# emmyoh/zebra

Measured on AMD Instinct MI355X. Metric: queries/sec, higher is better.
Workload: dtype f32

## Files before the change

### zebra_amd/csrc/zh_api.hip

```cpp
#include <algorithm>
#include <atomic>
#include <chrono>
#include <condition_variable>
#include <cmath>
#include <deque>
#include <cstdarg>
#include <cstdio>
#include <cstring>
#include <mutex>
#include <shared_mutex>
#include <new>
#include <string>
#include <thread>
#include <vector>

#include "zh_internal.h"
#include "zh_snapfile.h"

static thread_local std::string g_err;

static int fail(int code, const char *fmt, ...) {
    char buf[512];
    va_list ap;
    va_start(ap, fmt);
    vsnprintf(buf, sizeof buf, fmt, ap);
    va_end(ap);
    g_err = buf;
    return code;
}
#define HIPCHK(expr)                                                                                       \
    do {                                                                                                   \
        hipError_t e_ = (expr);                                                                            \
        if (e_ != hipSuccess)                                                                              \
            return fail(e_ == hipErrorOutOfMemory ? ZH_ENOMEM : ZH_EHIP, "%s: %s (%s:%d)", #expr,          \
                        hipGetErrorString(e_), __FILE__, __LINE__);                                        \
    } while (0)

int zh_set_error(int code, const char *fmt, ...) {
    char buf[512];
    va_list ap;
    va_start(ap, fmt);
    vsnprintf(buf, sizeof buf, fmt, ap);
    va_end(ap);
    g_err = buf;
    return code;
}

extern "C" const char *zh_last_error(void) { return g_err.c_str(); }
extern "C" const char *zh_version(void) { return "zebra-hip 0.1 (gfx950)"; }

struct DevBuf {
    void *p = nullptr;
    size_t cap = 0;
    bool defer = false;
    std::vector<void *> old;
    size_t old_bytes = 0;
    int ensure(size_t bytes, bool keep = false, hipStream_t s = nullptr) {
        if (bytes <= cap) return ZH_OK;
        if (defer) bytes += bytes / 8;
        if (defer && old_bytes + cap > (size_t(2) << 30)) {
            for (void *o : old) hipFree(o);
            old.clear();
            old_bytes = 0;
        }
        size_t ncap = std::max(bytes, cap + cap / 2);
        ncap = (ncap + 255) & ~size_t(255);
        void *np = nullptr;
        hipError_t e = hipMalloc(&np, ncap);
        if (e != hipSuccess) {
            ncap = (bytes + 255) & ~size_t(255);
            e = hipMalloc(&np, ncap);
        }
        if (e != hipSuccess) return fail(ZH_ENOMEM, "hipMalloc(%zu bytes): %s", ncap, hipGetErrorString(e));
        if (keep && p && cap) {
            e = hipMemcpyAsync(np, p, cap, hipMemcpyDeviceToDevice, s);
            if (e == hipSuccess) e = hipStreamSynchronize(s);
            if (e != hipSuccess) { hipFree(np); return fail(ZH_EHIP, "grow copy: %s", hipGetErrorString(e)); }
        }
        if (p) { if (defer) { old.push_back(p); old_bytes += cap; } else hipFree(p); }
        p = np;
        cap = ncap;
        return ZH_OK;
    }
    void release() {
        if (p) hipFree(p);
        for (void *o : old) hipFree(o);
        old.clear();
        old_bytes = 0;
        p = nullptr;
        cap = 0;
    }
    template <typename T>
    T *as() const { return reinterpret_cast<T *>(p); }
};

struct zh_search_ctx {
    zh_index *ix = nullptr;
    DevBuf wQQ, wBits, wCounts, wInline, wRowBase, wCandBase, wVisitBase, wTotals, wVisits, wKeys, wCandKeys, wCandIds,
        wLeafCount, wLeafFill, wGroupBase, wGroupRowBase, wGroups, wGroupRowOff, wWaveGroup, wVisitBits, wNodeVisit, wScore, wJunkBits, wZeros, wQnorm, wQpad, wFixList, wLogPool, wLogHead, wLogCtl,
        wPfRows, wPfCounts, wPfKeys, wPfIds, wPfAmb, wPfCtl, wUnc, wQh, wQmeta, wApList, wApCount, wApEx, wApExKeys, wApCtl, wRaw;
    ZhApprox dbg_ap{};
    bool dbg_valid = false, dbg_raw = false;
    size_t log_chunks = 0;
    ZhTotals *h_totals = nullptr;
    hipEvent_t ev[6] = {};
    hipEvent_t ev_totals = nullptr, ev_emit = nullptr, ev_sw0 = nullptr, ev_sw1 = nullptr;
    bool ev_ok = false;
    int state = 0;
    bool trivial = false;
    const float *dQ = nullptr;
    size_t B = 0, k = 0;
    size_t nwin = 1, bwin = 0;
    DevBuf wQwin, wOutWin;
    int metric = 0, mode = 0;
    uint32_t P_dense = 0, wpq = 0;
    hipStream_t s = nullptr;
    ZhTotals tot{};
    bool scan = false;
    bool approx_f32rows = false;
    bool approx_fused = false;
    bool approx_bytes = false;
    bool approx = false, approx_mfma = false, approx_leaf = false;
    uint32_t *h_ap = nullptr;
    bool score_hash = false;
    uint32_t score_Bp = 0;
    bool lazy_fix = false;
    bool prefilter = false, prefilter_off_once = false, stream_ordered = false;
    uint32_t pf_cap = 0;
    uint32_t *h_pf = nullptr;
    std::vector<const float *> sv_q;
    std::vector<uint64_t *> sv_ids, sv_keys;
    std::vector<uint32_t *> sv_counts;
    hipStream_t sv_heavy = nullptr;
    std::vector<DevBuf *> all_bufs() {
        return {&wQQ, &wBits, &wCounts, &wInline, &wRowBase, &wCandBase, &wVisitBase, &wTotals, &wVisits, &wKeys,
                &wCandKeys, &wCandIds, &wLeafCount, &wLeafFill, &wGroupBase, &wGroupRowBase, &wGroups, &wGroupRowOff, &wWaveGroup, &wVisitBits, &wNodeVisit, &wScore, &wJunkBits, &wZeros, &wQnorm, &wQpad, &wFixList,
                &wLogPool, &wLogHead, &wLogCtl, &wQwin, &wOutWin, &wPfRows, &wPfCounts, &wPfKeys, &wPfIds, &wPfAmb, &wPfCtl, &wUnc,
                &wQh, &wQmeta, &wApList, &wApCount, &wApEx, &wApExKeys, &wApCtl, &wRaw};
    }
    void release_all() {
        for (DevBuf *b : all_bufs()) b->release();
        if (ev_ok) { for (auto &e : ev) hipEventDestroy(e); hipEventDestroy(ev_totals); hipEventDestroy(ev_emit); hipEventDestroy(ev_sw0); hipEventDestroy(ev_sw1); ev_ok = false; }
        if (h_totals) { hipHostFree(h_totals); h_totals = nullptr; }
        if (h_pf) { hipHostFree(h_pf); h_pf = nullptr; }
        if (h_ap) { hipHostFree(h_ap); h_ap = nullptr; }
    }
};

struct zh_index {
    zh_options opt{};
    int device = 0;
    hipStream_t stream = nullptr;
    hipStream_t sweep_stream = nullptr;
    std::shared_mutex mu;

    DevBuf X;
    uint64_t n_rows = 0;

    DevBuf node_plane, node_left, node_right, node_pack, roots, planes, consts, leaf_ids;
    uint32_t n_nodes = 0, n_planes = 0, n_trees = 0;
    uint64_t n_leaf_ids = 0;
    std::vector<int32_t> h_plane, h_left, h_right;
    std::vector<uint32_t> h_roots;
    std::vector<uint32_t> planes_below_level;
    std::vector<uint32_t> h_leaf_ids;
    std::vector<uint8_t> h_dead;
    uint64_t n_dead = 0;
    uint64_t rows_gen = 1, dead_gen = 1;
    uint32_t max_leaf_len = 0;
    std::mutex blk_mu;

    struct Stamp {
        std::atomic<uint64_t> rows{0}, gen{0};
        bool is(uint64_t r, uint64_t g) const { return rows == r && gen == g; }
        void set(uint64_t r, uint64_t g) { rows = r; gen = g; }
    };
    struct BlocksView {
        DevBuf recs, upper, roots;
        std::atomic<uint32_t> n_blocks{0}, n_upper{0};
        std::atomic<bool> valid{false};
        std::atomic<bool> inner{false};
        std::atomic<size_t> recs_b{0};
        void mark_built(uint32_t blocks, uint32_t uppers, bool inner_only, size_t second_halves) {
            n_blocks = blocks; n_upper = uppers; inner = inner_only; recs_b = second_halves; valid = true;
        }
        void invalidate() { valid = false; }
        void drop() { recs.release(); upper.release(); roots.release(); n_blocks = 0; n_upper = 0; inner = false; recs_b = 0; valid = false; }
    } blocks;
    struct RowLeafView {
        DevBuf table;
        std::atomic<bool> valid{false}, failed{false};
        std::atomic<uint64_t> rows{0};
        uint64_t version = 0;
        bool current(const zh_index *ix) const { return valid && rows == ix->n_rows; }
        void mark_built(uint64_t n) { valid = true; rows = n; version++; }
        void mark_failed() { failed = true; }
        void invalidate() { valid = false; failed = false; }
        void drop() { table.release(); invalidate(); }
    } row_leaf;
    struct RowHalfView {
        DevBuf tiles, meta, rho_dev;
        Stamp at;
        std::atomic<bool> failed{false};
        std::atomic<float> rho{0.f};
        bool current(const zh_index *ix) const { return at.is(ix->n_rows, ix->rows_gen); }
        bool known_failed(const zh_index *ix) const { return failed && current(ix); }
        void mark_built(const zh_index *ix, float r) { rho = r; at.set(ix->n_rows, ix->rows_gen); }
        void mark_failed(const zh_index *ix) { failed = true; at.set(ix->n_rows, ix->rows_gen); }
        void retry() { failed = false; }
        void remake() { at.gen = 0; }
        void drop() { at.set(0, 0); rho = 0.f; tiles.release(); meta.release(); failed = false; }
    } half;
    struct ScanOrder {
        DevBuf perm, row_leaf_p;
        bool off = false;
        uint32_t keys = 0;
        double worth = 0;
        uint64_t rows = 0;
        uint64_t version = 0;
// ... 2164 lines not shown
    zh_index *ix = c->ix;
    if (c->state != 1) return fail(ZH_ESTATE, "zh_search_finish without zh_search_begin");
    const uint32_t d = ix->opt.dim, T = ix->n_trees;
    const size_t B = c->B, k = c->k, nwin = c->nwin, bwin = c->bwin;
    hipStream_t s = c->s;
    int rc;
    c->state = 0;
    if (c->trivial) {
        for (size_t j = 0; j < nwin && bwin; j++) {
            HIPCHK(hipMemsetAsync(outCounts[j], 0, bwin * 4, s));
            if (k) {
                HIPCHK(hipMemsetAsync(outIds[j], 0xFF, bwin * k * 8, s));
                HIPCHK(hipMemsetAsync(outKeys[j], 0xFF, bwin * k * 8, s));
            }
        }
        HIPCHK(hipEventRecord(c->ev[5], s));
        c->state = 2;
        return ZH_OK;
    }
    uint64_t *dOutIds = outIds[0], *dOutKeys = outKeys[0];
    uint32_t *dOutCounts = outCounts[0];
    if (nwin > 1) {
        if ((rc = c->wOutWin.ensure(B * k * 16 + B * 4))) { return rc; }
        dOutIds = c->wOutWin.as<uint64_t>();
        dOutKeys = dOutIds + B * k;
        dOutCounts = reinterpret_cast<uint32_t *>(dOutKeys + B * k);
    }
    HIPCHK(hipEventSynchronize(c->ev_totals));
    const ZhTotals tot = c->tot = *c->h_totals;
    {
        std::lock_guard<std::mutex> lk(ix->stats_mu);
        const double v = (double)tot.visits / (double)((uint64_t)B * T);
        ix->visits_per_pair = ix->visits_per_pair > 0 ? 0.5 * (ix->visits_per_pair + v) : v;
    }
    if (tot.visits > 0xFFFFFFFull || tot.rows >= (1ull << 36))
        return fail(ZH_ELIMIT, "more than 2^28 leaf visits or 2^36 scored rows in one batch; use a smaller batch");
    c->sv_ids.assign(outIds, outIds + nwin); c->sv_keys.assign(outKeys, outKeys + nwin); c->sv_counts.assign(outCounts, outCounts + nwin);
    c->sv_heavy = heavy;
    if (c->prefilter && (tot.flags & 1u)) {
        const std::vector<const float *> q = c->sv_q;
        c->prefilter_off_once = true;
        rc = ctx_begin(c, q.data(), nwin, bwin, k, c->metric, c->mode, s);
        c->prefilter_off_once = false;
        if (rc) return rc;
        return ctx_finish(c, outIds, outKeys, outCounts, heavy);
    }
    if (c->prefilter) return finish_prefilter(c, dOutIds, dOutKeys, dOutCounts, outIds, outKeys, outCounts);
    if ((rc = c->wVisits.ensure(std::max<uint64_t>(tot.visits, 1) * sizeof(ZhVisit)))) return rc;
    if ((rc = c->wGroups.ensure(std::max<uint64_t>(tot.groups, 1) * sizeof(ZhGroup)))) return rc;
    if ((rc = c->wGroupRowOff.ensure(std::max<uint64_t>(tot.groups, 1) * 8))) return rc;
    if ((rc = c->wWaveGroup.ensure((tot.group_rows / 64 + 2) * 4))) return rc;
    if ((rc = c->wKeys.ensure(std::max<uint64_t>(tot.rows, 1) * 8))) return rc;
    if ((rc = c->wCandKeys.ensure(std::max<uint64_t>(tot.takes, 1) * 8))) return rc;
    if ((rc = c->wCandIds.ensure(std::max<uint64_t>(tot.takes, 1) * 4))) return rc;
    ZhForestDev f = forest_dev(ix);
    if (!(tot.flags & 1u)) {
        HIPCHK(zh_launch_expand(f, (uint32_t)B, c->wCounts.as<ZhPairCounts>(), c->wInline.as<ZhVisit>(),
                                c->wRowBase.as<uint64_t>(), c->wCandBase.as<uint64_t>(), c->wVisitBase.as<uint64_t>(),
                                c->wVisits.as<ZhVisit>(), c->wLeafCount.as<uint32_t>(), c->wLeafFill.as<uint32_t>(),
                                c->wGroupBase.as<uint32_t>(), c->wGroupRowBase.as<uint64_t>(), c->wGroups.as<ZhGroup>(),
                                c->wGroupRowOff.as<uint64_t>(), walk_log(c), s));
    } else {
        if (c->lazy_fix)
            HIPCHK(zh_launch_score_unc_fix(c->dQ, (uint32_t)B, d, f.planes, f.consts, ix->n_planes, c->wBits.as<uint32_t>(), c->wUnc.as<uint32_t>(), c->wpq, s));
        HIPCHK(zh_launch_walk_emit(f, c->dQ, (uint32_t)B, d, (int32_t)k, c->wBits.as<uint32_t>(), c->wpq, c->P_dense,
                                   c->wCounts.as<ZhPairCounts>(), c->wInline.as<ZhVisit>(), c->wRowBase.as<uint64_t>(),
                                   c->wCandBase.as<uint64_t>(), c->wVisitBase.as<uint64_t>(), c->wVisits.as<ZhVisit>(),
                                   c->wLeafCount.as<uint32_t>(), c->wLeafFill.as<uint32_t>(), c->wGroupBase.as<uint32_t>(),
                                   c->wGroupRowBase.as<uint64_t>(), c->wGroups.as<ZhGroup>(), c->wGroupRowOff.as<uint64_t>(), s));
        const uint64_t pairs = (uint64_t)B * T;
        const uint64_t want = tot.visits / (ZH_LOG_CHUNK - 1) + std::min<uint64_t>(pairs, tot.visits / (ZH_INLINE_VISITS + 1)) + 16;
        static const bool fixed = getenv("ZH_WALK_LOG_FIXED") != nullptr;
        if (!fixed && want > c->log_chunks) {
            const size_t chunks = (size_t)(want + want / 2);
            if (c->wLogPool.ensure(chunks * ZH_LOG_CHUNK * sizeof(uint2)) == ZH_OK) c->log_chunks = chunks;
        }
    }
    c->scan = choose_scan(ix, tot, c->metric, B, k);
    if (c->scan && !ix->row_leaf.current(ix)) {
        std::lock_guard<std::mutex> lk(ix->blk_mu);
        if (!ix->row_leaf.current(ix) && !ix->row_leaf.failed && (rc = build_row_leaf(ix))) return rc;
        if (!ix->row_leaf.current(ix)) c->scan = false;
    }
    if (c->scan) {
        const size_t nn = std::max<uint32_t>(ix->n_nodes, 1);
        if ((rc = c->wVisitBits.ensure((nn + 31) / 32 * 4))) return rc;
        if ((rc = c->wNodeVisit.ensure(nn * sizeof(uint4)))) return rc;
        HIPCHK(zh_launch_node_visits(c->wLeafCount.as<uint32_t>(), c->wGroupBase.as<uint32_t>(), c->wGroups.as<ZhGroup>(), ix->n_nodes,
                                     c->wVisitBits.as<uint32_t>(), c->wNodeVisit.as<uint4>(), s));
    }
    if (!c->scan)
        HIPCHK(zh_launch_wave_groups(c->wGroups.as<ZhGroup>(), c->wGroupRowOff.as<uint64_t>(), tot.groups, c->wWaveGroup.as<uint32_t>(), s));
    c->approx = c->scan && use_approx(ix, tot, B, k, c->metric);
    c->approx_leaf = false; c->approx_bytes = false;
    if (!c->scan && use_approx_leaf(ix, tot, B, k, c->metric)) {
        bool ok = false;
        const char *be = getenv("ZH_S128H_BYTES"), *ke = getenv("ZH_S128H_KERNEL"), *de = getenv("ZH_S128H_DMA");
        const bool want_bytes = !(be && be[0] == '0') && !(ke && ke[0] == 'r') && !(de && de[0] == '1');
        std::lock_guard<std::mutex> lk(ix->blk_mu);
        if ((rc = ensure_row_half128(ix, &ok, want_bytes))) return rc;
        c->approx = c->approx_leaf = ok;
        c->approx_bytes = ok && ix->half128.bytes;
    }
    ZhApprox ap{};
    bool mfma = c->approx && !c->approx_leaf && mfma_wanted(ix) && B < (1u << 23) - 1;
    const uint2 *scan_row_leaf = ix->row_leaf.table.as<uint2>();
    if (mfma) {
        std::lock_guard<std::mutex> lk(ix->blk_mu);
        if ((rc = ensure_row_half(ix, &mfma))) return rc;
        if (mfma && ix->order.rows) {
            if ((rc = ensure_row_leaf_p(ix))) return rc;
            if (!ix->order.rows) {
                ix->order.switch_off();
                ix->half.remake();
                if ((rc = ensure_row_half(ix, &mfma))) return rc;
            } else
                scan_row_leaf = ix->order.row_leaf_p.as<uint2>();
        }
    }
    c->approx_mfma = mfma;
    c->approx_f32rows = mfma && ix->half.tiles.p == nullptr;
    if (c->approx) {
        const char *cap_e = getenv("ZH_APX_CAPS");
        unsigned e_capq = 0, e_excap = 0, e_exrows = 0;
        if (cap_e) sscanf(cap_e, "%u,%u,%u", &e_capq, &e_excap, &e_exrows);
        const uint32_t capq = e_capq ? std::min(e_capq, 8192u) : (ix->fb.approx_strikes.load() ? 8192u : 4096u);
        const uint32_t ex_cap = e_excap ? e_excap : (uint32_t)std::min<uint64_t>(std::max<uint64_t>(4096, tot.visits / 4 + 1024), 1u << 24);
        const uint32_t ex_rows = e_exrows ? e_exrows : (uint32_t)std::min<uint64_t>(std::max<uint64_t>(1u << 20, tot.rows / 16), 1u << 26);
        if ((rc = c->wQh.ensure(B * d * 2)) || (rc = c->wQmeta.ensure(B * sizeof(float4))) || (rc = c->wApList.ensure((size_t)B * capq * 12)) ||
            (rc = c->wApCount.ensure(B * 8 + std::max<uint64_t>(tot.visits, 1) * 4)) || (rc = c->wApEx.ensure((size_t)ex_cap * 8)) || (rc = c->wApExKeys.ensure((size_t)ex_rows * 20)) ||
            (rc = c->wApCtl.ensure(ZH_APX_CTL_WORDS * 4)))
            return rc;
        ap.Qh = c->wQh.p; ap.qmeta = c->wQmeta.as<float4>(); ap.iv = c->wKeys.as<uint64_t>();
        ap.list_lo = c->wApList.as<uint32_t>(); ap.list_hi = ap.list_lo + (size_t)B * capq; ap.list_id = ap.list_hi + (size_t)B * capq;
        ap.qcount = c->wApCount.as<uint32_t>(); ap.capq = capq; ap.qtau = ap.qcount + B; ap.tauv = ap.qtau + B;
        ap.ex_visits = c->wApEx.as<uint2>(); ap.ex_cap = ex_cap;
        ap.ex_keys = c->wApExKeys.as<uint64_t>(); ap.ex_ckeys = ap.ex_keys + ex_rows; ap.ex_cids = reinterpret_cast<uint32_t *>(ap.ex_ckeys + ex_rows);
        ap.ex_rows_cap = ex_rows; ap.ctl = c->wApCtl.as<uint32_t>();
        ap.n_queries = (uint32_t)B; ap.iv_cap = tot.rows;
        ap.mfma = mfma ? 1u : 0u; ap.row_half = mfma ? ix->half.tiles.p : nullptr; ap.row_meta = mfma ? ix->half.meta.as<float2>() : nullptr;
        ap.row_rho = mfma ? ix->half.rho.load() : 0.f;
        if (c->approx_leaf) { ap.mfma = 2u; ap.row_rho = ap.rho_norm = c->approx_bytes ? 0.f : ix->half128.rho.load(); }
        const char *pte = getenv("ZH_S128H_PRETEST");
        ap.nx_max = c->approx_leaf && c->approx_bytes && !(pte && pte[0] == '0') ? 2885.1f : 0.f;
        HIPCHK(hipMemsetAsync(c->wApCount.p, 0, B * 4, s));
        HIPCHK(hipMemsetAsync(ap.qtau, 0xFF, B * 4, s));
        HIPCHK(hipMemsetAsync(c->wApCtl.p, 0, ZH_APX_CTL_WORDS * 4, s));
        HIPCHK(zh_launch_qhalf(c->dQ, (uint32_t)B, d, c->wQh.p, c->wQmeta.as<float4>(), c->approx_leaf ? 2 : (mfma ? 1 : 0), s));
    }
    HIPCHK(hipEventRecord(c->ev[2], s));
    hipStream_t hs = heavy ? heavy : s;
    if (hs != s) { HIPCHK(hipEventRecord(c->ev_emit, s)); HIPCHK(hipStreamWaitEvent(hs, c->ev_emit, 0)); }
    HIPCHK(hipEventRecord(c->ev_sw0, hs));
    c->approx_fused = false;
    if (c->approx_leaf && k <= 64 && !ix->debug_keep_raw) {
        const char *fe = getenv("ZH_S128H_FUSED"), *ke = getenv("ZH_S128H_KERNEL"), *de = getenv("ZH_S128H_DMA");
        const bool lean = !(ke && ke[0] == 'r') && !(de && de[0] == '1');
        c->approx_fused = lean && (fe ? fe[0] == '1' : (!ix->fb.fused_off && tot.rows >= 1024 * std::max<uint64_t>(tot.visits, 1)));
    }
    const int kinda = c->metric != ZH_COSINE ? 0 : (c->mode == ZH_COSINE_PARITY ? 2 : 1);
    if (c->approx_leaf)
        HIPCHK(zh_launch_sweep128h(ix->half128.copy.p, c->wQh.p, ldexpf(1.f, ix->half128.ex - 14), c->wGroups.as<ZhGroup>(), c->wGroupRowOff.as<uint64_t>(),
                                   tot.groups, c->wWaveGroup.as<uint32_t>(), f.leaf_ids, tot.group_rows, c->wKeys.as<uint64_t>(), hs,
                                   c->approx_fused ? &ap : nullptr, kinda, (uint32_t)k, zh_approx_bound(c->metric, d, 2), c->approx_bytes));
    else if (c->approx)
        HIPCHK(zh_launch_scan_approx(ix->X.as<float>(), d, ix->n_rows, ap, mfma ? scan_row_leaf : ix->row_leaf.table.as<uint2>(), T, c->wVisitBits.as<uint32_t>(),
                                     c->wNodeVisit.as<uint4>(), c->wGroups.as<ZhGroup>(), f.group, c->metric, c->mode, hs));
    else if (c->scan)
        HIPCHK(zh_launch_scan_sweep(ix->X.as<float>(), d, ix->n_rows, c->dQ, c->wQQ.as<float>(), ix->row_leaf.table.as<uint2>(), T,
                                    c->wVisitBits.as<uint32_t>(), c->wNodeVisit.as<uint4>(), c->wGroups.as<ZhGroup>(), f.group,
                                    c->metric, c->mode, c->wKeys.as<uint64_t>(), nullptr, hs));
    else
        HIPCHK(zh_launch_sweep(ix->X.as<float>(), d, c->dQ, c->wQQ.as<float>(), c->wGroups.as<ZhGroup>(),
                               c->wGroupRowOff.as<uint64_t>(), tot.groups, c->wWaveGroup.as<uint32_t>(), f.leaf_ids,
                               tot.group_rows, c->metric, c->mode, c->wKeys.as<uint64_t>(), hs));
    HIPCHK(hipEventRecord(c->ev_sw1, hs));
    if (hs != s) HIPCHK(hipStreamWaitEvent(s, c->ev_sw1, 0));
    HIPCHK(hipEventRecord(c->ev[3], s));
    const uint32_t *run_if = nullptr;
    c->dbg_valid = c->approx;
    c->dbg_raw = false;
    if (c->approx) {
        c->dbg_ap = ap;
        if (ix->debug_keep_raw && tot.rows) {
            if ((rc = c->wRaw.ensure(tot.rows * 8))) return rc;
            HIPCHK(hipMemcpyAsync(c->wRaw.p, c->wKeys.p, tot.rows * 8, hipMemcpyDeviceToDevice, s));
            c->dbg_raw = true;
        }
        if (c->approx_fused) HIPCHK(zh_launch_exact_register(c->wVisits.as<ZhVisit>(), tot.visits, (uint32_t)k, ap, s));
        else HIPCHK(zh_launch_select_interval(c->wVisits.as<ZhVisit>(), tot.visits, (uint32_t)k, f.leaf_ids, ap, c->metric, c->mode, d, s));
        HIPCHK(hipEventRecord(c->ev[4], s));
        HIPCHK(zh_launch_final_interval(c->wVisits.as<ZhVisit>(), ix->X.as<float>(), d, c->dQ, c->wQQ.as<float>(), (uint32_t)B, (uint32_t)k,
                                        f.leaf_ids, c->metric, c->mode, ix->opt.id_base, ap, dOutIds, dOutKeys, dOutCounts, ix->max_leaf_len, s));
        HIPCHK(hipMemcpyAsync(c->h_ap, c->wApCtl.p, ZH_APX_CTL_WORDS * 4, hipMemcpyDeviceToHost, s));
        run_if = ap.ctl + 1;
        if (c->approx_leaf)
            HIPCHK(zh_launch_sweep(ix->X.as<float>(), d, c->dQ, c->wQQ.as<float>(), c->wGroups.as<ZhGroup>(), c->wGroupRowOff.as<uint64_t>(), tot.groups,
                                   c->wWaveGroup.as<uint32_t>(), f.leaf_ids, tot.group_rows, c->metric, c->mode, c->wKeys.as<uint64_t>(), s, run_if));
        else
            HIPCHK(zh_launch_scan_sweep(ix->X.as<float>(), d, ix->n_rows, c->dQ, c->wQQ.as<float>(), ix->row_leaf.table.as<uint2>(), T,
                                        c->wVisitBits.as<uint32_t>(), c->wNodeVisit.as<uint4>(), c->wGroups.as<ZhGroup>(), f.group,
                                        c->metric, c->mode, c->wKeys.as<uint64_t>(), run_if, s));
    }
    HIPCHK(zh_launch_select(c->wVisits.as<ZhVisit>(), tot.visits, f.leaf_ids, c->wKeys.as<uint64_t>(),
                            c->wCandKeys.as<uint64_t>(), c->wCandIds.as<uint32_t>(), ix->max_leaf_len, run_if, s));
    if (!c->approx) HIPCHK(hipEventRecord(c->ev[4], s));
    HIPCHK(zh_launch_final(c->wCandBase.as<uint64_t>(), (uint32_t)B, T, (uint32_t)k, c->wCandKeys.as<uint64_t>(),
                           c->wCandIds.as<uint32_t>(), ix->opt.id_base, dOutIds, dOutKeys, dOutCounts, run_if, s));
    for (size_t j = 0; j < nwin && nwin > 1; j++) {
        HIPCHK(hipMemcpyAsync(outIds[j], dOutIds + j * bwin * k, bwin * k * 8, hipMemcpyDeviceToDevice, s));
        HIPCHK(hipMemcpyAsync(outKeys[j], dOutKeys + j * bwin * k, bwin * k * 8, hipMemcpyDeviceToDevice, s));
        HIPCHK(hipMemcpyAsync(outCounts[j], dOutCounts + j * bwin, bwin * 4, hipMemcpyDeviceToDevice, s));
    }
    HIPCHK(hipEventRecord(c->ev[5], s));
    c->state = 2;
    return ZH_OK;
}

int ctx_wait(zh_search_ctx *c) {
    zh_index *ix = c->ix;
    if (c->state == 1) return fail(ZH_ESTATE, "zh_search_wait: the batch was begun but not finished");
    if (c->state != 2) return ZH_OK;
    c->state = 0;
    HIPCHK(hipEventSynchronize(c->ev[5]));
    if (c->trivial) return ZH_OK;
    const bool pf = c->prefilter;
    const uint32_t pf_amb = pf ? c->h_pf[0] : 0, pf_flags = pf ? c->h_pf[1] : 0, pf_exact = pf ? c->h_pf[2] : 0;
    if (pf_flags) {
        {
            std::lock_guard<std::mutex> lk(ix->stats_mu);
            ix->stats.prefilter_fallbacks_accum++;
            ix->stats.prefilter_last_overflow = pf_flags;
        }
        ix->fb.prefilter_ran_over();
        const std::vector<const float *> q = c->sv_q;
        const std::vector<uint64_t *> ids = c->sv_ids, keys = c->sv_keys;
        const std::vector<uint32_t *> counts = c->sv_counts;
        c->prefilter_off_once = true;
        int rc = ctx_begin(c, q.data(), c->nwin, c->bwin, c->k, c->metric, c->mode, c->s);
        if (!rc) rc = ctx_finish(c, ids.data(), keys.data(), counts.data(), c->sv_heavy);
        c->prefilter_off_once = false;
        if (rc) return rc;
        return ctx_wait(c);
    }
    if (pf) ix->fb.prefilter_held();
    const ZhTotals tot = c->tot;
    uint64_t uniq = 0;
    if (ix->profiling >= 2 && tot.visits && !pf) {
        std::vector<ZhVisit> hv(tot.visits);
        HIPCHK(hipMemcpy(hv.data(), c->wVisits.p, tot.visits * sizeof(ZhVisit), hipMemcpyDeviceToHost));
        std::vector<std::pair<uint32_t, uint32_t>> leaves(hv.size());
        for (size_t i = 0; i < hv.size(); i++) leaves[i] = {hv[i].leaf_off, hv[i].len};
        std::sort(leaves.begin(), leaves.end());
        leaves.erase(std::unique(leaves.begin(), leaves.end()), leaves.end());
        for (auto &l : leaves) uniq += l.second;
    }
    float ms[5] = {0, 0, 0, 0, 0};
    if (ix->profiling > 0) {
        for (int i = 0; i < 5; i++) HIPCHK(hipEventElapsedTime(&ms[i], c->ev[i], c->ev[i + 1]));
        HIPCHK(hipEventElapsedTime(&ms[2], c->ev_sw0, c->ev_sw1));
    }
    std::lock_guard<std::mutex> lk(ix->stats_mu);
    zh_stats_t &st = ix->stats;
    st.batch = c->B; st.window_batches = c->nwin; st.visits = tot.visits; st.rows_scored = tot.rows; st.candidates = tot.takes;
    st.planes_dense = c->P_dense; st.planes_total = ix->n_planes;
    const uint64_t swept = pf ? pf_exact : (c->scan ? ix->n_rows : tot.group_rows);
    st.rows_swept = swept;
    st.sweep_bytes = pf ? tot.rows * 64 + (uint64_t)pf_exact * 4 * ix->opt.dim
                        : (c->scan ? ix->n_rows * ((uint64_t)4 * ix->opt.dim + 8 * ix->n_trees) + tot.rows * 8
                                   : tot.group_rows * ((uint64_t)4 * ix->opt.dim + 4) + tot.rows * 8);
    st.table_scan = c->scan && !pf ? 1 : 0;
    const bool apx = c->approx && !pf;
    st.approx_scan = apx ? (c->approx_leaf ? 3 : (c->approx_mfma ? 2 : 1)) : 0;
    st.approx_fused = apx && c->approx_leaf && c->approx_fused ? 1 : 0;
    st.approx_byte_rows = apx && c->approx_leaf && c->approx_bytes ? 1 : 0;
    st.approx_exact_visits = apx ? c->h_ap[0] : 0;
    st.approx_survivors = apx ? c->h_ap[3] : 0;
    st.approx_list_entries = apx ? c->h_ap[4] : 0;
    if (apx && c->h_ap[7]) fprintf(stderr, "zebra_hip: scan guard tripped, bits %u (diagnostic build)\n", c->h_ap[7]);
    st.approx_columns = apx && c->approx_mfma ? c->h_ap[5] : 0;
    st.approx_column_pairs = apx && c->approx_mfma ? c->h_ap[6] : 0;
    if (apx && c->h_ap[1]) {
        st.approx_fallbacks_accum++;
        st.approx_last_overflow = c->h_ap[1];
// ... 3683 lines not shown
```

### zebra_amd/csrc/zh_approx.hip

```cpp

#include <cstdlib>

#include "zh_internal.h"
#include "zh_device.h"

#ifndef ZH_APX_G768
#define ZH_APX_G768 2
#endif
#ifndef ZH_APX_G128
#define ZH_APX_G128 8
#endif
uint32_t zh_approx_groups(uint32_t d) {
    switch (d) {
    case 128: return ZH_APX_G128;
    case 256: case 384: return 4;
    case 768: return ZH_APX_G768;
    case 512: case 1024: return 2;
    default: return 0;
    }
}
bool zh_approx_pays(uint32_t d) { return d >= 384; }

float zh_approx_bound(int metric, uint32_t d, int mfma) {
    const double u = 5.9604644775390625e-8, c0 = (d + 255) / 256 + 8.0, ops = mfma ? 33.0 * (d / 128) + 2.0 + (mfma == 2 ? 40.0 : 0.0) : 0.0;
    if (metric == ZH_COSINE) return (float)(1.01 * (2.0 * c0 + 80.0 + 2.0 * ops) * u);
    return (float)(1.01 * (c0 + 100.0 + ops) * u);
}

__device__ __forceinline__ _Float16 f16_no_subnormal(float v) {
    const _Float16 h = (_Float16)v;
    return fabsf((float)h) < 6.103515625e-05f ? (_Float16)0.f : h;
}

template <int G>
__global__ __launch_bounds__(64) void qhalf_kernel(const float *__restrict__ Q, uint32_t B, uint32_t d, _Float16 *__restrict__ Qh,
                                                    float4 *__restrict__ qmeta) {
    constexpr uint32_t LG = 64 / G;
    const uint32_t b = blockIdx.x, lane = threadIdx.x;
    const float *q = Q + (size_t)b * d;
    float m = 0.f, s2 = 0.f;
    bool bad = false;
    for (uint32_t e = lane; e < d; e += 64) {
        const float v = q[e];
        bad |= !(v - v == 0.f);
        m = fmaxf(m, fabsf(v));
        s2 = __builtin_fmaf(v, v, s2);
    }
    m = wave_butterfly<OpMax>(m);
    s2 = wave_sum_canonical(s2);
    bad = __ballot(bad) != 0;
    float sigma = 1.f, inv = 1.f;
    if (!bad && m > 0.f) {
        int ex = 0;
        (void)frexpf(m, &ex);
        if (ex < -90 || ex > 90) bad = true;
        else { sigma = ldexpf(1.f, 14 - ex); inv = ldexpf(1.f, ex - 14); }
    }
    float d2 = 0.f;
    for (uint32_t e = lane; e < d; e += 64) {
        const float v = bad ? 0.f : q[e];
        const _Float16 h = f16_no_subnormal(v * sigma);
        const float df = v - (float)h * inv;
        d2 = __builtin_fmaf(df, df, d2);
        const uint32_t j = e / (4 * LG), rem = e % (4 * LG), l = rem / 4, t = rem % 4, i = j / 2, wh = j % 2;
        Qh[(size_t)b * d + ((size_t)(i * LG + l)) * 8 + wh * 4 + t] = h;
    }
    d2 = wave_sum_canonical(d2);
    if (lane == 0) {
        float4 o;
        if (bad || !(s2 - s2 == 0.f)) o = make_float4(NAN, NAN, NAN, NAN);
        else o = make_float4(inv, s2, sqrtf(s2) * (1.0f + 1e-5f), sqrtf(d2) * 1.001f);
        qmeta[b] = o;
    }
}

hipError_t zh_launch_qhalf(const float *dQ, uint32_t B, uint32_t d, void *dQh, float4 *dQmeta, int layout, hipStream_t s) {
    if (!B) return hipSuccess;
    const uint32_t G = layout == 2 ? 64 : (layout == 1 ? 16 : zh_approx_groups(d));
    if (G == 64) hipLaunchKernelGGL(qhalf_kernel<64>, dim3(B), dim3(64), 0, s, dQ, B, d, (_Float16 *)dQh, dQmeta);
    else if (G == 16) hipLaunchKernelGGL(qhalf_kernel<16>, dim3(B), dim3(64), 0, s, dQ, B, d, (_Float16 *)dQh, dQmeta);
    else if (G == 8) hipLaunchKernelGGL(qhalf_kernel<8>, dim3(B), dim3(64), 0, s, dQ, B, d, (_Float16 *)dQh, dQmeta);
    else if (G == 4) hipLaunchKernelGGL(qhalf_kernel<4>, dim3(B), dim3(64), 0, s, dQ, B, d, (_Float16 *)dQh, dQmeta);
    else if (G == 2) hipLaunchKernelGGL(qhalf_kernel<2>, dim3(B), dim3(64), 0, s, dQ, B, d, (_Float16 *)dQh, dQmeta);
    else return hipErrorInvalidValue;
    return hipGetLastError();
}

template <int LG>
__device__ __forceinline__ float group_sum(float s) {
    s = s + dpp_mov<0xB1>(s);
    s = s + dpp_mov<0x4E>(s);
    s = s + dpp_mov<0x141>(s);
    if (LG >= 16) s = s + dpp_mov<0x140>(s);
    if (LG >= 32) s = xor16<OpAdd>(s);
    if (LG >= 64) {
        const auto r = __builtin_amdgcn_permlane32_swap(__float_as_uint(s), __float_as_uint(s), false, false);
        s = __uint_as_float(r[0]) + __uint_as_float(r[1]);
    }
    return s;
}


__device__ __forceinline__ uint32_t scan_phase1(uint32_t lane, uint32_t n_ent, const uint2 *__restrict__ ent,
                                                const uint32_t *__restrict__ visitBits, const uint4 *__restrict__ nodeVisit,
                                                uint32_t *eGb, uint32_t *eWithin, uint32_t *eC, uint32_t *off, uint32_t *eB0, uint64_t *eK0) {
    unsigned long long rlw[ZH_SCAN_NE];
#pragma unroll
    for (int j = 0; j < ZH_SCAN_NE; j++) {
        const uint32_t e = lane + 64u * j;
        rlw[j] = __builtin_nontemporal_load(reinterpret_cast<const unsigned long long *>(ent + (e < n_ent ? e : 0)));
    }
    uint32_t word[ZH_SCAN_NE];
    bool in[ZH_SCAN_NE];
#pragma unroll
    for (int j = 0; j < ZH_SCAN_NE; j++) {
        const uint32_t node = (uint32_t)rlw[j];
        in[j] = lane + 64u * j < n_ent && node != 0xFFFFFFFFu;
        word[j] = visitBits[in[j] ? node >> 5 : 0];
    }
    uint4 nv[ZH_SCAN_NE];
#pragma unroll
    for (int j = 0; j < ZH_SCAN_NE; j++) {
        const uint32_t node = (uint32_t)rlw[j];
        in[j] = in[j] && ((word[j] >> (node & 31)) & 1u);
        nv[j] = nodeVisit[in[j] ? node : 0];
    }
    uint32_t P = 0;
#pragma unroll
    for (int j = 0; j < ZH_SCAN_NE; j++) {
        eWithin[j] = (uint32_t)(rlw[j] >> 32);
        eC[j] = in[j] ? nv[j].x & 0x0FFFFFFFu : 0u;
        eGb[j] = nv[j].y; eB0[j] = nv[j].z;
        eK0[j] = ((uint64_t)(nv[j].x >> 28) << 32) | nv[j].w;
        uint32_t incl = eC[j];
#pragma unroll
        for (int o = 1; o < 64; o <<= 1) {
            const uint32_t t = __shfl_up(incl, o);
            if (lane >= (uint32_t)o) incl += t;
        }
        off[j] = P + incl - eC[j];
        P += (uint32_t)__builtin_amdgcn_readlane((int)incl, 63);
    }
    return P;
}

#define ZH_APX_CAP 512
#ifndef ZH_APX_WAVES
#define ZH_APX_WAVES 0
#endif
#ifndef ZH_APX_REPL_ROWS
#define ZH_APX_REPL_ROWS 0
#endif
template <int D, int G, int KINDA>
__global__ __launch_bounds__(256)
#if ZH_APX_WAVES
__attribute__((amdgpu_waves_per_eu(ZH_APX_WAVES, 8)))
#endif
void scan_approx_kernel(const float *__restrict__ X, const uint4 *__restrict__ Qh,
                                                           const float4 *__restrict__ qmeta, const uint2 *__restrict__ rowLeaf,
                                                           uint32_t T, uint32_t RW, const uint32_t *__restrict__ visitBits,
                                                           const uint4 *__restrict__ nodeVisit, const ZhGroup *__restrict__ groups,
                                                           uint32_t GRP, uint64_t row_begin, uint64_t row_end, float Kc,
                                                           uint64_t *__restrict__ iv) {
    constexpr int LG = 64 / G, NH = D * G / 512, NR = 2 * NH;
    constexpr int RB = NR <= 6 ? 4 : 2;
    static_assert(D * G % 512 == 0 && NH >= 1, "a lane's share of a query is whole 16-byte loads");
    __shared__ uint4 pair_list[4][ZH_APX_CAP];
    __shared__ uint32_t row_start[4][20];
    const uint32_t lane = threadIdx.x & 63, l = lane & (LG - 1), g = lane / LG;
    const uint32_t wid = (uint32_t)__builtin_amdgcn_readfirstlane((int)(threadIdx.x >> 6));
    const uint64_t wave = (uint64_t)blockIdx.x * (blockDim.x >> 6) + wid;
    const uint64_t r0 = row_begin + wave * RW;
    if (r0 >= row_end) return;
    const uint32_t nr = (uint32_t)(row_end - r0 < RW ? row_end - r0 : RW);
    const uint32_t n_ent = nr * T;
    const uint2 *__restrict__ ent = rowLeaf + (size_t)r0 * T;
    uint32_t eGb[ZH_SCAN_NE], eWithin[ZH_SCAN_NE], eC[ZH_SCAN_NE], off[ZH_SCAN_NE], eB0[ZH_SCAN_NE];
    uint64_t eK0[ZH_SCAN_NE];
    const uint32_t P = scan_phase1(lane, n_ent, ent, visitBits, nodeVisit, eGb, eWithin, eC, off, eB0, eK0);
    if (P == 0) return;
    const float4 *__restrict__ X4 = reinterpret_cast<const float4 *>(X);
    float my_s = 0.f, my_a2 = 0.f;
    uint64_t my_slot = 0;
    uint32_t nst = 0;
    bool my_on = false;
    auto flush = [&]() {
        if (my_on) __builtin_nontemporal_store(((uint64_t)__float_as_uint(my_a2) << 32) | __float_as_uint(my_s), iv + my_slot);
        my_on = false;
        nst = 0;
    };
    auto load_q = [&](uint32_t b, uint4 *hq) {
        const uint4 *qp = Qh + (size_t)b * (D / 8) + l;
#pragma unroll
        for (int i = 0; i < NH; i++) hq[i] = qp[i * LG];
    };
    auto load_x = [&](uint64_t row, float4 *v) {
        if constexpr (G == 2 && !ZH_APX_REPL_ROWS) {
            const float4 *r4 = X4 + (size_t)row * (D / 4) + lane;
#pragma unroll
            for (int j = 0; j < NR / 2; j++) {
                const float4 t = ld16<true>(r4 + 64 * j);
                const auto sx = __builtin_amdgcn_permlane32_swap(__float_as_uint(t.x), __float_as_uint(t.x), false, false);
                const auto sy = __builtin_amdgcn_permlane32_swap(__float_as_uint(t.y), __float_as_uint(t.y), false, false);
                const auto sz = __builtin_amdgcn_permlane32_swap(__float_as_uint(t.z), __float_as_uint(t.z), false, false);
                const auto sw = __builtin_amdgcn_permlane32_swap(__float_as_uint(t.w), __float_as_uint(t.w), false, false);
                v[2 * j] = make_float4(__uint_as_float(sx[0]), __uint_as_float(sy[0]), __uint_as_float(sz[0]), __uint_as_float(sw[0]));
                v[2 * j + 1] = make_float4(__uint_as_float(sx[1]), __uint_as_float(sy[1]), __uint_as_float(sz[1]), __uint_as_float(sw[1]));
            }
        } else {
            const float4 *r4 = X4 + (size_t)row * (D / 4) + l;
#pragma unroll
            for (int j = 0; j < NR; j++) v[j] = ld16<true>(r4 + LG * j);
        }
    };
    auto row_sumsq = [&](const float4 *v) {
        float4 c = make_float4(0.f, 0.f, 0.f, 0.f);
#pragma unroll
        for (int j = 0; j < NR; j++) sq4(v[j], c);
        return group_sum<LG>((c.x + c.y) + (c.z + c.w));
    };
    auto dot_h = [&](const float4 *v, const uint4 *hq) {
        float ax = 0.f, ay = 0.f, az = 0.f, aw = 0.f;
#pragma unroll
        for (int i = 0; i < NH; i++) {
            f16x8 h;
            __builtin_memcpy(&h, &hq[i], 16);
            ax = __builtin_fmaf(v[2 * i].x, (float)h[0], ax);
            ay = __builtin_fmaf(v[2 * i].y, (float)h[1], ay);
            az = __builtin_fmaf(v[2 * i].z, (float)h[2], az);
            aw = __builtin_fmaf(v[2 * i].w, (float)h[3], aw);
            ax = __builtin_fmaf(v[2 * i + 1].x, (float)h[4], ax);
            ay = __builtin_fmaf(v[2 * i + 1].y, (float)h[5], ay);
            az = __builtin_fmaf(v[2 * i + 1].z, (float)h[6], az);
            aw = __builtin_fmaf(v[2 * i + 1].w, (float)h[7], aw);
        }
        return group_sum<LG>((ax + ay) + (az + aw));
    };
    auto stash = [&](float s, float a2, uint32_t, uint64_t slot, bool valid) {
        if (l == nst) { my_s = s; my_a2 = a2; my_slot = slot; my_on = valid; }
        if (++nst == (uint32_t)LG) flush();
    };
    if (P <= ZH_APX_CAP) {
        uint4 *list = pair_list[wid];
        uint32_t *rstart = row_start[wid];
        uint32_t mrows = 0;
#pragma unroll
        for (int j = 0; j < ZH_SCAN_NE; j++) {
            const uint32_t e = lane + 64u * j, c = eC[j];
            if (e < n_ent && e % T == 0) rstart[e / T] = off[j];
            if (c) {
                const uint32_t rl = e / T, gb = eGb[j];
                mrows |= 1u << rl;
                {
                    const uint64_t slot = eK0[j] + eWithin[j];
                    list[off[j]] = make_uint4(rl, eB0[j], (uint32_t)slot, (uint32_t)(slot >> 32));
                }
                for (uint32_t sidx = 1; sidx < c; sidx++) {
                    const ZhGroup *gp = groups + gb + sidx / GRP;
                    const uint64_t slot = gp->key_off[sidx % GRP] + eWithin[j];
                    list[off[j] + sidx] = make_uint4(rl, gp->b[sidx % GRP], (uint32_t)slot, (uint32_t)(slot >> 32));
                }
            }
// ... 70 lines not shown
                    uint4 hq[NH];
                    load_q(b, hq);
                    const float s = dot_h(v, hq);
                    stash(s, a2, b, gp->key_off[sidx % GRP] + w, s0 + g < c);
                }
            }
        }
    }
    flush();
}


__global__ __launch_bounds__(256) void row_half_kernel(const float *__restrict__ X, uint64_t row0, uint64_t n_rows, uint32_t d,
                                                       _Float16 *__restrict__ Xh, float2 *__restrict__ rowMeta, uint32_t *__restrict__ rhoMax,
                                                       const uint32_t *__restrict__ perm, uint64_t perm_rows) {
    const uint32_t lane = threadIdx.x & 63, NS = d / 32;
    const uint64_t nw = (uint64_t)gridDim.x * 4;
    float rho_w = 0.f;
    for (uint64_t i = (uint64_t)blockIdx.x * 4 + (threadIdx.x >> 6); i < n_rows; i += nw) {
        const uint64_t row = row0 + i;
        const float *x = X + (size_t)(perm && row < perm_rows ? perm[row] : row) * d;
        float m = 0.f, a2 = 0.f;
        bool bad = false;
        for (uint32_t e = lane; e < d; e += 64) {
            const float v = x[e];
            bad |= !(v - v == 0.f);
            m = fmaxf(m, fabsf(v));
            a2 = __builtin_fmaf(v, v, a2);
        }
        m = wave_butterfly<OpMax>(m);
        a2 = wave_sum_canonical(a2);
        bad = __ballot(bad) != 0;
        bool usable = false;
        float sigma = 1.f, inv = __uint_as_float(0x7FC00000u);
        if (!bad) {
            int ex = 14;
            if (m > 0.f) (void)frexpf(m, &ex);
            if (ex >= -100 && ex <= 100) { usable = true; sigma = ldexpf(1.f, 14 - ex); inv = ldexpf(1.f, ex - 14); }
        }
        float s2 = 0.f, d2 = 0.f;
        _Float16 *tile = Xh + ((size_t)(row >> 4) * NS * 64 + (row & 15)) * 8;
        for (uint32_t e = lane; e < d; e += 64) {
            const float v = x[e] * sigma;
            const _Float16 hv = usable ? f16_no_subnormal(v) : (_Float16)0.f;
            const float df = v - (float)hv;
            s2 = __builtin_fmaf(v, v, s2);
            d2 = __builtin_fmaf(df, df, d2);
            const uint32_t st = e >> 5, w = e & 31, hh = (w & 15) >> 2, j = (w & 3) + ((w >> 4) << 2);
            if (Xh) tile[((size_t)st * 64 + hh * 16) * 8 + j] = hv;
        }
        s2 = wave_sum_canonical(s2);
        d2 = wave_sum_canonical(d2);
        if (usable && s2 > 0.f) rho_w = fmaxf(rho_w, sqrtf(d2) * 1.001f / (sqrtf(s2) * 0.9999f));
        if (lane == 0) rowMeta[row] = make_float2(a2, inv);
    }
    if (lane == 0 && rho_w > 0.f) atomicMax(rhoMax, __float_as_uint(rho_w));
}

hipError_t zh_launch_row_half(const float *dX, uint64_t row0, uint64_t n_rows, uint32_t d, void *dXh, float2 *dRowMeta, uint32_t *dRhoMax,
                              const uint32_t *dPerm, uint64_t perm_rows, hipStream_t s) {
    if (!n_rows) return hipSuccess;
    const uint64_t blocks = std::min<uint64_t>((n_rows + 3) / 4, 256 * 32);
    hipLaunchKernelGGL(row_half_kernel, dim3((uint32_t)blocks), dim3(256), 0, s, dX, row0, n_rows, d, (_Float16 *)dXh, dRowMeta, dRhoMax, dPerm, perm_rows);
    return hipGetLastError();
}

__global__ __launch_bounds__(256) void permute_row_leaf_kernel(const uint2 *__restrict__ rowLeaf, const uint32_t *__restrict__ perm, uint64_t perm_rows,
                                                               uint64_t n_entries, uint32_t T, uint2 *__restrict__ out) {
    for (uint64_t e = (uint64_t)blockIdx.x * blockDim.x + threadIdx.x; e < n_entries; e += (uint64_t)gridDim.x * blockDim.x) {
        const uint64_t p = e / T, t = e % T;
        out[e] = rowLeaf[(size_t)(p < perm_rows ? perm[p] : p) * T + t];
    }
}
hipError_t zh_launch_permute_row_leaf(const uint2 *dRowLeaf, const uint32_t *dPerm, uint64_t perm_rows, uint64_t n_rows, uint32_t T, uint2 *dOut, hipStream_t s) {
    const uint64_t n = n_rows * T;
    if (!n) return hipSuccess;
    hipLaunchKernelGGL(permute_row_leaf_kernel, dim3((uint32_t)std::min<uint64_t>((n + 255) / 256, 256 * 64)), dim3(256), 0, s, dRowLeaf, dPerm, perm_rows, n, T, dOut);
    return hipGetLastError();
}

#ifndef ZH_MFMA_CL
#define ZH_MFMA_CL 0
#endif
#ifdef ZH_SCAN_GUARD
#define ZH_GUARD(cond, bit) ((cond) ? true : (atomicOr(guard, (bit)), false))
#else
#define ZH_GUARD(cond, bit) true
#endif
#ifdef ZH_SCAN_PROF
__device__ unsigned long long zh_scan_prof_buf[16];
extern "C" __attribute__((visibility("default"))) int zh_debug_scan_prof(uint64_t *out, uint32_t words, int reset) {
    static const unsigned long long zero[16] = {};
    if (reset) return (int)hipMemcpyToSymbol(HIP_SYMBOL(zh_scan_prof_buf), zero, sizeof(zero));
    return (int)hipMemcpyFromSymbol(out, HIP_SYMBOL(zh_scan_prof_buf), (size_t)words * 8);
}
#define SP(...) __VA_ARGS__
#else
#define SP(...)
#endif
#ifndef ZH_MFMA_WAVES
#define ZH_MFMA_WAVES 3
#endif
template <int D, bool F32ROWS>
__global__ __launch_bounds__(256) __attribute__((amdgpu_waves_per_eu(D > 768 ? 2 : ZH_MFMA_WAVES, D > 768 ? 2 : ZH_MFMA_WAVES)))
void scan_mfma_kernel(const u32x4 *__restrict__ Xh, const float *__restrict__ Xf, const float2 *__restrict__ rowMeta,
                                                         const uint4 *__restrict__ Qh, const uint2 *__restrict__ rowLeaf, uint32_t T,
                                                         uint32_t RW, const uint32_t *__restrict__ visitBits,
                                                         const uint4 *__restrict__ nodeVisit, const ZhGroup *__restrict__ groups,
                                                         uint32_t GRP, uint64_t row_begin, uint64_t row_end, uint64_t *__restrict__ iv,
                                                         uint32_t *__restrict__ colStats ,
                                                         uint32_t nq, uint64_t iv_cap, uint32_t *__restrict__ guard) {
    constexpr int NS = D / 32;
    constexpr int NL = D / 64;
    constexpr int CL = ZH_MFMA_CL ? ZH_MFMA_CL : (NL % 4 == 0 ? 2 : 3);
    constexpr int NCH = NL / CL;
    static_assert(D % 128 == 0 && NL % CL == 0 && NCH % 2 == 0, "four accumulators; the chunk registers alternate with a static parity");
    __shared__ uint64_t pair_list[4][ZH_APX_CAP > CL * 256 ? ZH_APX_CAP : CL * 256];
    __shared__ uint64_t tile_list[4][ZH_APX_CAP];
    __shared__ uint32_t col_query[4][ZH_APX_CAP];
    __shared__ uint32_t tile_start[4][36];
    __shared__ f32x4 acc_lds[4][64];
    __shared__ float2 row_meta[4][16];
    const uint32_t lane = threadIdx.x & 63, c16 = lane & 15, h = lane >> 4;
    const uint32_t wid = (uint32_t)__builtin_amdgcn_readfirstlane((int)(threadIdx.x >> 6));
    const uint64_t wave = (uint64_t)blockIdx.x * (blockDim.x >> 6) + wid;
    const uint64_t r0 = row_begin + wave * RW;
    if (r0 >= row_end) return;
    SP(const uint64_t sp0 = clock64();)
    const uint32_t nr = (uint32_t)(row_end - r0 < RW ? row_end - r0 : RW);
    const uint32_t n_ent = nr * T;
    const uint2 *__restrict__ ent = rowLeaf + (size_t)r0 * T;
    uint32_t eGb[ZH_SCAN_NE], eWithin[ZH_SCAN_NE], eC[ZH_SCAN_NE], off[ZH_SCAN_NE], eB0[ZH_SCAN_NE];
    uint64_t eK0[ZH_SCAN_NE];
    const uint32_t P = scan_phase1(lane, n_ent, ent, visitBits, nodeVisit, eGb, eWithin, eC, off, eB0, eK0);
    if (P == 0) return;
    SP(const uint64_t sp1 = clock64();)
    uint64_t *list = pair_list[wid];
    const bool listed = P <= ZH_APX_CAP;
    auto pack = [](uint32_t rl, uint32_t b, uint64_t slot) { return slot | ((uint64_t)b << 36) | ((uint64_t)rl << 60); };
#pragma unroll
    for (int j = 0; j < ZH_SCAN_NE; j++) {
        const uint32_t e = lane + 64u * j, c = eC[j];
        if (c && listed && ZH_GUARD(off[j] + c <= (uint32_t)ZH_APX_CAP && e / T < 16u, 32u)) {
            const uint32_t rl = e / T, gb = eGb[j];
            list[off[j]] = pack(rl, eB0[j], eK0[j] + eWithin[j]);
            for (uint32_t sidx = 1; sidx < c; sidx++) {
                const ZhGroup *gp = groups + gb + sidx / GRP;
                list[off[j] + sidx] = pack(rl, gp->b[sidx % GRP], gp->key_off[sidx % GRP] + eWithin[j]);
            }
        }
    }
    SP(__builtin_amdgcn_s_waitcnt(0); const uint64_t sp2 = clock64();)
    f16x8 A[NS];
    if constexpr (!F32ROWS) {
        const u32x4 *tp = Xh + (size_t)(r0 >> 4) * (NS * 64) + lane;
#pragma unroll
        for (int st = 0; st < NS; st++) A[st] = __builtin_bit_cast(f16x8, __builtin_nontemporal_load(tp + 64 * st));
        if (lane < 16) row_meta[wid][lane] = rowMeta[r0 + (lane < nr ? lane : 0u)];
        __builtin_amdgcn_fence(__ATOMIC_RELEASE, "wavefront");
        __builtin_amdgcn_wave_barrier();
    } else {
        if (lane < 16) row_meta[wid][lane] = rowMeta[r0 + (lane < nr ? lane : 0u)];
        __builtin_amdgcn_fence(__ATOMIC_RELEASE, "wavefront");
        __builtin_amdgcn_wave_barrier();
        const float inv_c = row_meta[wid][c16].y;
        const bool usable_c = inv_c - inv_c == 0.f;
        const float sigma_c = usable_c ? 1.0f / inv_c : 0.f;
        f32x4 *xt = reinterpret_cast<f32x4 *>(tile_list[wid]);
        const f32x4 *X4 = reinterpret_cast<const f32x4 *>(Xf);
        const uint32_t g4 = lane >> 4, p16 = lane & 15;
        auto cvt8 = [&](const f32x4 lo, const f32x4 hi) {
            f16x8 o;
#pragma unroll
            for (int t = 0; t < 4; t++) {
                o[t] = usable_c ? f16_no_subnormal(lo[t] * sigma_c) : (_Float16)0.f;
                o[4 + t] = usable_c ? f16_no_subnormal(hi[t] * sigma_c) : (_Float16)0.f;
            }
            return o;
        };
        f32x4 Rr[4];
        auto issue_rows = [&](int kb) {
#pragma unroll
            for (int i = 0; i < 4; i++) {
                const uint32_t rr = 4u * i + g4;
                Rr[i] = __builtin_nontemporal_load(X4 + (size_t)(r0 + (rr < nr ? rr : nr - 1)) * (D / 4) + kb * 16 + p16);
            }
        };
        issue_rows(0);
#pragma unroll
        for (int kb = 0; kb < D / 64; kb++) {
#pragma unroll
            for (int i = 0; i < 4; i++) {
                const uint32_t rr = 4u * i + g4;
                xt[rr * 16 + (p16 ^ rr)] = Rr[i];
            }
            __builtin_amdgcn_fence(__ATOMIC_RELEASE, "wavefront");
            __builtin_amdgcn_wave_barrier();
            if (kb + 1 < D / 64) issue_rows(kb + 1);
#pragma unroll
            for (int s2 = 0; s2 < 2; s2++) {
                const f32x4 lo = xt[c16 * 16 + ((8u * s2 + h) ^ c16)], hi = xt[c16 * 16 + ((8u * s2 + 4u + h) ^ c16)];
                A[2 * kb + s2] = cvt8(lo, hi);
            }
            __builtin_amdgcn_fence(__ATOMIC_RELEASE, "wavefront");
            __builtin_amdgcn_wave_barrier();
        }
    }
    const float2 *rmeta = row_meta[wid];
    u32x4 *stg = reinterpret_cast<u32x4 *>(pair_list[wid]);
    const u32x4 *__restrict__ Qv = reinterpret_cast<const u32x4 *>(Qh);
    const uint32_t g8 = lane >> 3, pc = lane & 7;
    const uint32_t swA = (g8 >> 1) & 7u, swB = (4u + (g8 >> 1)) & 7u;
    const uint32_t rd0 = (c16 >> 3) * 64u + (c16 & 7u) * 8u + ((h ^ (c16 >> 1)) & 7u);
    const uint32_t rd1 = (c16 >> 3) * 64u + (c16 & 7u) * 8u + (((4u + h) ^ (c16 >> 1)) & 7u);
    auto issue = [&](uint32_t bA, uint32_t bB, int chunk, u32x4 *dst) {
        if (!ZH_GUARD(bA < nq && bB < nq, 1u)) { bA = 0; bB = 0; }
        const u32x4 *qa = Qv + (size_t)bA * (D / 8) + (size_t)(chunk * CL * 8) + (pc ^ swA);
// ... 101 lines not shown
        }
        __builtin_amdgcn_fence(__ATOMIC_RELEASE, "wavefront");
        __builtin_amdgcn_wave_barrier();
        const uint32_t nt = (nd + 15) / 16;
        SP(const uint64_t sp3 = clock64();)
        if (colStats && lane == 0 && (wave & 63u) == 0u) { atomicAdd(&colStats[0], nd); atomicAdd(&colStats[1], P); }
        auto col_b = [&](uint32_t t, uint32_t col) { const uint32_t ci = 16 * t + col; return colq[ci < nd ? ci : nd - 1]; };
        uint32_t bA = col_b(0, g8), bB = col_b(0, 8 + g8);
        u32x4 ra[2 * CL], rb[2 * CL];
        issue(bA, bB, 0, ra);
        SP(__builtin_amdgcn_s_waitcnt(0); const uint64_t sp4 = clock64();)
        f32x4 *al = acc_lds[wid];
        for (uint32_t t = 0; t < nt; t++) {
            f32x4 acc[4] = {{0.f, 0.f, 0.f, 0.f}, {0.f, 0.f, 0.f, 0.f}, {0.f, 0.f, 0.f, 0.f}, {0.f, 0.f, 0.f, 0.f}};
#pragma unroll
            for (int c = 0; c < NCH; c += 2) {
                issue(bA, bB, c + 1, rb);
                to_lds(ra);
                mfma_chunk(c, acc);
                if (c + 2 < NCH) issue(bA, bB, c + 2, ra);
                else {
                    bA = col_b(t + 1, g8); bB = col_b(t + 1, 8 + g8);
                    issue(bA, bB, 0, ra);
                }
                to_lds(rb);
                mfma_chunk(c + 1, acc);
            }
            al[c16 * 4 + h] = (acc[0] + acc[1]) + (acc[2] + acc[3]);
            __builtin_amdgcn_fence(__ATOMIC_RELEASE, "wavefront");
            __builtin_amdgcn_wave_barrier();
            const uint32_t pe = tstart[t + 1];
            for (uint32_t pi = tstart[t] + lane; pi < pe; pi += 64) {
                const uint64_t rec = tl[pi];
                const uint32_t rl = (uint32_t)(rec >> 60), col = (uint32_t)(rec >> 36) & 15u;
                const float sv = reinterpret_cast<const float *>(al)[col * 16 + rl];
                const float2 rm = rmeta[rl];
                if (ZH_GUARD((rec & 0xFFFFFFFFFull) < iv_cap, 2u))
                    __builtin_nontemporal_store(((uint64_t)__float_as_uint(rm.x) << 32) | __float_as_uint(sv * rm.y), iv + (rec & 0xFFFFFFFFFull));
            }
            __builtin_amdgcn_wave_barrier();
        }
        SP(if ((wave & 15u) == 0u && lane == 0) {
            __builtin_amdgcn_s_waitcnt(0);
            const uint64_t sp5 = clock64();
            atomicAdd(&zh_scan_prof_buf[0], 1ull); atomicAdd(&zh_scan_prof_buf[1], sp1 - sp0); atomicAdd(&zh_scan_prof_buf[2], sp2 - sp1);
            atomicAdd(&zh_scan_prof_buf[3], sp3 - sp2); atomicAdd(&zh_scan_prof_buf[4], sp4 - sp3); atomicAdd(&zh_scan_prof_buf[5], sp5 - sp4);
            atomicAdd(&zh_scan_prof_buf[6], (unsigned long long)nt); atomicAdd(&zh_scan_prof_buf[7], (unsigned long long)P);
            atomicAdd(&zh_scan_prof_buf[8], (unsigned long long)nd); atomicAdd(&zh_scan_prof_buf[9], sp5 - sp0);
        })
    } else {
#pragma unroll
        for (int j = 0; j < ZH_SCAN_NE; j++) {
            unsigned long long m = __ballot(eC[j] != 0);
            while (m) {
                const int ll = __builtin_ctzll(m);
                m &= m - 1;
                const uint32_t c = (uint32_t)__builtin_amdgcn_readlane((int)eC[j], ll);
                const uint32_t gb = (uint32_t)__builtin_amdgcn_readlane((int)eGb[j], ll);
                const uint32_t w = (uint32_t)__builtin_amdgcn_readlane((int)eWithin[j], ll);
                const uint32_t rl = ((uint32_t)ll + 64u * j) / T;
                for (uint32_t s0 = 0; s0 < c; s0 += 16) {
                    auto visit_b = [&](uint32_t col) { const uint32_t si = s0 + col < c ? s0 + col : c - 1; return groups[gb + si / GRP].b[si % GRP]; };
                    const uint32_t bA = visit_b(g8), bB = visit_b(8 + g8);
                    const uint32_t sidx = s0 + c16 < c ? s0 + c16 : c - 1;
                    const ZhGroup *gp = groups + gb + sidx / GRP;
                    f32x4 acc[4] = {{0.f, 0.f, 0.f, 0.f}, {0.f, 0.f, 0.f, 0.f}, {0.f, 0.f, 0.f, 0.f}, {0.f, 0.f, 0.f, 0.f}};
                    u32x4 rq[2 * CL];
#pragma unroll
                    for (int cc = 0; cc < NCH; cc++) {
                        issue(bA, bB, cc, rq);
                        to_lds(rq);
                        mfma_chunk(cc, acc);
                        __builtin_amdgcn_sched_barrier(0);
                    }
                    emit(acc, rl, gp->key_off[sidx % GRP] + w, s0 + c16 < c);
                }
            }
        }
    }
}

template <int D>
static hipError_t launch_scan_mfma_d(const float *dX, uint64_t n_rows, const ZhApprox &ap, const uint2 *dRowLeaf, uint32_t T,
                                     const uint32_t *dVisitBits, const uint4 *dNodeVisit, const ZhGroup *dGroups, uint32_t group, hipStream_t s) {
    const uint32_t RW = zh_scan_rows_per_wave(T);
    uint64_t rows_per_launch = zh_sweep_rows_per_launch(D);
    rows_per_launch = rows_per_launch / (4 * RW) * (4 * RW);
    for (uint64_t r = 0; r < n_rows; r += rows_per_launch) {
        const uint64_t r_end = r + rows_per_launch < n_rows ? r + rows_per_launch : n_rows;
        const uint64_t waves = (r_end - r + RW - 1) / RW, blocks = (waves + 3) / 4;
        if (blocks > 0x7FFFFFFFull) return hipErrorInvalidValue;
        if (ap.row_half)
            hipLaunchKernelGGL((scan_mfma_kernel<D, false>), dim3((uint32_t)blocks), dim3(256), 0, s, (const u32x4 *)ap.row_half, dX, ap.row_meta, (const uint4 *)ap.Qh, dRowLeaf, T, RW,
                               dVisitBits, dNodeVisit, dGroups, group, r, r_end, ap.iv, ap.ctl + 5, ap.n_queries, ap.iv_cap, ap.ctl + 7);
        else
            hipLaunchKernelGGL((scan_mfma_kernel<D, true>), dim3((uint32_t)blocks), dim3(256), 0, s, (const u32x4 *)nullptr, dX, ap.row_meta, (const uint4 *)ap.Qh, dRowLeaf, T, RW,
                               dVisitBits, dNodeVisit, dGroups, group, r, r_end, ap.iv, ap.ctl + 5, ap.n_queries, ap.iv_cap, ap.ctl + 7);
    }
    return hipGetLastError();
}

__global__ __launch_bounds__(256) void absmax_kernel(const float *__restrict__ X, uint64_t n, uint32_t *__restrict__ out) {
    float m = 0.f;
    for (uint64_t i = (uint64_t)blockIdx.x * blockDim.x + threadIdx.x; i < n; i += (uint64_t)gridDim.x * blockDim.x) {
        const float v = fabsf(X[i]);
        if (v - v == 0.f) m = fmaxf(m, v);
    }
    m = wave_butterfly<OpMax>(m);
    if ((threadIdx.x & 63) == 0 && m > 0.f) atomicMax(out, __float_as_uint(m));
}

__global__ __launch_bounds__(256) void row_half128_kernel(const float *__restrict__ X, uint64_t row0, uint64_t n_rows, float sigma,
                                                          _Float16 *__restrict__ Xh, uint32_t *__restrict__ rhoMax) {
    const uint32_t lane = threadIdx.x & 63;
    const uint64_t nw = (uint64_t)gridDim.x * 4;
    float rho_w = 0.f;
    for (uint64_t i = (uint64_t)blockIdx.x * 4 + (threadIdx.x >> 6); i < n_rows; i += nw) {
        const uint64_t row = row0 + i;
        const float2 x = reinterpret_cast<const float2 *>(X + (size_t)row * 128)[lane];
        const float v0 = x.x * sigma, v1 = x.y * sigma;
        bool bad = !(v0 - v0 == 0.f) || !(v1 - v1 == 0.f) || fabsf(v0) > 60000.f || fabsf(v1) > 60000.f;
        const _Float16 h0 = f16_no_subnormal(v0), h1 = f16_no_subnormal(v1);
        const float d0 = v0 - (float)h0, d1 = v1 - (float)h1;
        const float s2 = wave_sum_canonical(__builtin_fmaf(v0, v0, v1 * v1));
        const float d2 = wave_sum_canonical(__builtin_fmaf(d0, d0, d1 * d1));
        const float m = wave_butterfly<OpMax>(fmaxf(fabsf(x.x), fabsf(x.y)));
        bad = __ballot(bad) != 0 || !(s2 - s2 == 0.f) || (s2 == 0.f && m > 0.f);
        const float rho = s2 > 0.f ? sqrtf(d2) * 1.001f / (sqrtf(s2) * 0.9999f) : 0.f;
        bad = bad || !(rho <= 9.765625e-4f);
        if (!bad) rho_w = fmaxf(rho_w, rho);
        const _Float16 nanh = (_Float16)__uint_as_float(0x7FC00000u);
        typedef _Float16 f16x2v __attribute__((ext_vector_type(2)));
        reinterpret_cast<f16x2v *>(Xh + (size_t)row * 128)[lane] = bad ? f16x2v{nanh, nanh} : f16x2v{h0, h1};
    }
    if (lane == 0 && rho_w > 0.f) atomicMax(rhoMax, __float_as_uint(rho_w));
}

hipError_t zh_launch_absmax(const float *dX, uint64_t n, uint32_t *dOut, hipStream_t s) {
    if (!n) return hipSuccess;
    hipLaunchKernelGGL(absmax_kernel, dim3((uint32_t)std::min<uint64_t>((n + 255) / 256, 256 * 16)), dim3(256), 0, s, dX, n, dOut);
    return hipGetLastError();
}
hipError_t zh_launch_row_half128(const float *dX, uint64_t row0, uint64_t n_rows, float sigma, void *dXh, uint32_t *dRhoMax, hipStream_t s) {
    if (!n_rows) return hipSuccess;
    hipLaunchKernelGGL(row_half128_kernel, dim3((uint32_t)std::min<uint64_t>((n_rows + 3) / 4, 256 * 32)), dim3(256), 0, s, dX, row0, n_rows, sigma,
                       (_Float16 *)dXh, dRhoMax);
    return hipGetLastError();
}

__global__ __launch_bounds__(256) void row_byte128_kernel(const float4 *__restrict__ X4, uint64_t n4, uint32_t *__restrict__ Xb,
                                                          uint32_t *__restrict__ notBytes) {
    bool bad = false;
    for (uint64_t i = (uint64_t)blockIdx.x * 256 + threadIdx.x; i < n4; i += (uint64_t)gridDim.x * 256) {
        const float4 v = X4[i];
        const float e[4] = {v.x, v.y, v.z, v.w};
        uint32_t w = 0;
#pragma unroll
        for (int j = 0; j < 4; j++) {
            const uint32_t b = (uint32_t)fminf(fmaxf(e[j], 0.f), 255.f);
            bad |= !((float)b == e[j]);
            w |= b << (8 * j);
        }
        Xb[i] = w;
    }
    if (__ballot(bad) != 0 && (threadIdx.x & 63) == 0) atomicOr(notBytes, 1u);
}
hipError_t zh_launch_row_byte128(const float *dX, uint64_t row0, uint64_t n_rows, void *dXb, uint32_t *dNotBytes, hipStream_t s) {
    if (!n_rows) return hipSuccess;
    const uint64_t n4 = n_rows * 32;
    hipLaunchKernelGGL(row_byte128_kernel, dim3((uint32_t)std::min<uint64_t>((n4 + 255) / 256, 256 * 32)), dim3(256), 0, s,
                       reinterpret_cast<const float4 *>(dX + (size_t)row0 * 128), n4, reinterpret_cast<uint32_t *>(dXb) + (size_t)row0 * 32, dNotBytes);
    return hipGetLastError();
}
__device__ __forceinline__ f16x8 bytes8_to_f16(uint32_t w0, uint32_t w1) {
    typedef _Float16 h2 __attribute__((ext_vector_type(2)));
    const h2 off = {(_Float16)-1024.f, (_Float16)-1024.f};
    const h2 a = __builtin_bit_cast(h2, __builtin_amdgcn_perm(0x64646464u, w0, 0x04010400u)) + off;
    const h2 b = __builtin_bit_cast(h2, __builtin_amdgcn_perm(0x64646464u, w0, 0x04030402u)) + off;
    const h2 c = __builtin_bit_cast(h2, __builtin_amdgcn_perm(0x64646464u, w1, 0x04010400u)) + off;
    const h2 d = __builtin_bit_cast(h2, __builtin_amdgcn_perm(0x64646464u, w1, 0x04030402u)) + off;
// ... 880 lines not shown
#define ZH_S128L_CH 4
#endif
#ifndef ZH_S128F_CH
#define ZH_S128F_CH 16
#endif
#ifndef ZH_S128H_LAUNCH_X
#define ZH_S128H_LAUNCH_X 4
#endif
#ifndef ZH_S128B_LAUNCH_X
#define ZH_S128B_LAUNCH_X 8
#endif
#ifndef ZH_S128B_CH
#define ZH_S128B_CH 64
#endif
uint64_t zh_sweep128h_rows_per_launch(bool lean, bool byte_rows) {
    return (lean ? (byte_rows ? ZH_S128B_LAUNCH_X : ZH_S128H_LAUNCH_X) : 1) * zh_sweep_rows_per_launch(128);
}
template <int FUSE, bool BYTES>
static void launch_sweep128h_lean(const void *dXh, const void *dQh, float inv, const ZhGroup *dGroups, const uint64_t *dGroupRowOff, uint64_t n_groups,
                                  const uint32_t *dWaveGroup, const uint32_t *dLeafIds, uint64_t R_grouped, uint64_t *dIv, const ZhApprox &ap,
                                  uint32_t k_top, float Kc, hipStream_t s) {
    const uint64_t rows_per_launch = zh_sweep128h_rows_per_launch(true, BYTES);
    for (uint64_t r = 0; r < R_grouped; r += rows_per_launch) {
        const uint64_t r_end = r + rows_per_launch < R_grouped ? r + rows_per_launch : R_grouped;
        constexpr int CHL = FUSE >= 0 ? (BYTES ? ZH_S128B_CH : ZH_S128F_CH) : ZH_S128L_CH;
        const uint64_t wl = (r_end - r + 64 * CHL - 1) / (64 * CHL);
        if constexpr (BYTES)
            hipLaunchKernelGGL((sweep128b_lean_kernel<CHL, FUSE>), dim3((uint32_t)((wl + 3) / 4)), dim3(256), 0, s, (const u32x4 *)dXh,
                               (const u32x4 *)dQh, dGroups, dGroupRowOff, n_groups, dWaveGroup, dLeafIds, r, r_end, dIv, ap, k_top, Kc);
        else
            hipLaunchKernelGGL((sweep128h_lean_kernel<CHL, FUSE>), dim3((uint32_t)((wl + 3) / 4)), dim3(256), 0, s, (const u32x4 *)dXh,
                               (const u32x4 *)dQh, inv, dGroups, dGroupRowOff, n_groups, dWaveGroup, dLeafIds, r, r_end, dIv, ap, k_top, Kc);
    }
    const uint64_t bw = ((R_grouped + 63) / 64 + 63) / 64, bb = (bw + 3) / 4;
    hipLaunchKernelGGL((sweep128h_boundary_kernel<FUSE, BYTES>), dim3((uint32_t)bb), dim3(256), 0, s, (const u32x4 *)dXh, (const u32x4 *)dQh, inv, dGroups,
                       dGroupRowOff, n_groups, dWaveGroup, dLeafIds, (uint64_t)0, R_grouped, dIv, ap, k_top, Kc);
}
hipError_t zh_launch_sweep128h(const void *dXh, const void *dQh, float inv, const ZhGroup *dGroups, const uint64_t *dGroupRowOff, uint64_t n_groups,
                               const uint32_t *dWaveGroup, const uint32_t *dLeafIds, uint64_t R_grouped, uint64_t *dIv, hipStream_t s,
                               const ZhApprox *fuse, int fuse_kinda, uint32_t k_top, float Kc, bool byte_rows) {
    if (R_grouped == 0 || n_groups == 0) return hipSuccess;
    constexpr int CH = 4;
    const uint64_t rows_per_launch = zh_sweep_rows_per_launch(128);
    if ((R_grouped + 16383) / 16384 > 0x7FFFFFFFull) return hipErrorInvalidValue;
    const char *dma_e = getenv("ZH_S128H_DMA"), *kern_e = getenv("ZH_S128H_KERNEL");
    const bool dma = dma_e && dma_e[0] == '1', r5 = kern_e && kern_e[0] == 'r';
    if (fuse) {
        if (!dWaveGroup || k_top == 0 || k_top > 64) return hipErrorInvalidValue;
#define ZH_LEAN(F)                                                                                                                                  \
    do {                                                                                                                                            \
        if (byte_rows) launch_sweep128h_lean<F, true>(dXh, dQh, 1.f, dGroups, dGroupRowOff, n_groups, dWaveGroup, dLeafIds, R_grouped, dIv, *fuse, k_top, Kc, s); \
        else launch_sweep128h_lean<F, false>(dXh, dQh, inv, dGroups, dGroupRowOff, n_groups, dWaveGroup, dLeafIds, R_grouped, dIv, *fuse, k_top, Kc, s);           \
    } while (0)
        if (fuse_kinda == 0) ZH_LEAN(0);
        else if (fuse_kinda == 1) ZH_LEAN(1);
        else ZH_LEAN(2);
#undef ZH_LEAN
        return hipGetLastError();
    }
    if (!dma && !r5) {
        const ZhApprox none{};
        if (byte_rows) launch_sweep128h_lean<-1, true>(dXh, dQh, 1.f, dGroups, dGroupRowOff, n_groups, dWaveGroup, dLeafIds, R_grouped, dIv, none, 0u, 0.f, s);
        else launch_sweep128h_lean<-1, false>(dXh, dQh, inv, dGroups, dGroupRowOff, n_groups, dWaveGroup, dLeafIds, R_grouped, dIv, none, 0u, 0.f, s);
        return hipGetLastError();
    }
    if (byte_rows) return hipErrorInvalidValue;
    for (uint64_t r = 0; r < R_grouped; r += rows_per_launch) {
        const uint64_t r_end = r + rows_per_launch < R_grouped ? r + rows_per_launch : R_grouped;
        const uint64_t w = (r_end - r + 64 * CH - 1) / (64 * CH), blocks = (w + 3) / 4;
        if (!dma)
            hipLaunchKernelGGL((sweep128h_kernel<CH>), dim3((uint32_t)blocks), dim3(256), 0, s, (const u32x4 *)dXh, (const u32x4 *)dQh, inv, dGroups,
                               dGroupRowOff, n_groups, dWaveGroup, dLeafIds, r, r_end, dIv);
        else
            hipLaunchKernelGGL((sweep128h_dma_kernel<CH>), dim3((uint32_t)blocks), dim3(256), 0, s, (const u32x4 *)dXh, (const u32x4 *)dQh, inv, dGroups,
                               dGroupRowOff, n_groups, dWaveGroup, dLeafIds, r, r_end, dIv);
    }
    return hipGetLastError();
}


template <int G, int KINDA>
__global__ __launch_bounds__(256) void scan_approx128_kernel(const float *__restrict__ X, const uint4 *__restrict__ Qh,
                                                              const float4 *__restrict__ qmeta, const uint2 *__restrict__ rowLeaf,
                                                              uint32_t T, uint32_t RW, const uint32_t *__restrict__ visitBits,
                                                              const uint4 *__restrict__ nodeVisit, const ZhGroup *__restrict__ groups,
                                                              uint32_t GRP, uint64_t row_begin, uint64_t row_end, float Kc,
                                                              uint64_t *__restrict__ iv) {
    constexpr int LG = 64 / G, NH = G / 4, NR = 2 * NH;
    constexpr uint32_t CAP = 240;
    __shared__ uint64_t pair_list[4][CAP];
    __shared__ float4 row_lds[4][16 * 32];
    __shared__ float a2_lds[4][16];
    const uint32_t lane = threadIdx.x & 63, l = lane & (LG - 1), g = lane / LG;
    const uint32_t wid = (uint32_t)__builtin_amdgcn_readfirstlane((int)(threadIdx.x >> 6));
    const uint64_t wave = (uint64_t)blockIdx.x * (blockDim.x >> 6) + wid;
    const uint64_t r0 = row_begin + wave * RW;
    if (r0 >= row_end) return;
    const uint32_t nr = (uint32_t)(row_end - r0 < RW ? row_end - r0 : RW);
    const uint32_t n_ent = nr * T;
    const uint2 *__restrict__ ent = rowLeaf + (size_t)r0 * T;
    uint32_t eGb[ZH_SCAN_NE], eWithin[ZH_SCAN_NE], eC[ZH_SCAN_NE], off[ZH_SCAN_NE], eB0[ZH_SCAN_NE];
    uint64_t eK0[ZH_SCAN_NE];
    const uint32_t P = scan_phase1(lane, n_ent, ent, visitBits, nodeVisit, eGb, eWithin, eC, off, eB0, eK0);
    if (P == 0) return;
    {
        const float4 *src = reinterpret_cast<const float4 *>(X) + (size_t)r0 * 32;
        float4 t[8];
#pragma unroll
        for (int i = 0; i < 8; i++) t[i] = (lane + 64u * i < nr * 32u) ? ld16<true>(src + lane + 64 * i) : make_float4(0.f, 0.f, 0.f, 0.f);
#pragma unroll
        for (int i = 0; i < 8; i++) row_lds[wid][lane + 64 * i] = t[i];
    }
    __builtin_amdgcn_fence(__ATOMIC_RELEASE, "wavefront");
    __builtin_amdgcn_wave_barrier();
#pragma unroll
    for (int rr = 0; rr < 16 / G; rr++) {
        const uint32_t row = g + (uint32_t)G * rr;
        float4 c = make_float4(0.f, 0.f, 0.f, 0.f);
#pragma unroll
        for (int j = 0; j < NR; j++) sq4(row_lds[wid][row * 32 + LG * j + l], c);
        const float a2 = group_sum<LG>((c.x + c.y) + (c.z + c.w));
        if (l == 0) a2_lds[wid][row] = a2;
    }
    float my_s = 0.f;
    uint64_t my_slot = 0;
    uint32_t my_row = 0, nst = 0;
    bool my_on = false;
    auto flush = [&]() {
        if (my_on) __builtin_nontemporal_store(((uint64_t)__float_as_uint(a2_lds[wid][my_row]) << 32) | __float_as_uint(my_s), iv + my_slot);
        my_on = false;
        nst = 0;
    };
    struct Ops { float4 v[NR]; uint4 hq[NH]; };
    auto fetch = [&](uint32_t row, uint32_t b, Ops &o) {
#pragma unroll
        for (int i = 0; i < NH; i++) o.hq[i] = Qh[(size_t)b * 16 + i * LG + l];
#pragma unroll
        for (int j = 0; j < NR; j++) o.v[j] = row_lds[wid][row * 32 + LG * j + l];
    };
    auto dot8 = [&](const Ops &o) {
        float ax = 0.f, ay = 0.f, az = 0.f, aw = 0.f;
#pragma unroll
        for (int i = 0; i < NH; i++) {
            f16x8 h;
            __builtin_memcpy(&h, &o.hq[i], 16);
            ax = __builtin_fmaf(o.v[2 * i].x, (float)h[0], ax); ay = __builtin_fmaf(o.v[2 * i].y, (float)h[1], ay);
            az = __builtin_fmaf(o.v[2 * i].z, (float)h[2], az); aw = __builtin_fmaf(o.v[2 * i].w, (float)h[3], aw);
            ax = __builtin_fmaf(o.v[2 * i + 1].x, (float)h[4], ax); ay = __builtin_fmaf(o.v[2 * i + 1].y, (float)h[5], ay);
            az = __builtin_fmaf(o.v[2 * i + 1].z, (float)h[6], az); aw = __builtin_fmaf(o.v[2 * i + 1].w, (float)h[7], aw);
        }
        return group_sum<LG>((ax + ay) + (az + aw));
    };
    auto stash = [&](float s, uint32_t row, uint32_t, uint64_t slot, bool valid) {
        if (l == nst) { my_s = s; my_row = row; my_slot = slot; my_on = valid; }
        if (++nst == (uint32_t)LG) flush();
    };
    auto pack = [](uint32_t rl, uint32_t b, uint64_t slot) { return slot | ((uint64_t)b << 36) | ((uint64_t)rl << 60); };
    if (P <= CAP) {
        uint64_t *list = pair_list[wid];
#pragma unroll
        for (int j = 0; j < ZH_SCAN_NE; j++) {
            const uint32_t e = lane + 64u * j, c = eC[j];
            if (c) {
                const uint32_t rl = e / T, gb = eGb[j];
                {
                    const uint64_t slot = eK0[j] + eWithin[j];
                    list[off[j]] = pack(rl, eB0[j], slot);
                }
                for (uint32_t sidx = 1; sidx < c; sidx++) {
                    const ZhGroup *gp = groups + gb + sidx / GRP;
                    const uint64_t slot = gp->key_off[sidx % GRP] + eWithin[j];
                    list[off[j] + sidx] = pack(rl, gp->b[sidx % GRP], slot);
                }
            }
        }
        __builtin_amdgcn_fence(__ATOMIC_RELEASE, "wavefront");
        __builtin_amdgcn_wave_barrier();
        auto r_row = [](uint64_t r) { return (uint32_t)(r >> 60); };
        auto r_b = [](uint64_t r) { return (uint32_t)(r >> 36) & 0xFFFFFFu; };
        uint64_t rec = list[g < P ? g : P - 1];
        Ops cur;
        fetch(r_row(rec), r_b(rec), cur);
        for (uint32_t p = 0; p < P; p += G) {
            const uint32_t pn = p + G + g;
            const uint64_t recn = list[pn < P ? pn : P - 1];
            Ops nxt;
            fetch(r_row(recn), r_b(recn), nxt);
            const float s = dot8(cur);
            stash(s, r_row(rec), r_b(rec), rec & 0xFFFFFFFFFull, p + g < P);
            rec = recn; cur = nxt;
        }
    } else {
#pragma unroll
        for (int j = 0; j < ZH_SCAN_NE; j++) {
            unsigned long long m = __ballot(eC[j] != 0);
            while (m) {
                const int ll = __builtin_ctzll(m);
                m &= m - 1;
                const uint32_t c = (uint32_t)__builtin_amdgcn_readlane((int)eC[j], ll);
                const uint32_t gb = (uint32_t)__builtin_amdgcn_readlane((int)eGb[j], ll);
                const uint32_t w = (uint32_t)__builtin_amdgcn_readlane((int)eWithin[j], ll);
                const uint32_t rl = ((uint32_t)ll + 64u * j) / T;
                for (uint32_t s0 = 0; s0 < c; s0 += G) {
                    const uint32_t sidx = s0 + g < c ? s0 + g : c - 1;
                    const ZhGroup *gp = groups + gb + sidx / GRP;
                    const uint32_t b = gp->b[sidx % GRP];
                    Ops o;
                    fetch(rl, b, o);
                    const float s = dot8(o);
                    stash(s, rl, b, gp->key_off[sidx % GRP] + w, s0 + g < c);
                }
            }
        }
    }
    flush();
}

template <int D, int G>
static hipError_t launch_scan_approx_d(const float *dX, uint64_t n_rows, const ZhApprox &ap, const uint2 *dRowLeaf, uint32_t T,
                                       const uint32_t *dVisitBits, const uint4 *dNodeVisit, const ZhGroup *dGroups, uint32_t group,
                                       int metric, int mode, hipStream_t s) {
    const uint32_t RW = zh_scan_rows_per_wave(T);
    uint64_t rows_per_launch = zh_sweep_rows_per_launch(D);
    rows_per_launch = rows_per_launch / (4 * RW) * (4 * RW);
    const float Kc = zh_approx_bound(metric, D, 0);
    const int kinda = metric == ZH_COSINE ? (mode == ZH_COSINE_PARITY ? 2 : 1) : 0;
    for (uint64_t r = 0; r < n_rows; r += rows_per_launch) {
        const uint64_t r_end = r + rows_per_launch < n_rows ? r + rows_per_launch : n_rows;
        const uint64_t waves = (r_end - r + RW - 1) / RW, blocks = (waves + 3) / 4;
        if (blocks > 0x7FFFFFFFull) return hipErrorInvalidValue;
#define ZH_APX_LAUNCH(KA) \
        hipLaunchKernelGGL((scan_approx_kernel<D, G, KA>), dim3((uint32_t)blocks), dim3(256), 0, s, dX, (const uint4 *)ap.Qh, ap.qmeta, dRowLeaf, T, \
                           RW, dVisitBits, dNodeVisit, dGroups, group, r, r_end, Kc, ap.iv)
        if (kinda == 0) ZH_APX_LAUNCH(0);
        else if (kinda == 1) ZH_APX_LAUNCH(1);
        else ZH_APX_LAUNCH(2);
#undef ZH_APX_LAUNCH
    }
    return hipGetLastError();
}

bool zh_scan_mfma_supported(uint32_t d, uint32_t T) { return (d == 256 || d == 384 || d == 512 || d == 768 || d == 1024) && zh_scan_rows_per_wave(T) == 16; }
bool zh_scan_approx_supported(uint32_t d, uint32_t T, int metric) {
    if (metric != ZH_L2 && metric != ZH_L2SQ && metric != ZH_COSINE) return false;
    return zh_approx_groups(d) != 0 && zh_scan_rows_per_wave(T) != 0;
}

hipError_t zh_launch_scan_approx(const float *dX, uint32_t d, uint64_t n_rows, ZhApprox ap, const uint2 *dRowLeaf, uint32_t T,
                                 const uint32_t *dVisitBits, const uint4 *dNodeVisit, const ZhGroup *dGroups, uint32_t group, int metric,
                                 int mode, hipStream_t s) {
    if (!n_rows) return hipSuccess;
    if (ap.mfma) switch (d) {
    case 256: return launch_scan_mfma_d<256>(dX, n_rows, ap, dRowLeaf, T, dVisitBits, dNodeVisit, dGroups, group, s);
    case 384: return launch_scan_mfma_d<384>(dX, n_rows, ap, dRowLeaf, T, dVisitBits, dNodeVisit, dGroups, group, s);
    case 512: return launch_scan_mfma_d<512>(dX, n_rows, ap, dRowLeaf, T, dVisitBits, dNodeVisit, dGroups, group, s);
    case 768: return launch_scan_mfma_d<768>(dX, n_rows, ap, dRowLeaf, T, dVisitBits, dNodeVisit, dGroups, group, s);
    case 1024: return launch_scan_mfma_d<1024>(dX, n_rows, ap, dRowLeaf, T, dVisitBits, dNodeVisit, dGroups, group, s);
    default: return hipErrorInvalidValue;
    }
    switch (d) {
    case 128: {
        const uint32_t RW = zh_scan_rows_per_wave(T);
        uint64_t rows_per_launch = zh_sweep_rows_per_launch(128);
        rows_per_launch = rows_per_launch / (4 * RW) * (4 * RW);
        const float Kc = zh_approx_bound(metric, 128, 0);
        const int kinda = metric == ZH_COSINE ? (mode == ZH_COSINE_PARITY ? 2 : 1) : 0;
        for (uint64_t r = 0; r < n_rows; r += rows_per_launch) {
            const uint64_t r_end = r + rows_per_launch < n_rows ? r + rows_per_launch : n_rows;
            const uint64_t waves = (r_end - r + RW - 1) / RW, blocks = (waves + 3) / 4;
            if (blocks > 0x7FFFFFFFull) return hipErrorInvalidValue;
#define ZH_APX_LAUNCH(KA) \
            hipLaunchKernelGGL((scan_approx128_kernel<ZH_APX_G128, KA>), dim3((uint32_t)blocks), dim3(256), 0, s, dX, (const uint4 *)ap.Qh, ap.qmeta, dRowLeaf, T, RW, \
                               dVisitBits, dNodeVisit, dGroups, group, r, r_end, Kc, ap.iv)
            if (kinda == 0) ZH_APX_LAUNCH(0);
            else if (kinda == 1) ZH_APX_LAUNCH(1);
            else ZH_APX_LAUNCH(2);
#undef ZH_APX_LAUNCH
        }
        return hipGetLastError();
    }
    case 256: return launch_scan_approx_d<256, 4>(dX, n_rows, ap, dRowLeaf, T, dVisitBits, dNodeVisit, dGroups, group, metric, mode, s);
    case 384: return launch_scan_approx_d<384, 4>(dX, n_rows, ap, dRowLeaf, T, dVisitBits, dNodeVisit, dGroups, group, metric, mode, s);
    case 512: return launch_scan_approx_d<512, 2>(dX, n_rows, ap, dRowLeaf, T, dVisitBits, dNodeVisit, dGroups, group, metric, mode, s);
    case 768: return launch_scan_approx_d<768, ZH_APX_G768>(dX, n_rows, ap, dRowLeaf, T, dVisitBits, dNodeVisit, dGroups, group, metric, mode, s);
    case 1024: return launch_scan_approx_d<1024, 2>(dX, n_rows, ap, dRowLeaf, T, dVisitBits, dNodeVisit, dGroups, group, metric, mode, s);
    default: return hipErrorInvalidValue;
    }
}

#define ZH_APX_RADIX_SELECT(n, need_in, VAL, result)                                                        \
    {                                                                                                       \
        uint32_t prefix_ = 0, need_ = (need_in);                                                            \
        for (int sh_ = 24; sh_ >= 0; sh_ -= 8) {                                                            \
            __syncthreads();                                                                                \
            hist[tid] = 0;                                                                                  \
            __syncthreads();                                                                                \
            const uint32_t himask_ = sh_ == 24 ? 0u : (0xFFFFFFFFu << (sh_ + 8));                           \
            for (uint32_t i_ = tid; i_ < (n); i_ += 256) {                                                  \
                const uint32_t x_ = (VAL(i_));                                                              \
                if ((x_ & himask_) == prefix_) atomicAdd(&hist[(x_ >> sh_) & 255u], 1u);                    \
            }                                                                                               \
            __syncthreads();                                                                                \
            if (tid < 64) {                            \
                const uint32_t h0_ = hist[4 * tid], h1_ = hist[4 * tid + 1], h2_ = hist[4 * tid + 2], h3_ = hist[4 * tid + 3]; \
                const uint32_t ss_ = h0_ + h1_ + h2_ + h3_;                                                 \
                uint32_t inc_ = ss_;                                                                        \
                for (int m_ = 1; m_ < 64; m_ <<= 1) {                                                       \
                    const uint32_t t_ = __shfl_up(inc_, m_);                                                \
                    if ((int)tid >= m_) inc_ += t_;                                                         \
                }                                                                                           \
                const uint32_t exc_ = inc_ - ss_;                                                           \
                if (exc_ < need_ && need_ <= inc_) {                                                        \
                    uint32_t c_ = exc_, j_ = 4 * tid;                                                       \
                    if (need_ > c_ + h0_) { c_ += h0_; j_++;                                                \
                        if (need_ > c_ + h1_) { c_ += h1_; j_++;                                            \
                            if (need_ > c_ + h2_) { c_ += h2_; j_++; } } }                                  \
                    s_u[6] = j_; s_u[7] = c_;                                                               \
                }                                                                                           \
            }                                                                                               \
            __syncthreads();                                                                                \
            prefix_ |= s_u[6] << sh_;                                                                       \
            need_ -= s_u[7];                                                                                \
        }                                                                                                   \
        (result) = prefix_;                                                                                 \
    }

template <int KINDA>
__global__ __launch_bounds__(256) void select_tau_kernel(const ZhVisit *__restrict__ visits, uint64_t n_visits, uint32_t chunk,
                                                          uint32_t k_top, float Kc, ZhApprox ap) {
    __shared__ uint32_t hist[256];
    __shared__ uint32_t s_u[8];
    const uint32_t tid = threadIdx.x;
    const uint64_t base = (uint64_t)blockIdx.x * chunk;
    const uint32_t cnt = (uint32_t)(n_visits - base < chunk ? n_visits - base : chunk);
    for (uint32_t c = 0; c < cnt; c++) {
        const ZhVisit v = visits[base + c];
        if (v.take) {
            const float4 qm = ap.qmeta[v.b];
            uint64_t *__restrict__ raw = ap.iv + v.row_off;
            for (uint32_t i = tid; i < v.len; i += 256) {
                const uint64_t w = raw[i];
                raw[i] = approx_interval<KINDA>(__uint_as_float((uint32_t)w), __uint_as_float((uint32_t)(w >> 32)), qm, Kc, ap.row_rho, ap.rho_norm);
            }
            __syncthreads();
        }
        uint32_t tau = 0xFFFFFFFFu;
        if (v.take && v.take < v.len) {
            if (v.take < k_top) {
                if (tid == 0) {
                    const uint32_t slot = atomicAdd(&ap.ctl[0], 1u);
                    const uint32_t eb = atomicAdd(&ap.ctl[2], v.len);
                    if (slot >= ap.ex_cap) atomicOr(&ap.ctl[1], 4u);
                    else if ((uint64_t)eb + v.len > ap.ex_rows_cap) { atomicOr(&ap.ctl[1], 8u); ap.ex_visits[slot] = make_uint2(0xFFFFFFFFu, 0u); }
                    else ap.ex_visits[slot] = make_uint2((uint32_t)(base + c), eb);
                    ap.tauv[base + c] = 0u;
                }
                continue;
            }
            const uint64_t *__restrict__ kp = ap.iv + v.row_off;
#define ZH_APX_HI(i) ((uint32_t)(kp[i] >> 32))
            ZH_APX_RADIX_SELECT(v.len, v.take, ZH_APX_HI, tau);
#undef ZH_APX_HI
            if (tid == 0) atomicMin(&ap.qtau[v.b], tau);
        }
        if (tid == 0) ap.tauv[base + c] = tau;
    }
}

// ... 346 lines not shown
```

### zebra_amd/csrc/zh_device.h

```cpp
#pragma once
#include <type_traits>

#include "zh_internal.h"

#define WAVE 64

typedef float f32x16 __attribute__((ext_vector_type(16)));
typedef _Float16 f16x8 __attribute__((ext_vector_type(8)));
typedef float f32x4 __attribute__((ext_vector_type(4)));
typedef uint32_t u32x4 __attribute__((ext_vector_type(4)));

template <int CTRL>
__device__ __forceinline__ float dpp_mov(float x) {
    return __int_as_float(__builtin_amdgcn_update_dpp(0, __float_as_int(x), CTRL, 0xF, 0xF, false));
}
struct OpAdd { __device__ __forceinline__ static float f(float a, float b) { return a + b; } };
struct OpMax { __device__ __forceinline__ static float f(float a, float b) { return fmaxf(a, b); } };
template <class OP>
__device__ __forceinline__ float xor16(float s) {
    const auto r = __builtin_amdgcn_permlane16_swap(__float_as_uint(s), __float_as_uint(s), false, false);
    return OP::f(__uint_as_float(r[0]), __uint_as_float(r[1]));
}
template <class OP>
__device__ __forceinline__ float wave_butterfly(float s) {
    s = OP::f(s, dpp_mov<0xB1>(s));
    s = OP::f(s, dpp_mov<0x4E>(s));
    s = OP::f(s, dpp_mov<0x141>(s));
    s = OP::f(s, dpp_mov<0x140>(s));
    s = xor16<OP>(s);
    const auto r = __builtin_amdgcn_permlane32_swap(__float_as_uint(s), __float_as_uint(s), false, false);
    return OP::f(__uint_as_float(r[0]), __uint_as_float(r[1]));
}
__device__ __forceinline__ float wave_sum_canonical(float s) { return wave_butterfly<OpAdd>(s); }
__device__ __forceinline__ uint64_t f64_bits(double x) { return (uint64_t)__double_as_longlong(x); }

__device__ __forceinline__ uint64_t key_cosine(float ab, float a2, float b2, int mode) {
    double c;
    if (a2 == 0.0f && b2 == 0.0f) c = 0.0;
    else if (ab == 0.0f) c = 1.0;
    else {
        double r = 1.0 - (double)ab / sqrt((double)a2 * (double)b2);
        c = r > 0.0 ? r : 0.0;
    }
    return f64_bits(mode == ZH_COSINE_PARITY ? 1.0 - c : c);
}
__device__ __forceinline__ uint64_t key_l2(float l2sq, int metric) {
    return f64_bits(metric == ZH_L2SQ ? (double)l2sq : sqrt((double)l2sq));
}

enum { K_L2 = 0, K_COS = 1, K_MAX = 2, K_CANB = 3, K_BRAY = 4, K_ABS = 5, K_P3 = 6, K_P4 = 7, K_HAMM = 8, K_PP = 9 };

__host__ __device__ inline int zh_kind_of(int metric) {
    switch (metric) {
    case ZH_COSINE: return K_COS;
    case ZH_CHEBYSHEV: return K_MAX;
    case ZH_CANBERRA: return K_CANB;
    case ZH_BRAY_CURTIS: return K_BRAY;
    case ZH_MANHATTAN: return K_ABS;
    case ZH_L3: return K_P3;
    case ZH_L4: return K_P4;
    case ZH_HAMMING: return K_HAMM;
    case ZH_MINKOWSKI: case ZH_PNORM: return K_PP;
    default: return K_L2;
    }
}

template <int KIND, class F>
inline hipError_t zh_dispatch_dim(uint32_t d, F &f) {
    using K = std::integral_constant<int, KIND>;
    if constexpr (KIND == K_L2 || KIND == K_COS) {
        switch (d) {
        case 256: return f(K{}, std::integral_constant<int, 256>{});
        case 512: return f(K{}, std::integral_constant<int, 512>{});
        case 1024: return f(K{}, std::integral_constant<int, 1024>{});
        default: break;
        }
    }
    switch (d) {
    case 128: return f(K{}, std::integral_constant<int, 128>{});
    case 384: return f(K{}, std::integral_constant<int, 384>{});
    case 768: return f(K{}, std::integral_constant<int, 768>{});
    default: return f(K{}, std::integral_constant<int, 0>{});
    }
}
template <class F>
inline hipError_t zh_dispatch_kind_dim(int metric, uint32_t d, F f) {
    switch (zh_kind_of(metric)) {
    case K_COS: return zh_dispatch_dim<K_COS>(d, f);
    case K_MAX: return zh_dispatch_dim<K_MAX>(d, f);
    case K_CANB: return zh_dispatch_dim<K_CANB>(d, f);
    case K_BRAY: return zh_dispatch_dim<K_BRAY>(d, f);
    case K_ABS: return zh_dispatch_dim<K_ABS>(d, f);
    case K_P3: return zh_dispatch_dim<K_P3>(d, f);
    case K_P4: return zh_dispatch_dim<K_P4>(d, f);
    case K_HAMM: return zh_dispatch_dim<K_HAMM>(d, f);
    case K_PP: return zh_dispatch_dim<K_PP>(d, f);
    default: return zh_dispatch_dim<K_L2>(d, f);
    }
}

__device__ __forceinline__ float powi_f32(float a, int b) {
    const bool recip = b < 0;
    float r = 1.0f;
    for (;;) {
        if (b & 1) r *= a;
        b /= 2;
        if (b == 0) break;
        a *= a;
    }
    return recip ? 1.0f / r : r;
}

__device__ __forceinline__ double root_p(double s, int p) {
    if (!(s > 0.0) || s == (double)INFINITY || p == 1) return s;
    if (p == 2) return sqrt(s);
    uint64_t u = (uint64_t)__double_as_longlong(s);
    int e = (int)((u >> 52) & 0x7FF) - 1023;
// ... 679 lines not shown
```

### zebra_amd/csrc/zh_internal.h

```cpp
#pragma once
#include <hip/hip_runtime.h>
#include <stddef.h>
#include <stdint.h>

#include "../../include/zebra_hip.h"

int zh_set_error(int code, const char *fmt, ...) __attribute__((format(printf, 2, 3)));
double zh_index_visits_per_pair(zh_index *ix);
void zh_search_ctx_abandon(zh_search_ctx *c);
void zh_search_ctx_stream_ordered(zh_search_ctx *c);

struct ZhVisit {
    uint32_t b;
    uint32_t leaf_off;
    uint32_t len;
    uint32_t take;
    uint64_t row_off;
    uint64_t cand_off;
    uint32_t node;
    uint32_t pad;
};

#define ZH_GROUP_MAX 4
struct ZhGroup {
// ... 45 lines not shown
    uint32_t n_nodes, n_planes, n_trees;
    uint32_t group;
};

#if defined(__HIPCC__)
__device__ __forceinline__ bool zh_plane_above(const float *__restrict__ w, float c, const float *__restrict__ x,
                                               uint32_t d) {
    float acc = 0.0f;
    if ((d & 3u) == 0) {
        const float4 *w4 = reinterpret_cast<const float4 *>(w);
        const float4 *x4 = reinterpret_cast<const float4 *>(x);
        const uint32_t n4 = d / 4;
        uint32_t k = 0;
        for (; k + 8 <= n4; k += 8) {
            float4 a[8], b[8];
#pragma unroll
            for (int u = 0; u < 8; u++) { a[u] = w4[k + u]; b[u] = x4[k + u]; }
#pragma unroll
            for (int u = 0; u < 8; u++) {
                acc = __builtin_fmaf(a[u].x, b[u].x, acc);
                acc = __builtin_fmaf(a[u].y, b[u].y, acc);
                acc = __builtin_fmaf(a[u].z, b[u].z, acc);
                acc = __builtin_fmaf(a[u].w, b[u].w, acc);
            }
        }
        for (; k < n4; k++) {
            float4 a = w4[k], b = x4[k];
            acc = __builtin_fmaf(a.x, b.x, acc);
            acc = __builtin_fmaf(a.y, b.y, acc);
            acc = __builtin_fmaf(a.z, b.z, acc);
            acc = __builtin_fmaf(a.w, b.w, acc);
        }
    } else {
        for (uint32_t k = 0; k < d; k++) acc = __builtin_fmaf(w[k], x[k], acc);
    }
    return ((double)acc + (double)c) >= 0.0;
}
#endif

#define ZH_INLINE_VISITS 32

hipError_t zh_launch_hash_dense(const float *dQ, uint32_t B, const float *dPlanes, const float *dConsts,
                                uint32_t P, uint32_t d, uint32_t *dBits, uint32_t words_per_q, float *dDots,
                                hipStream_t s);
hipError_t zh_launch_qnorm(const float *dQ, uint32_t B, uint32_t d, float *dQQ, hipStream_t s);
hipError_t zh_launch_walk_count(ZhForestDev f, const float *dQ, uint32_t B, uint32_t d, int32_t n,
                                const uint32_t *dBits, uint32_t words_per_q, uint32_t P_dense, ZhPairCounts *dCounts,
                                ZhVisit *dInline, uint32_t *dLeafCount, ZhWalkLog log, hipStream_t s);
hipError_t zh_launch_walk_blocked(ZhForestDev f, ZhBlocksDev blk, uint32_t B, int32_t n, const uint32_t *dBits,
                                  uint32_t words_per_q, ZhPairCounts *dCounts, ZhVisit *dInline, uint32_t *dLeafCount,
                                  ZhWalkLog log, const uint32_t *dUnc , const float *dQ,
                                  uint32_t d, hipStream_t s);
hipError_t zh_launch_expand(ZhForestDev f, uint32_t B, const ZhPairCounts *dCounts, const ZhVisit *dInline,
                            const uint64_t *dRowBase, const uint64_t *dCandBase, const uint64_t *dVisitBase,
                            ZhVisit *dVisits, const uint32_t *dLeafCount, uint32_t *dLeafFill,
                            const uint32_t *dGroupBase, const uint64_t *dGroupRowBase, ZhGroup *dGroups,
                            uint64_t *dGroupRowOff, ZhWalkLog log, hipStream_t s);
hipError_t zh_launch_batch_init(uint32_t *dLeafCount, uint32_t *dLeafFill, uint32_t n_nodes, ZhLogCtl *dLogCtl,
                                ZhTotals *dTotals, hipStream_t s);
hipError_t zh_launch_leaf_scan(ZhForestDev f, const uint32_t *dLeafCount, uint32_t *dGroupBase,
                               uint64_t *dGroupRowBase, ZhTotals *dTotals, hipStream_t s);
hipError_t zh_launch_pair_scan(const ZhPairCounts *dCounts, uint32_t n_pairs, uint64_t *dRowBase,
                               uint64_t *dCandBase, uint64_t *dVisitBase, ZhTotals *dTotals, const ZhLogCtl *dLogCtl,
                               hipStream_t s);
hipError_t zh_launch_walk_emit(ZhForestDev f, const float *dQ, uint32_t B, uint32_t d, int32_t n,
                               const uint32_t *dBits, uint32_t words_per_q, uint32_t P_dense,
                               const ZhPairCounts *dCounts, const ZhVisit *dInline, const uint64_t *dRowBase,
                               const uint64_t *dCandBase, const uint64_t *dVisitBase, ZhVisit *dVisits,
                               const uint32_t *dLeafCount, uint32_t *dLeafFill, const uint32_t *dGroupBase,
                               const uint64_t *dGroupRowBase, ZhGroup *dGroups, uint64_t *dGroupRowOff, hipStream_t s);
hipError_t zh_launch_sweep(const float *dX, uint32_t d, const float *dQ, const float *dQQ, const ZhGroup *dGroups,
                           const uint64_t *dGroupRowOff, uint64_t n_groups, const uint32_t *dWaveGroup,
                           const uint32_t *dLeafIds, uint64_t R_grouped, int metric, int mode, uint64_t *dKeys,
                           hipStream_t s, const uint32_t *dRunIf = nullptr);
bool zh_sweep_has_predicate(uint32_t d, int metric);
hipError_t zh_launch_wave_groups(const ZhGroup *dGroups, const uint64_t *dGroupRowOff, uint64_t n_groups, uint32_t *dWaveGroup,
                                 hipStream_t s);
#define ZH_SCAN_NE 4
bool zh_scan_sweep_supported(uint32_t d, uint32_t T, int metric);
uint32_t zh_scan_rows_per_wave(uint32_t T);
hipError_t zh_launch_row_leaf(const int4 *dNodePack, const uint32_t *dNodeTree, uint32_t n_nodes, const uint32_t *dLeafIds,
                              uint32_t T, uint64_t n_rows, uint2 *dRowLeaf, hipStream_t s);
hipError_t zh_launch_node_visits(const uint32_t *dLeafCount, const uint32_t *dGroupBase, const ZhGroup *dGroups, uint32_t n_nodes,
                                 uint32_t *dBits, uint4 *dNodeVisit, hipStream_t s);
hipError_t zh_launch_scan_sweep(const float *dX, uint32_t d, uint64_t n_rows, const float *dQ, const float *dQQ,
                                const uint2 *dRowLeaf, uint32_t T, const uint32_t *dVisitBits, const uint4 *dNodeVisit,
                                const ZhGroup *dGroups, uint32_t group, int metric, int param, uint64_t *dKeys,
                                const uint32_t *dRunIf , hipStream_t s);
uint64_t zh_sweep_rows_per_launch(uint32_t d);
hipError_t zh_launch_select(const ZhVisit *dVisits, uint64_t n_visits, const uint32_t *dLeafIds,
                            const uint64_t *dKeys, uint64_t *dCandKeys, uint32_t *dCandIds, uint32_t max_leaf_len,
                            const uint32_t *dRunIf, hipStream_t s);
hipError_t zh_launch_final(const uint64_t *dCandBase, uint32_t B, uint32_t T, uint32_t k, const uint64_t *dCandKeys,
                           const uint32_t *dCandIds, uint64_t id_base, uint64_t *dOutIds, uint64_t *dOutKeys,
                           uint32_t *dOutCounts, const uint32_t *dRunIf, hipStream_t s);
hipError_t zh_launch_merge(uint32_t S, uint32_t B, uint32_t k, const uint64_t *dIds, const uint64_t *dKeys,
                           const uint32_t *dCounts, uint64_t *dOutIds, uint64_t *dOutKeys, uint32_t *dOutCounts,
                           uint64_t stride64, uint64_t stride32, hipStream_t s);
#define ZH_DISTANCE_SCRATCH_BYTES (sizeof(ZhGroup) + 16)
hipError_t zh_launch_distance_rows(const float *dX, uint64_t n, uint32_t d, const float *dq, int metric, int mode,
                                   uint64_t *dKeys, void *dScratch, hipStream_t s);

#define ZH_APX_CTL_WORDS 8
struct ZhApprox {
    const void *Qh;
    const float4 *qmeta;
    uint64_t *iv;
    uint32_t *list_lo, *list_hi, *list_id;
    uint32_t *qcount;
    uint32_t capq;
    uint32_t *tauv;
    uint32_t *qtau;
    uint2 *ex_visits;
    uint32_t ex_cap;
    uint64_t *ex_keys, *ex_ckeys;
    uint32_t *ex_cids;
    uint32_t ex_rows_cap;
    uint32_t *ctl;
    const void *row_half;
    const float2 *row_meta;
    float row_rho;
    float rho_norm;
    uint32_t mfma;
    uint32_t n_queries;
    uint64_t iv_cap;
    float nx_max;
};
uint32_t zh_approx_groups(uint32_t d);
bool zh_approx_pays(uint32_t d);
float zh_approx_bound(int metric, uint32_t d, int mfma);
bool zh_scan_mfma_supported(uint32_t d, uint32_t T);
hipError_t zh_launch_row_half(const float *dX, uint64_t row0, uint64_t n_rows, uint32_t d, void *dXh, float2 *dRowMeta, uint32_t *dRhoMax,
                              const uint32_t *dPerm , uint64_t perm_rows, hipStream_t s);
hipError_t zh_launch_scan_order(const uint2 *dRowLeaf, uint64_t n_rows, uint32_t T, uint32_t n_keys, uint32_t *dPerm, hipStream_t s);
hipError_t zh_launch_order_agreement(const uint2 *dRowLeaf, const uint32_t *dPerm, uint64_t n_rows, uint32_t T, unsigned long long *dOut, hipStream_t s);
hipError_t zh_launch_permute_row_leaf(const uint2 *dRowLeaf, const uint32_t *dPerm, uint64_t perm_rows, uint64_t n_rows, uint32_t T, uint2 *dOut, hipStream_t s);
bool zh_scan_approx_supported(uint32_t d, uint32_t T, int metric);
hipError_t zh_launch_qhalf(const float *dQ, uint32_t B, uint32_t d, void *dQh, float4 *dQmeta, int layout, hipStream_t s);
hipError_t zh_launch_absmax(const float *dX, uint64_t n, uint32_t *dOut, hipStream_t s);
hipError_t zh_launch_row_half128(const float *dX, uint64_t row0, uint64_t n_rows, float sigma, void *dXh, uint32_t *dRhoMax, hipStream_t s);
hipError_t zh_launch_sweep128h(const void *dXh, const void *dQh, float inv, const ZhGroup *dGroups, const uint64_t *dGroupRowOff, uint64_t n_groups,
                               const uint32_t *dWaveGroup, const uint32_t *dLeafIds, uint64_t R_grouped, uint64_t *dIv, hipStream_t s,
                               const ZhApprox *fuse = nullptr, int fuse_kinda = 0, uint32_t k_top = 0, float Kc = 0.f, bool byte_rows = false);
uint64_t zh_sweep128h_rows_per_launch(bool lean, bool byte_rows);
hipError_t zh_launch_row_byte128(const float *dX, uint64_t row0, uint64_t n_rows, void *dXb, uint32_t *dNotBytes, hipStream_t s);
hipError_t zh_launch_exact_register(const ZhVisit *dVisits, uint64_t n_visits, uint32_t k, ZhApprox ap, hipStream_t s);
hipError_t zh_launch_scan_approx(const float *dX, uint32_t d, uint64_t n_rows, ZhApprox ap, const uint2 *dRowLeaf, uint32_t T,
                                 const uint32_t *dVisitBits, const uint4 *dNodeVisit, const ZhGroup *dGroups, uint32_t group, int metric,
                                 int mode, hipStream_t s);
hipError_t zh_launch_select_interval(const ZhVisit *dVisits, uint64_t n_visits, uint32_t k, const uint32_t *dLeafIds, ZhApprox ap,
                                     int metric, int mode, uint32_t d, hipStream_t s);
hipError_t zh_launch_final_interval(const ZhVisit *dVisits, const float *dX, uint32_t d, const float *dQ, const float *dQQ, uint32_t B,
                                    uint32_t k, const uint32_t *dLeafIds, int metric, int mode, uint64_t id_base, ZhApprox ap,
                                    uint64_t *dOutIds, uint64_t *dOutKeys, uint32_t *dOutCounts, uint32_t max_leaf_len, hipStream_t s);

hipError_t zh_launch_exact_score(const float *dX, uint32_t d, const uint32_t *dLive, uint64_t p0, uint32_t nr, const float *dQ,
                                 const float *dQQ, uint32_t B, int metric, int param, uint64_t *dKeys, uint64_t ld, hipStream_t s);
hipError_t zh_launch_exact_visits(uint32_t B, uint32_t nsub, uint32_t nr, uint32_t L, uint32_t k, uint64_t p0, uint64_t ld, ZhVisit *dVisits,
                                  uint64_t *dCandBase, hipStream_t s);
struct ZhExact2 {
    const void *Xh; const float2 *rowMeta; const uint32_t *perm; uint64_t perm_rows; const uint32_t *liveBits;
    const void *Qh; const float4 *qmeta; uint32_t B; float Kc, rho;
    uint32_t *tau, *cnt, *lid, *llo, *lhi; uint32_t cap; uint32_t *over;
};
bool zh_exact_mfma_supported(uint32_t d, int metric);
hipError_t zh_launch_exact_mfma(uint32_t d, int metric, int mode, const ZhExact2 &e, uint64_t p_begin, uint64_t p_end, hipStream_t s,
                                bool filtered = false);
hipError_t zh_launch_exact_prune(const ZhExact2 &e, uint32_t k, uint32_t *dScratch, hipStream_t s);
hipError_t zh_launch_exact_survivor_keys(const float *dX, uint32_t d, const float *dQ, const float *dQQ, int metric, int mode, const ZhExact2 &e,
                                         uint64_t *dCKeys, uint32_t *dCIds, hipStream_t s);
hipError_t zh_launch_exact_empty(uint32_t B, uint32_t k, uint64_t *dIds, uint64_t *dKeys, uint32_t *dCounts, hipStream_t s);

#define ZH_FILTER_BLOCK_ROWS 8192u
hipError_t zh_launch_filter_and(const uint32_t *dFilter, uint64_t n_bits, const uint32_t *dLiveBits, uint64_t n_rows, uint32_t *dOut,
                                uint32_t *dBlockCount, uint32_t *dBlockExcl, uint32_t *dScanTmp, uint32_t *dTiles, hipStream_t s);
hipError_t zh_launch_filter_permute(const uint32_t *dBits, const uint32_t *dPerm, uint64_t perm_rows, uint64_t n_rows, uint32_t *dOut,
                                    uint32_t *dBlockCount, uint32_t *dBlockExcl, uint32_t *dScanTmp, uint32_t *dTiles, hipStream_t s);
hipError_t zh_launch_filter_list(const uint32_t *dBits, uint64_t n_rows, const uint32_t *dBlockExcl, uint32_t *dList, hipStream_t s);

hipError_t zh_launch_range_collect(const uint64_t *dKeys, uint64_t ld, const uint32_t *dLive, uint64_t p0, uint32_t nr, uint32_t B,
                                   const uint64_t *dMaxKeys, uint32_t *dCnt, unsigned long long *dHitCtr, uint64_t *dPoolV, uint64_t *dPoolK,
                                   uint64_t pool_cap, hipStream_t s);
hipError_t zh_launch_range_tau(const uint64_t *dMaxKeys, uint32_t B, int metric, int mode, uint32_t *dTau, hipStream_t s);
hipError_t zh_launch_range_mfma(uint32_t d, int metric, int mode, const ZhExact2 &e, uint64_t p_begin, uint64_t p_end, uint64_t *dCand, uint64_t cand_cap,
                                unsigned long long *dCandCtr, hipStream_t s);
hipError_t zh_launch_range_survivors(const float *dX, uint32_t d, const float *dQ, const float *dQQ, int metric, int mode, const uint64_t *dCand,
                                     const unsigned long long *dCandCtr, uint64_t cand_cap, const uint64_t *dMaxKeys, uint32_t *dCnt,
                                     unsigned long long *dHitCtr, uint64_t *dPoolV, uint64_t *dPoolK, uint64_t pool_cap, hipStream_t s);
hipError_t zh_launch_range_offsets(const uint32_t *dCnt, uint32_t B, uint64_t base, uint64_t *dOff, hipStream_t s);
hipError_t zh_launch_pool_sort(uint64_t *dV[2], uint64_t *dK[2], uint64_t n, uint64_t lo_values, uint64_t hi_values, bool skip_high, void *dTmp,
                               size_t *tmp_bytes, const uint64_t **v_out, const uint64_t **k_out, hipStream_t s);
hipError_t zh_launch_range_sort(uint64_t *dV[2], uint64_t *dK[2], uint64_t n, uint64_t n_rows, uint32_t B, void *dTmp, size_t *tmp_bytes, uint64_t id_base,
                                uint64_t *dOutIds, uint64_t *dOutKeys, hipStream_t s);

#define ZH_JOIN_CHUNK 64u
#define ZH_JOIN_PANEL_ROWS 16384u
hipError_t zh_launch_join_gather(const float *dX, uint32_t d, const uint32_t *dRows, uint32_t B, float *dQ, hipStream_t s);
hipError_t zh_launch_pair_collect(const uint64_t *dKeys, uint64_t ld, const uint32_t *dLive, uint64_t p0, uint32_t nr, const uint32_t *dQRows, uint32_t B,
                                  bool upper, uint64_t max_key, unsigned long long *dHitCtr, uint64_t *dPoolV, uint64_t *dPoolK, uint64_t pool_cap,
                                  hipStream_t s);
hipError_t zh_launch_join_prep(const float2 *dRowMeta, const uint32_t *dPerm, uint64_t perm_rows, const uint32_t *dLiveBits, uint64_t n_rows, float rho,
                               float4 *dQm, uint32_t *dCid, hipStream_t s);
uint64_t zh_join_geometry(uint64_t T, uint64_t tileA0, uint64_t tileA1, uint32_t *first);
hipError_t zh_launch_join_mfma(uint32_t d, int metric, int mode, const void *dXh, const float2 *dRowMeta, const float4 *dQm, const uint32_t *dCid,
                               uint64_t n_rows, uint64_t tileA0, const uint32_t *dFirst, uint32_t n_ab, uint32_t blocks, float Kc, float rho,
                               const uint32_t *dTau, uint64_t *dCand, uint64_t cand_cap, unsigned long long *dCandCtr, hipStream_t s);
hipError_t zh_launch_pair_survivors(const float *dXA, const float *dXB, uint32_t d, int metric, int mode, const uint64_t *dCand,
                                    const unsigned long long *dCandCtr, uint64_t cand_cap, const uint32_t *dLeafOf, uint32_t T, uint32_t t, uint64_t max_key,
                                    unsigned long long *dHitCtr, unsigned long long *dKeyed, uint64_t *dPoolV, uint64_t *dPoolK, uint64_t pool_cap,
                                    hipStream_t s);
hipError_t zh_launch_join_panel_rows(const uint32_t *dCid, uint64_t p_begin, uint64_t p_end, uint32_t *dList, unsigned long long *dCount, hipStream_t s);
hipError_t zh_launch_pair_sort(uint64_t *dV[2], uint64_t *dK[2], uint64_t n, uint64_t n_rows_a, uint64_t n_rows_b, void *dTmp, size_t *tmp_bytes,
                               uint64_t id_base_a, uint64_t id_base_b, uint64_t *dOutA, uint64_t *dOutB, uint64_t *dOutKeys, hipStream_t s);

uint64_t zh_xjoin_geometry(uint64_t TA, uint64_t TB, uint64_t tileA0, uint64_t tileA1, uint32_t *n_ab, uint32_t *blocks);
hipError_t zh_launch_xjoin_mfma(uint32_t d, int metric, int mode, const void *dXhA, const float2 *dRowMetaA, const uint32_t *dCidA, uint64_t n_rows_a,
                                const void *dXhB, const float4 *dQmB, const uint32_t *dCidB, uint64_t n_rows_b, uint64_t tileA0, uint64_t tileA1, float Kc,
                                float rhoA, const uint32_t *dTau, uint64_t *dCand, uint64_t cand_cap, unsigned long long *dCandCtr, hipStream_t s);

#define ZH_DEBUG_WALK_ROWS 1024u
hipError_t zh_launch_walk_debug(uint32_t d, int metric, int mode, const void *dXhA, const float2 *dRowMetaA, const uint32_t *dCidA, uint64_t n_rows_a,
                                const void *dXhB, const float4 *dQmB, const uint32_t *dCidB, uint64_t n_rows_b, uint64_t p0, uint64_t p1, float Kc, float rhoA,
                                zh_debug_walk_pair *dOut, uint64_t cap, hipStream_t s);

#define ZH_KNN_PANEL_ROWS 1024u
#define ZH_KNN_CHUNK 64u
static_assert(ZH_KNN_PANEL_ROWS % 64 == 0, "a held block is four tiles of 16 lines");
hipError_t zh_launch_knn_rowpos(const uint32_t *dCid, uint64_t n_pos, uint32_t *dPos, hipStream_t s);
hipError_t zh_launch_knn_panel(uint32_t d, const void *dXh, const float2 *dRowMeta, const uint32_t *dPos, const uint32_t *dRows, uint32_t B, void *dA,
                               float2 *dPMeta, uint32_t *dPid, hipStream_t s);
uint32_t zh_knn_chunk(uint64_t tiles, uint32_t n_ab);
// ... 211 lines not shown
```

### zebra_amd/csrc/zh_search.hip

```cpp
#include <cstdlib>

#include "zh_internal.h"
#include "zh_device.h"

#define HD_KT 32
#define HD_PITCH 65

template <bool WRITE_DOTS>
__global__ __launch_bounds__(256) void hash_dense_kernel(const float *__restrict__ Q, uint32_t B,
                                                          const float *__restrict__ W,
                                                          const float *__restrict__ C, uint32_t P, uint32_t d,
                                                          uint32_t *__restrict__ bits, uint32_t wpq,
                                                          float *__restrict__ dots) {
    __shared__ float Qs[HD_KT][HD_PITCH];
    __shared__ float Ws[HD_KT][HD_PITCH];
    const uint32_t tid = threadIdx.x, lane = tid & 63, wv = tid >> 6;
    const uint32_t wr = wv >> 1, wc = wv & 1;
    const uint32_t p0 = blockIdx.x * 64, b0 = blockIdx.y * 64;
    f32x16 acc;
#pragma unroll
    for (int i = 0; i < 16; i++) acc[i] = 0.0f;
    const bool vec4 = (d & 3u) == 0;
    auto fetch = [&](uint32_t k0, float4 *qv, float4 *wv) {
#pragma unroll
// ... 1447 lines not shown
    }
    return hipGetLastError();
}

template <int KIND>
static hipError_t launch_sweep_kind(const SweepArgs &a) {
#define ZH_SWEEP_CASE(DD) case DD: return launch_sweep_k<DD, KIND>(a)
    if constexpr (KIND == K_L2 || KIND == K_COS) {
        switch (a.d) {
            ZH_SWEEP_CASE(64);
            ZH_SWEEP_CASE(256);
            ZH_SWEEP_CASE(512);
            ZH_SWEEP_CASE(1024);
            ZH_SWEEP_CASE(1536);
        default: break;
        }
    }
    switch (a.d) {
        ZH_SWEEP_CASE(128);
        ZH_SWEEP_CASE(384);
        ZH_SWEEP_CASE(768);
    default: return launch_sweep_k<0, KIND>(a);
    }
#undef ZH_SWEEP_CASE
}

bool zh_sweep_has_predicate(uint32_t d, int metric) {
    const int kind = zh_kind_of(metric);
    return d == 128 && (kind == K_L2 || kind == K_COS);
}

uint32_t zh_group_size(uint32_t dim) {
    return 4u;
}

hipError_t zh_launch_sweep(const float *dX, uint32_t d, const float *dQ, const float *dQQ, const ZhGroup *dGroups,
                           const uint64_t *dGroupRowOff, uint64_t n_groups, const uint32_t *dWaveGroup,
                           const uint32_t *dLeafIds, uint64_t R_grouped, int metric, int param, uint64_t *dKeys,
                           hipStream_t s, const uint32_t *dRunIf) {
    if (R_grouped == 0 || n_groups == 0) return hipSuccess;
    if (dRunIf && !zh_sweep_has_predicate(d, metric)) return hipErrorInvalidValue;
    const SweepArgs a{dX, d, dQ, dQQ, dGroups, dGroupRowOff, n_groups, dWaveGroup, dLeafIds, R_grouped, metric, param, dKeys, s, dRunIf};
#define ZH_KIND_CASE(K) case K: return launch_sweep_kind<K>(a)
    switch (zh_kind_of(metric)) {
        ZH_KIND_CASE(K_COS);
        ZH_KIND_CASE(K_MAX);
        ZH_KIND_CASE(K_CANB);
        ZH_KIND_CASE(K_BRAY);
        ZH_KIND_CASE(K_ABS);
        ZH_KIND_CASE(K_P3);
        ZH_KIND_CASE(K_P4);
        ZH_KIND_CASE(K_HAMM);
        ZH_KIND_CASE(K_PP);
    default: return launch_sweep_kind<K_L2>(a);
    }
#undef ZH_KIND_CASE
}

__global__ __launch_bounds__(64) void row_leaf_kernel(const int4 *__restrict__ node_pack, const uint32_t *__restrict__ node_tree,
                                                       const uint32_t *__restrict__ leaf_ids, uint32_t T, uint64_t n_rows,
                                                       uint32_t node0, uint2 *__restrict__ rowLeaf) {
    const uint32_t node = node0 + blockIdx.x;
    const int4 rec = node_pack[node];
    if (rec.x >= 0) return;
    const uint32_t t = node_tree[node];
    if (t >= T) return;
    const uint32_t off = (uint32_t)rec.y, len = (uint32_t)rec.z;
    for (uint32_t i = threadIdx.x; i < len; i += 64) {
        const uint32_t r = leaf_ids[(size_t)off + i];
        if (r < n_rows) rowLeaf[(size_t)r * T + t] = make_uint2(node, i);
    }
}
hipError_t zh_launch_row_leaf(const int4 *dNodePack, const uint32_t *dNodeTree, uint32_t n_nodes, const uint32_t *dLeafIds,
                              uint32_t T, uint64_t n_rows, uint2 *dRowLeaf, hipStream_t s) {
    hipError_t e = hipMemsetAsync(dRowLeaf, 0xFF, n_rows * T * sizeof(uint2), s);
    if (e != hipSuccess) return e;
    for (uint32_t n0 = 0; n0 < n_nodes; n0 += (1u << 22)) {
        const uint32_t nb = n_nodes - n0 < (1u << 22) ? n_nodes - n0 : (1u << 22);
        hipLaunchKernelGGL(row_leaf_kernel, dim3(nb), dim3(64), 0, s, dNodePack, dNodeTree, dLeafIds, T, n_rows, n0, dRowLeaf);
    }
    return hipGetLastError();
}

__global__ __launch_bounds__(256) void node_visit_kernel(const uint32_t *__restrict__ leafCount, const uint32_t *__restrict__ groupBase,
                                                          const ZhGroup *__restrict__ groups, uint32_t n_nodes,
                                                          uint32_t *__restrict__ bits, uint4 *__restrict__ nodeVisit) {
    const uint32_t w = blockIdx.x * blockDim.x + threadIdx.x;
    const uint32_t n0 = w * 32;
    if (n0 >= n_nodes) return;
    uint32_t word = 0;
    for (uint32_t i = 0; i < 32 && n0 + i < n_nodes; i++) {
        const uint32_t c = leafCount[n0 + i];
        if (c) {
            word |= 1u << i;
            const uint32_t gb = groupBase[n0 + i];
            const uint64_t k0 = groups[gb].key_off[0];
            nodeVisit[n0 + i] = make_uint4(c | ((uint32_t)(k0 >> 32) << 28), gb, groups[gb].b[0], (uint32_t)k0);
        }
    }
    bits[w] = word;
}
hipError_t zh_launch_node_visits(const uint32_t *dLeafCount, const uint32_t *dGroupBase, const ZhGroup *dGroups, uint32_t n_nodes,
                                 uint32_t *dBits, uint4 *dNodeVisit, hipStream_t s) {
    const uint32_t words = (n_nodes + 31) / 32;
    if (!words) return hipSuccess;
    hipLaunchKernelGGL(node_visit_kernel, dim3((words + 255) / 256), dim3(256), 0, s, dLeafCount, dGroupBase, dGroups, n_nodes, dBits, dNodeVisit);
    return hipGetLastError();
}

#define ZH_SCAN_CAP 256
template <int D, int KIND>
__global__ __launch_bounds__(256) void scan_sweep_kernel(const float *__restrict__ X, const float *__restrict__ Q,
                                                          const float *__restrict__ QQ, const uint2 *__restrict__ rowLeaf,
                                                          uint32_t T, uint32_t RW, const uint32_t *__restrict__ visitBits,
                                                          const uint4 *__restrict__ nodeVisit,
                                                          const ZhGroup *__restrict__ groups, uint32_t GRP, uint64_t row_begin,
                                                          uint64_t row_end, int metric, int param,
                                                          uint64_t *__restrict__ keys, const uint32_t *__restrict__ run_if) {
    constexpr int NV = RowVec<D>::NV;
    __shared__ uint4 pair_list[4][ZH_SCAN_CAP];
    if (run_if && *run_if == 0) return;
    const uint32_t lane = threadIdx.x & 63;
    const uint32_t wid = (uint32_t)__builtin_amdgcn_readfirstlane((int)(threadIdx.x >> 6));
    const uint64_t wave = (uint64_t)blockIdx.x * (blockDim.x >> 6) + wid;
    const uint64_t r0 = row_begin + wave * RW;
    if (r0 >= row_end) return;
    const uint32_t nr = (uint32_t)(row_end - r0 < RW ? row_end - r0 : RW);
    const uint32_t n_ent = nr * T;
    const uint2 *__restrict__ ent = rowLeaf + (size_t)r0 * T;
    uint32_t eGb[ZH_SCAN_NE], eWithin[ZH_SCAN_NE], eC[ZH_SCAN_NE], off[ZH_SCAN_NE], eB0[ZH_SCAN_NE];
    uint64_t eK0[ZH_SCAN_NE];
    uint32_t P = 0;
#pragma unroll
    for (int j = 0; j < ZH_SCAN_NE; j++) {
        const uint32_t e = lane + 64u * j;
        eGb[j] = 0; eWithin[j] = 0; eC[j] = 0; eB0[j] = 0; eK0[j] = 0;
        if (e < n_ent) {
            const unsigned long long rlw = __builtin_nontemporal_load(reinterpret_cast<const unsigned long long *>(ent + e));
            const uint2 rl = make_uint2((uint32_t)rlw, (uint32_t)(rlw >> 32));
            eWithin[j] = rl.y;
            if (rl.x != 0xFFFFFFFFu && ((visitBits[rl.x >> 5] >> (rl.x & 31)) & 1u)) {
                const uint4 nv = nodeVisit[rl.x];
                eC[j] = nv.x & 0x0FFFFFFFu; eGb[j] = nv.y; eB0[j] = nv.z;
                eK0[j] = ((uint64_t)(nv.x >> 28) << 32) | nv.w;
            }
        }
        uint32_t incl = eC[j];
#pragma unroll
        for (int o = 1; o < 64; o <<= 1) {
            const uint32_t t = __shfl_up(incl, o);
            if (lane >= (uint32_t)o) incl += t;
        }
        off[j] = P + incl - eC[j];
        P += (uint32_t)__builtin_amdgcn_readlane((int)incl, 63);
    }
    if (P == 0) return;
    float my_s0 = 0.f, my_s1 = 0.f;
    uint64_t my_slot = 0;
    uint32_t my_b = 0, npend = 0;
    auto flush = [&]() {
        if (lane < npend) {
            uint64_t key;
            if constexpr (KIND == K_COS) key = key_cosine(my_s0, my_s1, QQ[my_b], param);
            else if constexpr (KIND == K_L2) key = key_l2(my_s0, metric);
            else key = key_of(metric, param, my_s0, my_s1, 0.f);
            __builtin_nontemporal_store(key, keys + my_slot);
        }
        npend = 0;
    };
    auto row_norm = [&](const float4 *v) {
        float4 c = make_float4(0.f, 0.f, 0.f, 0.f);
#pragma unroll
        for (int j = 0; j < NV; j++) {
            const bool act = (j < RowVec<D>::NJ) || (lane < (uint32_t)RowVec<D>::REM4);
            if (act) sq4(v[j], c);
        }
        return wave_sum_canonical((c.x + c.y) + (c.z + c.w));
    };
    auto score = [&](const float4 *v, float a2, uint32_t b, uint64_t slot, const float4 *q) {
        float s0 = 0.f, s1 = 0.f;
        row_pair_sums<D, KIND>(v, q, lane, param, s0, s1);
        if (lane == npend) { my_s0 = s0; my_s1 = KIND == K_COS ? a2 : s1; my_slot = slot; my_b = b; }
        if (++npend == 64) flush();
    };
    if (P <= ZH_SCAN_CAP) {
        uint4 *list = pair_list[wid];
        uint32_t mrows = 0;
#pragma unroll
        for (int j = 0; j < ZH_SCAN_NE; j++) {
            const uint32_t c = eC[j];
            if (c) {
                const uint32_t rl = (lane + 64u * j) / T, gb = eGb[j];
                mrows |= 1u << rl;
                {
                    const uint64_t slot = eK0[j] + eWithin[j];
                    list[off[j]] = make_uint4(rl, eB0[j], (uint32_t)slot, (uint32_t)(slot >> 32));
                }
                for (uint32_t sidx = 1; sidx < c; sidx++) {
                    const ZhGroup *g = groups + gb + sidx / GRP;
                    const uint64_t slot = g->key_off[sidx % GRP] + eWithin[j];
                    list[off[j] + sidx] = make_uint4(rl, g->b[sidx % GRP], (uint32_t)slot, (uint32_t)(slot >> 32));
                }
            }
        }
        uint32_t rowmask = 0;
#pragma unroll
        for (int bit = 0; bit < 16; bit++) rowmask |= (__ballot((mrows >> bit) & 1u) != 0 ? 1u : 0u) << bit;
        __builtin_amdgcn_fence(__ATOMIC_RELEASE, "wavefront");
        __builtin_amdgcn_wave_barrier();
        auto rd = [&](uint32_t p) {
            const uint4 r = list[p];
            return make_uint4((uint32_t)__builtin_amdgcn_readfirstlane((int)r.x), (uint32_t)__builtin_amdgcn_readfirstlane((int)r.y),
                              (uint32_t)__builtin_amdgcn_readfirstlane((int)r.z), (uint32_t)__builtin_amdgcn_readfirstlane((int)r.w));
        };
        float4 qa[NV], qb[NV], qc[NV], qd[NV];
        uint32_t p = 0;
        auto segment = [&](const float4 *vr, float a2, uint32_t rowid) {
            for (;;) {
                const uint4 ra = rd(p < P ? p : P - 1), rb = rd(p + 1 < P ? p + 1 : P - 1), rc = rd(p + 2 < P ? p + 2 : P - 1),
                            rdd = rd(p + 3 < P ? p + 3 : P - 1);
                const bool ha = p < P && ra.x == rowid, hb = ha && p + 1 < P && rb.x == rowid, hc = hb && p + 2 < P && rc.x == rowid,
                           hd = hc && p + 3 < P && rdd.x == rowid;
                if (!ha) return;
                load_row<D>(Q + (size_t)ra.y * D, lane, qa);
                if (hb) load_row<D>(Q + (size_t)rb.y * D, lane, qb);
                if (hc) load_row<D>(Q + (size_t)rc.y * D, lane, qc);
                if (hd) load_row<D>(Q + (size_t)rdd.y * D, lane, qd);
                score(vr, a2, ra.y, ((uint64_t)ra.w << 32) | ra.z, qa);
                if (hb) score(vr, a2, rb.y, ((uint64_t)rb.w << 32) | rb.z, qb);
                if (hc) score(vr, a2, rc.y, ((uint64_t)rc.w << 32) | rc.z, qc);
                if (hd) score(vr, a2, rdd.y, ((uint64_t)rdd.w << 32) | rdd.z, qd);
                p += hd ? 4u : (hc ? 3u : (hb ? 2u : 1u));
                if (!hd) return;
            }
        };
        while (rowmask) {
            uint32_t rid[4];
#pragma unroll
            for (int r = 0; r < 4; r++) {
                rid[r] = rowmask ? (uint32_t)__builtin_ctz(rowmask) : 0xFFFFFFFFu;
                rowmask &= rowmask - 1;
            }
            float4 v0[NV], v1[NV], v2[NV], v3[NV];
            load_row<D, true>(X + (size_t)(r0 + rid[0]) * D, lane, v0);
            if (rid[1] != 0xFFFFFFFFu) load_row<D, true>(X + (size_t)(r0 + rid[1]) * D, lane, v1);
            if (rid[2] != 0xFFFFFFFFu) load_row<D, true>(X + (size_t)(r0 + rid[2]) * D, lane, v2);
            if (rid[3] != 0xFFFFFFFFu) load_row<D, true>(X + (size_t)(r0 + rid[3]) * D, lane, v3);
            segment(v0, KIND == K_COS ? row_norm(v0) : 0.f, rid[0]);
            if (rid[1] != 0xFFFFFFFFu) segment(v1, KIND == K_COS ? row_norm(v1) : 0.f, rid[1]);
            if (rid[2] != 0xFFFFFFFFu) segment(v2, KIND == K_COS ? row_norm(v2) : 0.f, rid[2]);
            if (rid[3] != 0xFFFFFFFFu) segment(v3, KIND == K_COS ? row_norm(v3) : 0.f, rid[3]);
        }
    } else {
        float4 v[NV];
        float a2 = 0.f;
        uint32_t cur = 0xFFFFFFFFu;
#pragma unroll
        for (int j = 0; j < ZH_SCAN_NE; j++) {
            unsigned long long m = __ballot(eC[j] != 0);
            while (m) {
                const int l = __builtin_ctzll(m);
                m &= m - 1;
                const uint32_t c = (uint32_t)__builtin_amdgcn_readlane((int)eC[j], l);
                const uint32_t gb = (uint32_t)__builtin_amdgcn_readlane((int)eGb[j], l);
                const uint32_t w = (uint32_t)__builtin_amdgcn_readlane((int)eWithin[j], l);
                const uint32_t rl = ((uint32_t)l + 64u * j) / T;
                if (rl != cur) {
                    cur = rl;
                    load_row<D, true>(X + (size_t)(r0 + rl) * D, lane, v);
                    if (KIND == K_COS) a2 = row_norm(v);
                }
                for (uint32_t sidx = 0; sidx < c; sidx++) {
                    const ZhGroup *g = groups + gb + sidx / GRP;
                    const uint32_t b = g->b[sidx % GRP];
                    float4 q[NV];
                    load_row<D>(Q + (size_t)b * D, lane, q);
                    score(v, a2, b, g->key_off[sidx % GRP] + w, q);
                }
            }
        }
    }
    flush();
}

#define ZH_SCAN128_CAP 192
template <int KIND>
__global__ __launch_bounds__(256) void scan128_sweep_kernel(const float *__restrict__ X, const float *__restrict__ Q,
                                                             const float *__restrict__ QQ, const uint2 *__restrict__ rowLeaf,
                                                             uint32_t T, uint32_t RW, const uint32_t *__restrict__ visitBits,
                                                             const uint4 *__restrict__ nodeVisit,
                                                             const ZhGroup *__restrict__ groups, uint32_t GRP, uint64_t row_begin,
                                                             uint64_t row_end, int metric, int param,
                                                             uint64_t *__restrict__ keys, const uint32_t *__restrict__ run_if) {
    static_assert(KIND == K_L2 || KIND == K_COS, "the paired scan covers the two simsimd-path kinds");
    if (run_if && *run_if == 0) return;
    __shared__ uint4 pair_list[4][ZH_SCAN128_CAP];
    __shared__ float4 row_lds[4][4][32];
    __shared__ uint32_t row_start[4][20];
    const uint32_t lane = threadIdx.x & 63, hl = lane & 31, half = lane >> 5;
    const uint32_t wid = (uint32_t)__builtin_amdgcn_readfirstlane((int)(threadIdx.x >> 6));
    const uint64_t wave = (uint64_t)blockIdx.x * (blockDim.x >> 6) + wid;
    const uint64_t r0 = row_begin + wave * RW;
    if (r0 >= row_end) return;
    const uint32_t nr = (uint32_t)(row_end - r0 < RW ? row_end - r0 : RW);
    const uint32_t n_ent = nr * T;
    const uint2 *__restrict__ ent = rowLeaf + (size_t)r0 * T;
    const float4 *__restrict__ X4 = reinterpret_cast<const float4 *>(X);
    const float4 *__restrict__ Q4 = reinterpret_cast<const float4 *>(Q);
    uint32_t eGb[ZH_SCAN_NE], eWithin[ZH_SCAN_NE], eC[ZH_SCAN_NE], off[ZH_SCAN_NE], eB0[ZH_SCAN_NE];
    uint64_t eK0[ZH_SCAN_NE];
    uint32_t P = 0;
#pragma unroll
    for (int j = 0; j < ZH_SCAN_NE; j++) {
        const uint32_t e = lane + 64u * j;
        eGb[j] = 0; eWithin[j] = 0; eC[j] = 0; eB0[j] = 0; eK0[j] = 0;
        if (e < n_ent) {
            const unsigned long long rlw = __builtin_nontemporal_load(reinterpret_cast<const unsigned long long *>(ent + e));
            const uint2 rl = make_uint2((uint32_t)rlw, (uint32_t)(rlw >> 32));
            eWithin[j] = rl.y;
            if (rl.x != 0xFFFFFFFFu && ((visitBits[rl.x >> 5] >> (rl.x & 31)) & 1u)) {
                const uint4 nv = nodeVisit[rl.x];
                eC[j] = nv.x & 0x0FFFFFFFu; eGb[j] = nv.y; eB0[j] = nv.z;
                eK0[j] = ((uint64_t)(nv.x >> 28) << 32) | nv.w;
            }
        }
        uint32_t incl = eC[j];
#pragma unroll
        for (int o = 1; o < 64; o <<= 1) {
            const uint32_t t = __shfl_up(incl, o);
            if (lane >= (uint32_t)o) incl += t;
        }
        off[j] = P + incl - eC[j];
        P += (uint32_t)__builtin_amdgcn_readlane((int)incl, 63);
    }
    if (P == 0) return;
    float my_s0 = 0.f, my_s1 = 0.f;
    uint64_t my_slot = ~0ull;
    uint32_t my_b = 0;
    if (P <= ZH_SCAN128_CAP) {
        uint4 *list = pair_list[wid];
        uint32_t *rstart = row_start[wid];
#pragma unroll
        for (int j = 0; j < ZH_SCAN_NE; j++) {
            const uint32_t e = lane + 64u * j, c = eC[j];
            if (e < n_ent && e % T == 0) rstart[e / T] = off[j];
            if (c) {
                const uint32_t rl = e / T, gb = eGb[j];
                {
                    const uint64_t slot = eK0[j] + eWithin[j];
                    list[off[j]] = make_uint4(rl, eB0[j], (uint32_t)slot, (uint32_t)(slot >> 32));
                }
                for (uint32_t sidx = 1; sidx < c; sidx++) {
                    const ZhGroup *g = groups + gb + sidx / GRP;
                    const uint64_t slot = g->key_off[sidx % GRP] + eWithin[j];
                    list[off[j] + sidx] = make_uint4(rl, g->b[sidx % GRP], (uint32_t)slot, (uint32_t)(slot >> 32));
                }
            }
        }
        if (lane == 0) rstart[nr] = P;
        __builtin_amdgcn_fence(__ATOMIC_RELEASE, "wavefront");
        __builtin_amdgcn_wave_barrier();
        uint32_t npl = 0;
        auto flush = [&]() {
            if (hl < npl && my_slot != ~0ull)
                __builtin_nontemporal_store(key_of(metric, param, my_s0, my_s1, KIND == K_COS ? QQ[my_b] : 0.f), keys + my_slot);
            npl = 0;
        };
        for (uint32_t rb = 0; rb < nr; rb += 4) {
            const uint32_t re = rb + 4 < nr ? rb + 4 : nr;
            const uint32_t pa = (uint32_t)__builtin_amdgcn_readfirstlane((int)rstart[rb]);
            const uint32_t pb = (uint32_t)__builtin_amdgcn_readfirstlane((int)rstart[re]);
            if (pa == pb) continue;
            {
                const uint32_t ra = rb + half, rc = rb + 2 + half;
                float4 va = make_float4(0.f, 0.f, 0.f, 0.f), vc = va;
                if (ra < re) va = ld16<true>(X4 + (size_t)(r0 + ra) * 32 + hl);
                if (rc < re) vc = ld16<true>(X4 + (size_t)(r0 + rc) * 32 + hl);
                row_lds[wid][half][hl] = va;
                row_lds[wid][2 + half][hl] = vc;
            }
            __builtin_amdgcn_fence(__ATOMIC_RELEASE, "wavefront");
            __builtin_amdgcn_wave_barrier();
            uint32_t pi = pa + half;
            uint4 rec = list[pi < pb ? pi : pb - 1];
            float4 qc = Q4[(size_t)rec.y * 32 + hl];
            for (uint32_t p = pa; p < pb; p += 2) {
                const bool valid = p + half < pb;
                const uint32_t pn = p + 2 + half;
                const uint4 recn = list[pn < pb ? pn : pb - 1];
                const float4 qn = Q4[(size_t)recn.y * 32 + hl];
                const float4 v = row_lds[wid][rec.x - rb][hl];
                float a2 = 0.f;
                if (KIND == K_COS) {
                    float4 c;
                    c.x = __builtin_fmaf(v.x, v.x, 0.f); c.y = __builtin_fmaf(v.y, v.y, 0.f);
                    c.z = __builtin_fmaf(v.z, v.z, 0.f); c.w = __builtin_fmaf(v.w, v.w, 0.f);
                    a2 = half_sum_canonical((c.x + c.y) + (c.z + c.w));
                }
                float4 a = make_float4(0.f, 0.f, 0.f, 0.f), e1 = a;
                acc4<KIND>(v, qc, a, e1, param);
                const float s0 = half_sum_canonical((a.x + a.y) + (a.z + a.w));
                if (hl == npl) {
                    my_s0 = s0; my_s1 = a2; my_b = rec.y;
                    my_slot = valid ? (((uint64_t)rec.w << 32) | rec.z) : ~0ull;
                }
                if (++npl == 32) flush();
                rec = recn; qc = qn;
            }
            __builtin_amdgcn_wave_barrier();
        }
        flush();
        return;
    }
    uint32_t npend = 0;
    auto flush1 = [&]() {
        if (lane < npend) __builtin_nontemporal_store(key_of(metric, param, my_s0, my_s1, KIND == K_COS ? QQ[my_b] : 0.f), keys + my_slot);
        npend = 0;
    };
    float4 v[1];
    float a2 = 0.f;
    uint32_t cur = 0xFFFFFFFFu;
#pragma unroll
    for (int j = 0; j < ZH_SCAN_NE; j++) {
        unsigned long long m = __ballot(eC[j] != 0);
        while (m) {
            const int l = __builtin_ctzll(m);
            m &= m - 1;
            const uint32_t c = (uint32_t)__builtin_amdgcn_readlane((int)eC[j], l);
            const uint32_t gb = (uint32_t)__builtin_amdgcn_readlane((int)eGb[j], l);
            const uint32_t w = (uint32_t)__builtin_amdgcn_readlane((int)eWithin[j], l);
            const uint32_t rl = ((uint32_t)l + 64u * j) / T;
            if (rl != cur) {
                cur = rl;
                load_row<128, true>(X + (size_t)(r0 + rl) * 128, lane, v);
                if (KIND == K_COS) {
                    float4 c4 = make_float4(0.f, 0.f, 0.f, 0.f);
                    if (lane < 32) {
                        c4.x = __builtin_fmaf(v[0].x, v[0].x, 0.f); c4.y = __builtin_fmaf(v[0].y, v[0].y, 0.f);
                        c4.z = __builtin_fmaf(v[0].z, v[0].z, 0.f); c4.w = __builtin_fmaf(v[0].w, v[0].w, 0.f);
                    }
                    a2 = wave_sum_canonical((c4.x + c4.y) + (c4.z + c4.w));
                }
            }
            for (uint32_t sidx = 0; sidx < c; sidx++) {
                const ZhGroup *g = groups + gb + sidx / GRP;
                const uint32_t b = g->b[sidx % GRP];
                float4 q[1];
                load_row<128>(Q + (size_t)b * 128, lane, q);
                float s0 = 0.f, s1 = 0.f;
                row_pair_sums<128, KIND>(v, q, lane, param, s0, s1);
                if (lane == npend) { my_s0 = s0; my_s1 = KIND == K_COS ? a2 : s1; my_slot = g->key_off[sidx % GRP] + w; my_b = b; }
                if (++npend == 64) flush1();
            }
        }
    }
    flush1();
}

uint32_t zh_scan_rows_per_wave(uint32_t T) {
    if (T == 0 || T > 64u * ZH_SCAN_NE) return 0;
    const uint32_t rw = 64u * ZH_SCAN_NE / T;
    return rw > 16 ? 16 : rw;
}
bool zh_scan_sweep_supported(uint32_t d, uint32_t T, int metric) {
    if (!zh_scan_rows_per_wave(T)) return false;
    const int kind = zh_kind_of(metric);
    if (d == 128 || d == 384 || d == 768) return true;
    if (kind != K_L2 && kind != K_COS) return false;
    switch (d) { case 64: case 256: case 512: case 1024: case 1536: return true; default: return false; }
}

template <int D, int KIND>
static hipError_t launch_scan_dk(const float *dX, uint64_t n_rows, const float *dQ, const float *dQQ, const uint2 *dRowLeaf,
                                 uint32_t T, const uint32_t *dVisitBits, const uint4 *dNodeVisit, const ZhGroup *dGroups,
                                 uint32_t group, int metric, int param, uint64_t *dKeys, const uint32_t *dRunIf, hipStream_t s) {
    const uint32_t RW = zh_scan_rows_per_wave(T);
    uint64_t rows_per_launch = zh_sweep_rows_per_launch(D);
    rows_per_launch = rows_per_launch / (4 * RW) * (4 * RW);
    for (uint64_t r = 0; r < n_rows; r += rows_per_launch) {
        const uint64_t r_end = r + rows_per_launch < n_rows ? r + rows_per_launch : n_rows;
        const uint64_t waves = (r_end - r + RW - 1) / RW, blocks = (waves + 3) / 4;
        if (blocks > 0x7FFFFFFFull) return hipErrorInvalidValue;
        if constexpr (D == 128 && (KIND == K_L2 || KIND == K_COS))
            hipLaunchKernelGGL((scan128_sweep_kernel<KIND>), dim3((uint32_t)blocks), dim3(256), 0, s, dX, dQ, dQQ, dRowLeaf, T, RW,
                               dVisitBits, dNodeVisit, dGroups, group, r, r_end, metric, param, dKeys, dRunIf);
        else
            hipLaunchKernelGGL((scan_sweep_kernel<D, KIND>), dim3((uint32_t)blocks), dim3(256), 0, s, dX, dQ, dQQ, dRowLeaf, T, RW,
                               dVisitBits, dNodeVisit, dGroups, group, r, r_end, metric, param, dKeys, dRunIf);
    }
    return hipGetLastError();
}
template <int KIND>
static hipError_t launch_scan_k(const float *dX, uint32_t d, uint64_t n_rows, const float *dQ, const float *dQQ,
                                const uint2 *dRowLeaf, uint32_t T, const uint32_t *dVisitBits, const uint4 *dNodeVisit,
                                const ZhGroup *dGroups, uint32_t group, int metric, int param, uint64_t *dKeys, const uint32_t *dRunIf, hipStream_t s) {
#define ZH_SCAN_CASE(DD) \
    case DD: return launch_scan_dk<DD, KIND>(dX, n_rows, dQ, dQQ, dRowLeaf, T, dVisitBits, dNodeVisit, dGroups, group, metric, param, dKeys, dRunIf, s)
    if constexpr (KIND == K_L2 || KIND == K_COS) {
        switch (d) {
            ZH_SCAN_CASE(64); ZH_SCAN_CASE(256); ZH_SCAN_CASE(512); ZH_SCAN_CASE(1024); ZH_SCAN_CASE(1536);
        default: break;
        }
    }
    switch (d) {
        ZH_SCAN_CASE(128); ZH_SCAN_CASE(384); ZH_SCAN_CASE(768);
    default: return hipErrorInvalidValue;
    }
#undef ZH_SCAN_CASE
}
hipError_t zh_launch_scan_sweep(const float *dX, uint32_t d, uint64_t n_rows, const float *dQ, const float *dQQ,
                                const uint2 *dRowLeaf, uint32_t T, const uint32_t *dVisitBits, const uint4 *dNodeVisit,
                                const ZhGroup *dGroups, uint32_t group, int metric, int param, uint64_t *dKeys, const uint32_t *dRunIf,
                                hipStream_t s) {
    if (!n_rows) return hipSuccess;
#define ZH_KIND_CASE(K) \
    case K: return launch_scan_k<K>(dX, d, n_rows, dQ, dQQ, dRowLeaf, T, dVisitBits, dNodeVisit, dGroups, group, metric, param, dKeys, dRunIf, s)
    switch (zh_kind_of(metric)) {
        ZH_KIND_CASE(K_COS);
        ZH_KIND_CASE(K_MAX);
        ZH_KIND_CASE(K_CANB);
        ZH_KIND_CASE(K_BRAY);
        ZH_KIND_CASE(K_ABS);
        ZH_KIND_CASE(K_P3);
        ZH_KIND_CASE(K_P4);
        ZH_KIND_CASE(K_HAMM);
        ZH_KIND_CASE(K_PP);
    default: return launch_scan_k<K_L2>(dX, d, n_rows, dQ, dQQ, dRowLeaf, T, dVisitBits, dNodeVisit, dGroups, group, metric, param, dKeys, dRunIf, s);
    }
#undef ZH_KIND_CASE
}

__global__ void one_group_kernel(ZhGroup *g, uint64_t *rowoff, uint64_t n) {
    g->leaf_off = 0; g->len = (uint32_t)n; g->gsize = 1; g->take4 = 0;
    for (int m = 0; m < ZH_GROUP_MAX; m++) { g->b[m] = 0; g->key_off[m] = 0; }
    rowoff[0] = 0;
}
hipError_t zh_launch_distance_rows(const float *dX, uint64_t n, uint32_t d, const float *dq, int metric, int mode,
                                   uint64_t *dKeys, void *dScratch, hipStream_t s) {
    if (!n) return hipSuccess;
    ZhGroup *dg = reinterpret_cast<ZhGroup *>(dScratch);
    uint64_t *dro = reinterpret_cast<uint64_t *>(dg + 1);
    float *dqq = reinterpret_cast<float *>(dro + 1);
    hipLaunchKernelGGL(one_group_kernel, dim3(1), dim3(1), 0, s, dg, dro, n);
    hipError_t e = zh_launch_qnorm(dq, 1, d, dqq, s);
    if (e == hipSuccess) e = zh_launch_sweep(dX, d, dq, dqq, dg, dro, 1, nullptr, nullptr, n, metric, mode, dKeys, s);
    return e;
}

#define SEL_GROUP_LEN 16
template <int CAP>
__global__ __launch_bounds__(256) void select_kernel(const ZhVisit *__restrict__ visits, uint64_t n_visits, uint32_t chunk,
                                                      const uint32_t *__restrict__ leaf_ids,
                                                      const uint64_t *__restrict__ keys,
                                                      uint64_t *__restrict__ cand_keys,
                                                      uint32_t *__restrict__ cand_ids, const uint32_t *__restrict__ run_if) {
    __shared__ uint64_t sk[CAP];
    __shared__ __attribute__((aligned(16))) uint32_t si[CAP < 2048 ? 2048 : CAP];
    __shared__ uint32_t s_u32[8];
    __shared__ uint32_t s_list[256], s_small[256], s_nlist, s_nsmall;
    const uint32_t tid = threadIdx.x;
    if (run_if && *run_if == 0) return;
    const uint64_t base = (uint64_t)blockIdx.x * chunk;
    const uint32_t cnt = (uint32_t)(n_visits - base < chunk ? n_visits - base : chunk);
    if (tid == 0) { s_nlist = 0; s_nsmall = 0; }
    __syncthreads();
    if (tid < cnt) {
        const uint32_t len = visits[base + tid].len, take = visits[base + tid].take;
        if (take > 0) {
            if (len <= SEL_GROUP_LEN) s_small[atomicAdd(&s_nsmall, 1u)] = tid;
            else s_list[atomicAdd(&s_nlist, 1u)] = tid;
        }
    }
    __syncthreads();
    {
        const uint32_t ns = s_nsmall, g = tid >> 4, l = tid & 15;
        for (uint32_t i = g; i < ns; i += 16) {
            const ZhVisit v = visits[base + s_small[i]];
            const bool on = l < v.len;
            const uint64_t k = on ? keys[v.row_off + l] : ~0ull;
            const uint32_t id = on ? leaf_ids[(size_t)v.leaf_off + l] : ~0u;
            uint32_t rank = l;
            if (v.take < v.len) {
                rank = 0;
#pragma unroll
                for (int j = 0; j < SEL_GROUP_LEN; j++) {
                    const uint64_t kj = __shfl(k, j, SEL_GROUP_LEN);
                    const uint32_t ij = __shfl(id, j, SEL_GROUP_LEN);
                    rank += (kj < k || (kj == k && ij < id)) ? 1u : 0u;
                }
            }
            if (on && rank < v.take) {
                cand_keys[v.cand_off + rank] = k;
                cand_ids[v.cand_off + rank] = id;
            }
        }
    }
    const uint32_t nl = s_nlist;
    for (uint32_t li = 0; li < nl; li++) {
        const ZhVisit v = visits[base + s_list[li]];
        if (v.take >= v.len) {
            for (uint32_t i = tid; i < v.len; i += 256) {
                cand_keys[v.cand_off + i] = keys[v.row_off + i];
                cand_ids[v.cand_off + i] = leaf_ids[(size_t)v.leaf_off + i];
            }
            continue;
        }
        bool need_slow = false;
        if (v.len <= CAP) select_fast<true>(v, leaf_ids, keys, cand_keys, cand_ids, sk, si, s_u32, need_slow);
        else select_fast<false>(v, leaf_ids, keys, cand_keys, cand_ids, sk, si, s_u32, need_slow);
        if (need_slow) {
// ... 528 lines not shown
```

Baseline: 201,100.

## Compact per-node visit records into rank-indexed array with bitmap directory

New measurement: 203,000 (median of 5 runs). Within noise of the previous version (+1.0%).

```diff
diff --git a/zebra_amd/csrc/zh_api.hip b/zebra_amd/csrc/zh_api.hip
--- a/zebra_amd/csrc/zh_api.hip
+++ b/zebra_amd/csrc/zh_api.hip
@@ -97,7 +97,7 @@
 struct zh_search_ctx {
     zh_index *ix = nullptr;
     DevBuf wQQ, wBits, wCounts, wInline, wRowBase, wCandBase, wVisitBase, wTotals, wVisits, wKeys, wCandKeys, wCandIds,
-        wLeafCount, wLeafFill, wGroupBase, wGroupRowBase, wGroups, wGroupRowOff, wWaveGroup, wVisitBits, wNodeVisit, wScore, wJunkBits, wZeros, wQnorm, wQpad, wFixList, wLogPool, wLogHead, wLogCtl,
+        wLeafCount, wLeafFill, wGroupBase, wGroupRowBase, wGroups, wGroupRowOff, wWaveGroup, wVisitDir, wVisitRec, wScore, wJunkBits, wZeros, wQnorm, wQpad, wFixList, wLogPool, wLogHead, wLogCtl,
         wPfRows, wPfCounts, wPfKeys, wPfIds, wPfAmb, wPfCtl, wUnc, wQh, wQmeta, wApList, wApCount, wApEx, wApExKeys, wApCtl, wRaw;
     ZhApprox dbg_ap{};
     bool dbg_valid = false, dbg_raw = false;
@@ -134,7 +134,7 @@
     hipStream_t sv_heavy = nullptr;
     std::vector<DevBuf *> all_bufs() {
         return {&wQQ, &wBits, &wCounts, &wInline, &wRowBase, &wCandBase, &wVisitBase, &wTotals, &wVisits, &wKeys,
-                &wCandKeys, &wCandIds, &wLeafCount, &wLeafFill, &wGroupBase, &wGroupRowBase, &wGroups, &wGroupRowOff, &wWaveGroup, &wVisitBits, &wNodeVisit, &wScore, &wJunkBits, &wZeros, &wQnorm, &wQpad, &wFixList,
+                &wCandKeys, &wCandIds, &wLeafCount, &wLeafFill, &wGroupBase, &wGroupRowBase, &wGroups, &wGroupRowOff, &wWaveGroup, &wVisitDir, &wVisitRec, &wScore, &wJunkBits, &wZeros, &wQnorm, &wQpad, &wFixList,
                 &wLogPool, &wLogHead, &wLogCtl, &wQwin, &wOutWin, &wPfRows, &wPfCounts, &wPfKeys, &wPfIds, &wPfAmb, &wPfCtl, &wUnc,
                 &wQh, &wQmeta, &wApList, &wApCount, &wApEx, &wApExKeys, &wApCtl, &wRaw};
     }
@@ -2465,12 +2465,14 @@
         if (!ix->row_leaf.current(ix) && !ix->row_leaf.failed && (rc = build_row_leaf(ix))) return rc;
         if (!ix->row_leaf.current(ix)) c->scan = false;
     }
+    uint32_t visit_recs = 0;
     if (c->scan) {
         const size_t nn = std::max<uint32_t>(ix->n_nodes, 1);
-        if ((rc = c->wVisitBits.ensure((nn + 31) / 32 * 4))) return rc;
-        if ((rc = c->wNodeVisit.ensure(nn * sizeof(uint4)))) return rc;
+        visit_recs = (uint32_t)std::max<uint64_t>(std::min<uint64_t>(nn, tot.visits), 1);
+        if ((rc = c->wVisitDir.ensure((nn + 31) / 32 * sizeof(uint2)))) return rc;
+        if ((rc = c->wVisitRec.ensure((size_t)visit_recs * sizeof(uint4)))) return rc;
         HIPCHK(zh_launch_node_visits(c->wLeafCount.as<uint32_t>(), c->wGroupBase.as<uint32_t>(), c->wGroups.as<ZhGroup>(), ix->n_nodes,
-                                     c->wVisitBits.as<uint32_t>(), c->wNodeVisit.as<uint4>(), s));
+                                     c->wVisitDir.as<uint2>(), c->wVisitRec.as<uint4>(), visit_recs, s));
     }
     if (!c->scan)
         HIPCHK(zh_launch_wave_groups(c->wGroups.as<ZhGroup>(), c->wGroupRowOff.as<uint64_t>(), tot.groups, c->wWaveGroup.as<uint32_t>(), s));
@@ -2520,7 +2522,7 @@
         ap.ex_visits = c->wApEx.as<uint2>(); ap.ex_cap = ex_cap;
         ap.ex_keys = c->wApExKeys.as<uint64_t>(); ap.ex_ckeys = ap.ex_keys + ex_rows; ap.ex_cids = reinterpret_cast<uint32_t *>(ap.ex_ckeys + ex_rows);
         ap.ex_rows_cap = ex_rows; ap.ctl = c->wApCtl.as<uint32_t>();
-        ap.n_queries = (uint32_t)B; ap.iv_cap = tot.rows;
+        ap.n_queries = (uint32_t)B; ap.iv_cap = tot.rows; ap.visit_recs = visit_recs;
         ap.mfma = mfma ? 1u : 0u; ap.row_half = mfma ? ix->half.tiles.p : nullptr; ap.row_meta = mfma ? ix->half.meta.as<float2>() : nullptr;
         ap.row_rho = mfma ? ix->half.rho.load() : 0.f;
         if (c->approx_leaf) { ap.mfma = 2u; ap.row_rho = ap.rho_norm = c->approx_bytes ? 0.f : ix->half128.rho.load(); }
@@ -2547,11 +2549,11 @@
                                    tot.groups, c->wWaveGroup.as<uint32_t>(), f.leaf_ids, tot.group_rows, c->wKeys.as<uint64_t>(), hs,
                                    c->approx_fused ? &ap : nullptr, kinda, (uint32_t)k, zh_approx_bound(c->metric, d, 2), c->approx_bytes));
     else if (c->approx)
-        HIPCHK(zh_launch_scan_approx(ix->X.as<float>(), d, ix->n_rows, ap, mfma ? scan_row_leaf : ix->row_leaf.table.as<uint2>(), T, c->wVisitBits.as<uint32_t>(),
-                                     c->wNodeVisit.as<uint4>(), c->wGroups.as<ZhGroup>(), f.group, c->metric, c->mode, hs));
+        HIPCHK(zh_launch_scan_approx(ix->X.as<float>(), d, ix->n_rows, ap, mfma ? scan_row_leaf : ix->row_leaf.table.as<uint2>(), T, c->wVisitDir.as<uint2>(),
+                                     c->wVisitRec.as<uint4>(), c->wGroups.as<ZhGroup>(), f.group, c->metric, c->mode, hs));
     else if (c->scan)
         HIPCHK(zh_launch_scan_sweep(ix->X.as<float>(), d, ix->n_rows, c->dQ, c->wQQ.as<float>(), ix->row_leaf.table.as<uint2>(), T,
-                                    c->wVisitBits.as<uint32_t>(), c->wNodeVisit.as<uint4>(), c->wGroups.as<ZhGroup>(), f.group,
+                                    c->wVisitDir.as<uint2>(), c->wVisitRec.as<uint4>(), c->wGroups.as<ZhGroup>(), f.group,
                                     c->metric, c->mode, c->wKeys.as<uint64_t>(), nullptr, hs));
     else
         HIPCHK(zh_launch_sweep(ix->X.as<float>(), d, c->dQ, c->wQQ.as<float>(), c->wGroups.as<ZhGroup>(),
@@ -2582,7 +2584,7 @@
                                    c->wWaveGroup.as<uint32_t>(), f.leaf_ids, tot.group_rows, c->metric, c->mode, c->wKeys.as<uint64_t>(), s, run_if));
         else
             HIPCHK(zh_launch_scan_sweep(ix->X.as<float>(), d, ix->n_rows, c->dQ, c->wQQ.as<float>(), ix->row_leaf.table.as<uint2>(), T,
-                                        c->wVisitBits.as<uint32_t>(), c->wNodeVisit.as<uint4>(), c->wGroups.as<ZhGroup>(), f.group,
+                                        c->wVisitDir.as<uint2>(), c->wVisitRec.as<uint4>(), c->wGroups.as<ZhGroup>(), f.group,
                                         c->metric, c->mode, c->wKeys.as<uint64_t>(), run_if, s));
     }
     HIPCHK(zh_launch_select(c->wVisits.as<ZhVisit>(), tot.visits, f.leaf_ids, c->wKeys.as<uint64_t>(),
diff --git a/zebra_amd/csrc/zh_approx.hip b/zebra_amd/csrc/zh_approx.hip
--- a/zebra_amd/csrc/zh_approx.hip
+++ b/zebra_amd/csrc/zh_approx.hip
@@ -101,29 +101,37 @@
 }
 
 
+#ifdef ZH_SCAN_GUARD
+#define ZH_GUARD(cond, bit) ((cond) ? true : (atomicOr(guard, (bit)), false))
+#else
+#define ZH_GUARD(cond, bit) true
+#endif
+
 __device__ __forceinline__ uint32_t scan_phase1(uint32_t lane, uint32_t n_ent, const uint2 *__restrict__ ent,
-                                                const uint32_t *__restrict__ visitBits, const uint4 *__restrict__ nodeVisit,
-                                                uint32_t *eGb, uint32_t *eWithin, uint32_t *eC, uint32_t *off, uint32_t *eB0, uint64_t *eK0) {
+                                                const uint2 *__restrict__ visitDir, const uint4 *__restrict__ visitRec,
+                                                uint32_t *eGb, uint32_t *eWithin, uint32_t *eC, uint32_t *off, uint32_t *eB0, uint64_t *eK0,
+                                                uint32_t n_rec = 0, uint32_t *guard = nullptr) {
     unsigned long long rlw[ZH_SCAN_NE];
 #pragma unroll
     for (int j = 0; j < ZH_SCAN_NE; j++) {
         const uint32_t e = lane + 64u * j;
         rlw[j] = __builtin_nontemporal_load(reinterpret_cast<const unsigned long long *>(ent + (e < n_ent ? e : 0)));
     }
-    uint32_t word[ZH_SCAN_NE];
+    uint2 word[ZH_SCAN_NE];
     bool in[ZH_SCAN_NE];
 #pragma unroll
     for (int j = 0; j < ZH_SCAN_NE; j++) {
         const uint32_t node = (uint32_t)rlw[j];
         in[j] = lane + 64u * j < n_ent && node != 0xFFFFFFFFu;
-        word[j] = visitBits[in[j] ? node >> 5 : 0];
+        word[j] = visitDir[in[j] ? node >> 5 : 0];
     }
     uint4 nv[ZH_SCAN_NE];
 #pragma unroll
     for (int j = 0; j < ZH_SCAN_NE; j++) {
         const uint32_t node = (uint32_t)rlw[j];
-        in[j] = in[j] && ((word[j] >> (node & 31)) & 1u);
-        nv[j] = nodeVisit[in[j] ? node : 0];
+        const uint32_t rank = visit_dir_rank(word[j], node);
+        in[j] = in[j] && visit_dir_has(word[j], node) && (guard == nullptr || ZH_GUARD(rank < n_rec, 256u));
+        nv[j] = visitRec[in[j] ? rank : 0];
     }
     uint32_t P = 0;
 #pragma unroll
@@ -158,8 +166,8 @@
 #endif
 void scan_approx_kernel(const float *__restrict__ X, const uint4 *__restrict__ Qh,
                                                            const float4 *__restrict__ qmeta, const uint2 *__restrict__ rowLeaf,
-                                                           uint32_t T, uint32_t RW, const uint32_t *__restrict__ visitBits,
-                                                           const uint4 *__restrict__ nodeVisit, const ZhGroup *__restrict__ groups,
+                                                           uint32_t T, uint32_t RW, const uint2 *__restrict__ visitDir,
+                                                           const uint4 *__restrict__ visitRec, const ZhGroup *__restrict__ groups,
                                                            uint32_t GRP, uint64_t row_begin, uint64_t row_end, float Kc,
                                                            uint64_t *__restrict__ iv) {
     constexpr int LG = 64 / G, NH = D * G / 512, NR = 2 * NH;
@@ -177,7 +185,7 @@
     const uint2 *__restrict__ ent = rowLeaf + (size_t)r0 * T;
     uint32_t eGb[ZH_SCAN_NE], eWithin[ZH_SCAN_NE], eC[ZH_SCAN_NE], off[ZH_SCAN_NE], eB0[ZH_SCAN_NE];
     uint64_t eK0[ZH_SCAN_NE];
-    const uint32_t P = scan_phase1(lane, n_ent, ent, visitBits, nodeVisit, eGb, eWithin, eC, off, eB0, eK0);
+    const uint32_t P = scan_phase1(lane, n_ent, ent, visitDir, visitRec, eGb, eWithin, eC, off, eB0, eK0);
     if (P == 0) return;
     const float4 *__restrict__ X4 = reinterpret_cast<const float4 *>(X);
     float my_s = 0.f, my_a2 = 0.f;
@@ -414,11 +422,6 @@
 #ifndef ZH_MFMA_CL
 #define ZH_MFMA_CL 0
 #endif
-#ifdef ZH_SCAN_GUARD
-#define ZH_GUARD(cond, bit) ((cond) ? true : (atomicOr(guard, (bit)), false))
-#else
-#define ZH_GUARD(cond, bit) true
-#endif
 #ifdef ZH_SCAN_PROF
 __device__ unsigned long long zh_scan_prof_buf[16];
 extern "C" __attribute__((visibility("default"))) int zh_debug_scan_prof(uint64_t *out, uint32_t words, int reset) {
@@ -437,11 +440,11 @@
 __global__ __launch_bounds__(256) __attribute__((amdgpu_waves_per_eu(D > 768 ? 2 : ZH_MFMA_WAVES, D > 768 ? 2 : ZH_MFMA_WAVES)))
 void scan_mfma_kernel(const u32x4 *__restrict__ Xh, const float *__restrict__ Xf, const float2 *__restrict__ rowMeta,
                                                          const uint4 *__restrict__ Qh, const uint2 *__restrict__ rowLeaf, uint32_t T,
-                                                         uint32_t RW, const uint32_t *__restrict__ visitBits,
-                                                         const uint4 *__restrict__ nodeVisit, const ZhGroup *__restrict__ groups,
+                                                         uint32_t RW, const uint2 *__restrict__ visitDir,
+                                                         const uint4 *__restrict__ visitRec, const ZhGroup *__restrict__ groups,
                                                          uint32_t GRP, uint64_t row_begin, uint64_t row_end, uint64_t *__restrict__ iv,
                                                          uint32_t *__restrict__ colStats ,
-                                                         uint32_t nq, uint64_t iv_cap, uint32_t *__restrict__ guard) {
+                                                         uint32_t nq, uint64_t iv_cap, uint32_t n_rec, uint32_t *__restrict__ guard) {
     constexpr int NS = D / 32;
     constexpr int NL = D / 64;
     constexpr int CL = ZH_MFMA_CL ? ZH_MFMA_CL : (NL % 4 == 0 ? 2 : 3);
@@ -464,7 +467,7 @@
     const uint2 *__restrict__ ent = rowLeaf + (size_t)r0 * T;
     uint32_t eGb[ZH_SCAN_NE], eWithin[ZH_SCAN_NE], eC[ZH_SCAN_NE], off[ZH_SCAN_NE], eB0[ZH_SCAN_NE];
     uint64_t eK0[ZH_SCAN_NE];
-    const uint32_t P = scan_phase1(lane, n_ent, ent, visitBits, nodeVisit, eGb, eWithin, eC, off, eB0, eK0);
+    const uint32_t P = scan_phase1(lane, n_ent, ent, visitDir, visitRec, eGb, eWithin, eC, off, eB0, eK0, n_rec, guard);
     if (P == 0) return;
     SP(const uint64_t sp1 = clock64();)
     uint64_t *list = pair_list[wid];
@@ -732,7 +735,7 @@
 
 template <int D>
 static hipError_t launch_scan_mfma_d(const float *dX, uint64_t n_rows, const ZhApprox &ap, const uint2 *dRowLeaf, uint32_t T,
-                                     const uint32_t *dVisitBits, const uint4 *dNodeVisit, const ZhGroup *dGroups, uint32_t group, hipStream_t s) {
+                                     const uint2 *dVisitDir, const uint4 *dVisitRec, const ZhGroup *dGroups, uint32_t group, hipStream_t s) {
     const uint32_t RW = zh_scan_rows_per_wave(T);
     uint64_t rows_per_launch = zh_sweep_rows_per_launch(D);
     rows_per_launch = rows_per_launch / (4 * RW) * (4 * RW);
@@ -742,10 +745,10 @@
         if (blocks > 0x7FFFFFFFull) return hipErrorInvalidValue;
         if (ap.row_half)
             hipLaunchKernelGGL((scan_mfma_kernel<D, false>), dim3((uint32_t)blocks), dim3(256), 0, s, (const u32x4 *)ap.row_half, dX, ap.row_meta, (const uint4 *)ap.Qh, dRowLeaf, T, RW,
-                               dVisitBits, dNodeVisit, dGroups, group, r, r_end, ap.iv, ap.ctl + 5, ap.n_queries, ap.iv_cap, ap.ctl + 7);
+                               dVisitDir, dVisitRec, dGroups, group, r, r_end, ap.iv, ap.ctl + 5, ap.n_queries, ap.iv_cap, ap.visit_recs, ap.ctl + 7);
         else
             hipLaunchKernelGGL((scan_mfma_kernel<D, true>), dim3((uint32_t)blocks), dim3(256), 0, s, (const u32x4 *)nullptr, dX, ap.row_meta, (const uint4 *)ap.Qh, dRowLeaf, T, RW,
-                               dVisitBits, dNodeVisit, dGroups, group, r, r_end, ap.iv, ap.ctl + 5, ap.n_queries, ap.iv_cap, ap.ctl + 7);
+                               dVisitDir, dVisitRec, dGroups, group, r, r_end, ap.iv, ap.ctl + 5, ap.n_queries, ap.iv_cap, ap.visit_recs, ap.ctl + 7);
     }
     return hipGetLastError();
 }
@@ -1792,8 +1795,8 @@
 template <int G, int KINDA>
 __global__ __launch_bounds__(256) void scan_approx128_kernel(const float *__restrict__ X, const uint4 *__restrict__ Qh,
                                                               const float4 *__restrict__ qmeta, const uint2 *__restrict__ rowLeaf,
-                                                              uint32_t T, uint32_t RW, const uint32_t *__restrict__ visitBits,
-                                                              const uint4 *__restrict__ nodeVisit, const ZhGroup *__restrict__ groups,
+                                                              uint32_t T, uint32_t RW, const uint2 *__restrict__ visitDir,
+                                                              const uint4 *__restrict__ visitRec, const ZhGroup *__restrict__ groups,
                                                               uint32_t GRP, uint64_t row_begin, uint64_t row_end, float Kc,
                                                               uint64_t *__restrict__ iv) {
     constexpr int LG = 64 / G, NH = G / 4, NR = 2 * NH;
@@ -1811,7 +1814,7 @@
     const uint2 *__restrict__ ent = rowLeaf + (size_t)r0 * T;
     uint32_t eGb[ZH_SCAN_NE], eWithin[ZH_SCAN_NE], eC[ZH_SCAN_NE], off[ZH_SCAN_NE], eB0[ZH_SCAN_NE];
     uint64_t eK0[ZH_SCAN_NE];
-    const uint32_t P = scan_phase1(lane, n_ent, ent, visitBits, nodeVisit, eGb, eWithin, eC, off, eB0, eK0);
+    const uint32_t P = scan_phase1(lane, n_ent, ent, visitDir, visitRec, eGb, eWithin, eC, off, eB0, eK0);
     if (P == 0) return;
     {
         const float4 *src = reinterpret_cast<const float4 *>(X) + (size_t)r0 * 32;
@@ -1928,7 +1931,7 @@
 
 template <int D, int G>
 static hipError_t launch_scan_approx_d(const float *dX, uint64_t n_rows, const ZhApprox &ap, const uint2 *dRowLeaf, uint32_t T,
-                                       const uint32_t *dVisitBits, const uint4 *dNodeVisit, const ZhGroup *dGroups, uint32_t group,
+                                       const uint2 *dVisitDir, const uint4 *dVisitRec, const ZhGroup *dGroups, uint32_t group,
                                        int metric, int mode, hipStream_t s) {
     const uint32_t RW = zh_scan_rows_per_wave(T);
     uint64_t rows_per_launch = zh_sweep_rows_per_launch(D);
@@ -1941,7 +1944,7 @@
         if (blocks > 0x7FFFFFFFull) return hipErrorInvalidValue;
 #define ZH_APX_LAUNCH(KA) \
         hipLaunchKernelGGL((scan_approx_kernel<D, G, KA>), dim3((uint32_t)blocks), dim3(256), 0, s, dX, (const uint4 *)ap.Qh, ap.qmeta, dRowLeaf, T, \
-                           RW, dVisitBits, dNodeVisit, dGroups, group, r, r_end, Kc, ap.iv)
+                           RW, dVisitDir, dVisitRec, dGroups, group, r, r_end, Kc, ap.iv)
         if (kinda == 0) ZH_APX_LAUNCH(0);
         else if (kinda == 1) ZH_APX_LAUNCH(1);
         else ZH_APX_LAUNCH(2);
@@ -1957,15 +1960,15 @@
 }
 
 hipError_t zh_launch_scan_approx(const float *dX, uint32_t d, uint64_t n_rows, ZhApprox ap, const uint2 *dRowLeaf, uint32_t T,
-                                 const uint32_t *dVisitBits, const uint4 *dNodeVisit, const ZhGroup *dGroups, uint32_t group, int metric,
+                                 const uint2 *dVisitDir, const uint4 *dVisitRec, const ZhGroup *dGroups, uint32_t group, int metric,
                                  int mode, hipStream_t s) {
     if (!n_rows) return hipSuccess;
     if (ap.mfma) switch (d) {
-    case 256: return launch_scan_mfma_d<256>(dX, n_rows, ap, dRowLeaf, T, dVisitBits, dNodeVisit, dGroups, group, s);
-    case 384: return launch_scan_mfma_d<384>(dX, n_rows, ap, dRowLeaf, T, dVisitBits, dNodeVisit, dGroups, group, s);
-    case 512: return launch_scan_mfma_d<512>(dX, n_rows, ap, dRowLeaf, T, dVisitBits, dNodeVisit, dGroups, group, s);
-    case 768: return launch_scan_mfma_d<768>(dX, n_rows, ap, dRowLeaf, T, dVisitBits, dNodeVisit, dGroups, group, s);
-    case 1024: return launch_scan_mfma_d<1024>(dX, n_rows, ap, dRowLeaf, T, dVisitBits, dNodeVisit, dGroups, group, s);
+    case 256: return launch_scan_mfma_d<256>(dX, n_rows, ap, dRowLeaf, T, dVisitDir, dVisitRec, dGroups, group, s);
+    case 384: return launch_scan_mfma_d<384>(dX, n_rows, ap, dRowLeaf, T, dVisitDir, dVisitRec, dGroups, group, s);
+    case 512: return launch_scan_mfma_d<512>(dX, n_rows, ap, dRowLeaf, T, dVisitDir, dVisitRec, dGroups, group, s);
+    case 768: return launch_scan_mfma_d<768>(dX, n_rows, ap, dRowLeaf, T, dVisitDir, dVisitRec, dGroups, group, s);
+    case 1024: return launch_scan_mfma_d<1024>(dX, n_rows, ap, dRowLeaf, T, dVisitDir, dVisitRec, dGroups, group, s);
     default: return hipErrorInvalidValue;
     }
     switch (d) {
@@ -1981,7 +1984,7 @@
             if (blocks > 0x7FFFFFFFull) return hipErrorInvalidValue;
 #define ZH_APX_LAUNCH(KA) \
             hipLaunchKernelGGL((scan_approx128_kernel<ZH_APX_G128, KA>), dim3((uint32_t)blocks), dim3(256), 0, s, dX, (const uint4 *)ap.Qh, ap.qmeta, dRowLeaf, T, RW, \
-                               dVisitBits, dNodeVisit, dGroups, group, r, r_end, Kc, ap.iv)
+                               dVisitDir, dVisitRec, dGroups, group, r, r_end, Kc, ap.iv)
             if (kinda == 0) ZH_APX_LAUNCH(0);
             else if (kinda == 1) ZH_APX_LAUNCH(1);
             else ZH_APX_LAUNCH(2);
@@ -1989,11 +1992,11 @@
         }
         return hipGetLastError();
     }
-    case 256: return launch_scan_approx_d<256, 4>(dX, n_rows, ap, dRowLeaf, T, dVisitBits, dNodeVisit, dGroups, group, metric, mode, s);
-    case 384: return launch_scan_approx_d<384, 4>(dX, n_rows, ap, dRowLeaf, T, dVisitBits, dNodeVisit, dGroups, group, metric, mode, s);
-    case 512: return launch_scan_approx_d<512, 2>(dX, n_rows, ap, dRowLeaf, T, dVisitBits, dNodeVisit, dGroups, group, metric, mode, s);
-    case 768: return launch_scan_approx_d<768, ZH_APX_G768>(dX, n_rows, ap, dRowLeaf, T, dVisitBits, dNodeVisit, dGroups, group, metric, mode, s);
-    case 1024: return launch_scan_approx_d<1024, 2>(dX, n_rows, ap, dRowLeaf, T, dVisitBits, dNodeVisit, dGroups, group, metric, mode, s);
+    case 256: return launch_scan_approx_d<256, 4>(dX, n_rows, ap, dRowLeaf, T, dVisitDir, dVisitRec, dGroups, group, metric, mode, s);
+    case 384: return launch_scan_approx_d<384, 4>(dX, n_rows, ap, dRowLeaf, T, dVisitDir, dVisitRec, dGroups, group, metric, mode, s);
+    case 512: return launch_scan_approx_d<512, 2>(dX, n_rows, ap, dRowLeaf, T, dVisitDir, dVisitRec, dGroups, group, metric, mode, s);
+    case 768: return launch_scan_approx_d<768, ZH_APX_G768>(dX, n_rows, ap, dRowLeaf, T, dVisitDir, dVisitRec, dGroups, group, metric, mode, s);
+    case 1024: return launch_scan_approx_d<1024, 2>(dX, n_rows, ap, dRowLeaf, T, dVisitDir, dVisitRec, dGroups, group, metric, mode, s);
     default: return hipErrorInvalidValue;
     }
 }
diff --git a/zebra_amd/csrc/zh_device.h b/zebra_amd/csrc/zh_device.h
--- a/zebra_amd/csrc/zh_device.h
+++ b/zebra_amd/csrc/zh_device.h
@@ -33,6 +33,10 @@
 }
 __device__ __forceinline__ float wave_sum_canonical(float s) { return wave_butterfly<OpAdd>(s); }
 __device__ __forceinline__ uint64_t f64_bits(double x) { return (uint64_t)__double_as_longlong(x); }
+__device__ __forceinline__ bool visit_dir_has(uint2 dw, uint32_t node) { return (dw.x >> (node & 31)) & 1u; }
+__device__ __forceinline__ uint32_t visit_dir_rank(uint2 dw, uint32_t node) {
+    return dw.y + (uint32_t)__popc(dw.x & ((1u << (node & 31)) - 1u));
+}
 
 __device__ __forceinline__ uint64_t key_cosine(float ab, float a2, float b2, int mode) {
     double c;
diff --git a/zebra_amd/csrc/zh_internal.h b/zebra_amd/csrc/zh_internal.h
--- a/zebra_amd/csrc/zh_internal.h
+++ b/zebra_amd/csrc/zh_internal.h
@@ -151,9 +151,9 @@
 hipError_t zh_launch_row_leaf(const int4 *dNodePack, const uint32_t *dNodeTree, uint32_t n_nodes, const uint32_t *dLeafIds,
                               uint32_t T, uint64_t n_rows, uint2 *dRowLeaf, hipStream_t s);
 hipError_t zh_launch_node_visits(const uint32_t *dLeafCount, const uint32_t *dGroupBase, const ZhGroup *dGroups, uint32_t n_nodes,
-                                 uint32_t *dBits, uint4 *dNodeVisit, hipStream_t s);
+                                 uint2 *dVisitDir, uint4 *dVisitRec, uint32_t rec_cap, hipStream_t s);
 hipError_t zh_launch_scan_sweep(const float *dX, uint32_t d, uint64_t n_rows, const float *dQ, const float *dQQ,
-                                const uint2 *dRowLeaf, uint32_t T, const uint32_t *dVisitBits, const uint4 *dNodeVisit,
+                                const uint2 *dRowLeaf, uint32_t T, const uint2 *dVisitDir, const uint4 *dVisitRec,
                                 const ZhGroup *dGroups, uint32_t group, int metric, int param, uint64_t *dKeys,
                                 const uint32_t *dRunIf , hipStream_t s);
 uint64_t zh_sweep_rows_per_launch(uint32_t d);
@@ -193,6 +193,7 @@
     uint32_t mfma;
     uint32_t n_queries;
     uint64_t iv_cap;
+    uint32_t visit_recs;
     float nx_max;
 };
 uint32_t zh_approx_groups(uint32_t d);
@@ -215,7 +216,7 @@
 hipError_t zh_launch_row_byte128(const float *dX, uint64_t row0, uint64_t n_rows, void *dXb, uint32_t *dNotBytes, hipStream_t s);
 hipError_t zh_launch_exact_register(const ZhVisit *dVisits, uint64_t n_visits, uint32_t k, ZhApprox ap, hipStream_t s);
 hipError_t zh_launch_scan_approx(const float *dX, uint32_t d, uint64_t n_rows, ZhApprox ap, const uint2 *dRowLeaf, uint32_t T,
-                                 const uint32_t *dVisitBits, const uint4 *dNodeVisit, const ZhGroup *dGroups, uint32_t group, int metric,
+                                 const uint2 *dVisitDir, const uint4 *dVisitRec, const ZhGroup *dGroups, uint32_t group, int metric,
                                  int mode, hipStream_t s);
 hipError_t zh_launch_select_interval(const ZhVisit *dVisits, uint64_t n_visits, uint32_t k, const uint32_t *dLeafIds, ZhApprox ap,
                                      int metric, int mode, uint32_t d, hipStream_t s);
diff --git a/zebra_amd/csrc/zh_search.hip b/zebra_amd/csrc/zh_search.hip
--- a/zebra_amd/csrc/zh_search.hip
+++ b/zebra_amd/csrc/zh_search.hip
@@ -1553,29 +1553,63 @@
     return hipGetLastError();
 }
 
-__global__ __launch_bounds__(256) void node_visit_kernel(const uint32_t *__restrict__ leafCount, const uint32_t *__restrict__ groupBase,
-                                                          const ZhGroup *__restrict__ groups, uint32_t n_nodes,
-                                                          uint32_t *__restrict__ bits, uint4 *__restrict__ nodeVisit) {
+__global__ __launch_bounds__(256) void visit_bits_kernel(const uint32_t *__restrict__ leafCount, uint32_t n_nodes, uint2 *__restrict__ dir) {
     const uint32_t w = blockIdx.x * blockDim.x + threadIdx.x;
     const uint32_t n0 = w * 32;
     if (n0 >= n_nodes) return;
     uint32_t word = 0;
-    for (uint32_t i = 0; i < 32 && n0 + i < n_nodes; i++) {
-        const uint32_t c = leafCount[n0 + i];
-        if (c) {
-            word |= 1u << i;
-            const uint32_t gb = groupBase[n0 + i];
-            const uint64_t k0 = groups[gb].key_off[0];
-            nodeVisit[n0 + i] = make_uint4(c | ((uint32_t)(k0 >> 32) << 28), gb, groups[gb].b[0], (uint32_t)k0);
-        }
-    }
-    bits[w] = word;
+    for (uint32_t i = 0; i < 32 && n0 + i < n_nodes; i++)
+        if (leafCount[n0 + i]) word |= 1u << i;
+    dir[w] = make_uint2(word, 0u);
+}
+__global__ __launch_bounds__(1024) void visit_prefix_kernel(uint2 *__restrict__ dir, uint32_t words) {
+    __shared__ uint32_t wave_sum[16];
+    const uint32_t lane = threadIdx.x & 63, wid = threadIdx.x >> 6;
+    uint32_t base = 0;
+    for (uint32_t w0 = 0; w0 < words; w0 += 1024) {
+        const uint32_t w = w0 + threadIdx.x;
+        const uint32_t c = w < words ? (uint32_t)__popc(dir[w].x) : 0u;
+        uint32_t incl = c;
+#pragma unroll
+        for (int o = 1; o < 64; o <<= 1) {
+            const uint32_t t = __shfl_up(incl, o);
+            if (lane >= (uint32_t)o) incl += t;
+        }
+        if (lane == 63) wave_sum[wid] = incl;
+        __syncthreads();
+        uint32_t before = 0, total = 0;
+        for (uint32_t i = 0; i < 16; i++) {
+            const uint32_t v = wave_sum[i];
+            if (i < wid) before += v;
+            total += v;
+        }
+        if (w < words) dir[w].y = base + before + incl - c;
+        base += total;
+        __syncthreads();
+    }
+}
+__global__ __launch_bounds__(256) void node_visit_kernel(const uint32_t *__restrict__ leafCount, const uint32_t *__restrict__ groupBase,
+                                                          const ZhGroup *__restrict__ groups, uint32_t n_nodes,
+                                                          const uint2 *__restrict__ dir, uint4 *__restrict__ rec, uint32_t rec_cap) {
+    const uint32_t w = blockIdx.x * blockDim.x + threadIdx.x;
+    const uint32_t n0 = w * 32;
+    if (n0 >= n_nodes) return;
+    const uint2 dw = dir[w];
+    uint32_t rank = dw.y;
+    for (uint32_t m = dw.x; m; m &= m - 1, rank++) {
+        const uint32_t n = n0 + (uint32_t)__builtin_ctz(m);
+        const uint32_t c = leafCount[n], gb = groupBase[n];
+        const uint64_t k0 = groups[gb].key_off[0];
+        if (rank < rec_cap) rec[rank] = make_uint4(c | ((uint32_t)(k0 >> 32) << 28), gb, groups[gb].b[0], (uint32_t)k0);
+    }
 }
 hipError_t zh_launch_node_visits(const uint32_t *dLeafCount, const uint32_t *dGroupBase, const ZhGroup *dGroups, uint32_t n_nodes,
-                                 uint32_t *dBits, uint4 *dNodeVisit, hipStream_t s) {
+                                 uint2 *dVisitDir, uint4 *dVisitRec, uint32_t rec_cap, hipStream_t s) {
     const uint32_t words = (n_nodes + 31) / 32;
     if (!words) return hipSuccess;
-    hipLaunchKernelGGL(node_visit_kernel, dim3((words + 255) / 256), dim3(256), 0, s, dLeafCount, dGroupBase, dGroups, n_nodes, dBits, dNodeVisit);
+    hipLaunchKernelGGL(visit_bits_kernel, dim3((words + 255) / 256), dim3(256), 0, s, dLeafCount, n_nodes, dVisitDir);
+    hipLaunchKernelGGL(visit_prefix_kernel, dim3(1), dim3(1024), 0, s, dVisitDir, words);
+    hipLaunchKernelGGL(node_visit_kernel, dim3((words + 255) / 256), dim3(256), 0, s, dLeafCount, dGroupBase, dGroups, n_nodes, dVisitDir, dVisitRec, rec_cap);
     return hipGetLastError();
 }
 
@@ -1583,8 +1617,8 @@
 template <int D, int KIND>
 __global__ __launch_bounds__(256) void scan_sweep_kernel(const float *__restrict__ X, const float *__restrict__ Q,
                                                           const float *__restrict__ QQ, const uint2 *__restrict__ rowLeaf,
-                                                          uint32_t T, uint32_t RW, const uint32_t *__restrict__ visitBits,
-                                                          const uint4 *__restrict__ nodeVisit,
+                                                          uint32_t T, uint32_t RW, const uint2 *__restrict__ visitDir,
+                                                          const uint4 *__restrict__ visitRec,
                                                           const ZhGroup *__restrict__ groups, uint32_t GRP, uint64_t row_begin,
                                                           uint64_t row_end, int metric, int param,
                                                           uint64_t *__restrict__ keys, const uint32_t *__restrict__ run_if) {
@@ -1610,8 +1644,9 @@
             const unsigned long long rlw = __builtin_nontemporal_load(reinterpret_cast<const unsigned long long *>(ent + e));
             const uint2 rl = make_uint2((uint32_t)rlw, (uint32_t)(rlw >> 32));
             eWithin[j] = rl.y;
-            if (rl.x != 0xFFFFFFFFu && ((visitBits[rl.x >> 5] >> (rl.x & 31)) & 1u)) {
-                const uint4 nv = nodeVisit[rl.x];
+            const uint2 dw = rl.x != 0xFFFFFFFFu ? visitDir[rl.x >> 5] : make_uint2(0u, 0u);
+            if (visit_dir_has(dw, rl.x)) {
+                const uint4 nv = visitRec[visit_dir_rank(dw, rl.x)];
                 eC[j] = nv.x & 0x0FFFFFFFu; eGb[j] = nv.y; eB0[j] = nv.z;
                 eK0[j] = ((uint64_t)(nv.x >> 28) << 32) | nv.w;
             }
@@ -1758,8 +1793,8 @@
 template <int KIND>
 __global__ __launch_bounds__(256) void scan128_sweep_kernel(const float *__restrict__ X, const float *__restrict__ Q,
                                                              const float *__restrict__ QQ, const uint2 *__restrict__ rowLeaf,
-                                                             uint32_t T, uint32_t RW, const uint32_t *__restrict__ visitBits,
-                                                             const uint4 *__restrict__ nodeVisit,
+                                                             uint32_t T, uint32_t RW, const uint2 *__restrict__ visitDir,
+                                                             const uint4 *__restrict__ visitRec,
                                                              const ZhGroup *__restrict__ groups, uint32_t GRP, uint64_t row_begin,
                                                              uint64_t row_end, int metric, int param,
                                                              uint64_t *__restrict__ keys, const uint32_t *__restrict__ run_if) {
@@ -1789,8 +1824,9 @@
             const unsigned long long rlw = __builtin_nontemporal_load(reinterpret_cast<const unsigned long long *>(ent + e));
             const uint2 rl = make_uint2((uint32_t)rlw, (uint32_t)(rlw >> 32));
             eWithin[j] = rl.y;
-            if (rl.x != 0xFFFFFFFFu && ((visitBits[rl.x >> 5] >> (rl.x & 31)) & 1u)) {
-                const uint4 nv = nodeVisit[rl.x];
+            const uint2 dw = rl.x != 0xFFFFFFFFu ? visitDir[rl.x >> 5] : make_uint2(0u, 0u);
+            if (visit_dir_has(dw, rl.x)) {
+                const uint4 nv = visitRec[visit_dir_rank(dw, rl.x)];
                 eC[j] = nv.x & 0x0FFFFFFFu; eGb[j] = nv.y; eB0[j] = nv.z;
                 eK0[j] = ((uint64_t)(nv.x >> 28) << 32) | nv.w;
             }
@@ -1943,7 +1979,7 @@
 
 template <int D, int KIND>
 static hipError_t launch_scan_dk(const float *dX, uint64_t n_rows, const float *dQ, const float *dQQ, const uint2 *dRowLeaf,
-                                 uint32_t T, const uint32_t *dVisitBits, const uint4 *dNodeVisit, const ZhGroup *dGroups,
+                                 uint32_t T, const uint2 *dVisitDir, const uint4 *dVisitRec, const ZhGroup *dGroups,
                                  uint32_t group, int metric, int param, uint64_t *dKeys, const uint32_t *dRunIf, hipStream_t s) {
     const uint32_t RW = zh_scan_rows_per_wave(T);
     uint64_t rows_per_launch = zh_sweep_rows_per_launch(D);
@@ -1954,19 +1990,19 @@
         if (blocks > 0x7FFFFFFFull) return hipErrorInvalidValue;
         if constexpr (D == 128 && (KIND == K_L2 || KIND == K_COS))
             hipLaunchKernelGGL((scan128_sweep_kernel<KIND>), dim3((uint32_t)blocks), dim3(256), 0, s, dX, dQ, dQQ, dRowLeaf, T, RW,
-                               dVisitBits, dNodeVisit, dGroups, group, r, r_end, metric, param, dKeys, dRunIf);
+                               dVisitDir, dVisitRec, dGroups, group, r, r_end, metric, param, dKeys, dRunIf);
         else
             hipLaunchKernelGGL((scan_sweep_kernel<D, KIND>), dim3((uint32_t)blocks), dim3(256), 0, s, dX, dQ, dQQ, dRowLeaf, T, RW,
-                               dVisitBits, dNodeVisit, dGroups, group, r, r_end, metric, param, dKeys, dRunIf);
+                               dVisitDir, dVisitRec, dGroups, group, r, r_end, metric, param, dKeys, dRunIf);
     }
     return hipGetLastError();
 }
 template <int KIND>
 static hipError_t launch_scan_k(const float *dX, uint32_t d, uint64_t n_rows, const float *dQ, const float *dQQ,
-                                const uint2 *dRowLeaf, uint32_t T, const uint32_t *dVisitBits, const uint4 *dNodeVisit,
+                                const uint2 *dRowLeaf, uint32_t T, const uint2 *dVisitDir, const uint4 *dVisitRec,
                                 const ZhGroup *dGroups, uint32_t group, int metric, int param, uint64_t *dKeys, const uint32_t *dRunIf, hipStream_t s) {
 #define ZH_SCAN_CASE(DD) \
-    case DD: return launch_scan_dk<DD, KIND>(dX, n_rows, dQ, dQQ, dRowLeaf, T, dVisitBits, dNodeVisit, dGroups, group, metric, param, dKeys, dRunIf, s)
+    case DD: return launch_scan_dk<DD, KIND>(dX, n_rows, dQ, dQQ, dRowLeaf, T, dVisitDir, dVisitRec, dGroups, group, metric, param, dKeys, dRunIf, s)
     if constexpr (KIND == K_L2 || KIND == K_COS) {
         switch (d) {
             ZH_SCAN_CASE(64); ZH_SCAN_CASE(256); ZH_SCAN_CASE(512); ZH_SCAN_CASE(1024); ZH_SCAN_CASE(1536);
@@ -1980,12 +2016,12 @@
 #undef ZH_SCAN_CASE
 }
 hipError_t zh_launch_scan_sweep(const float *dX, uint32_t d, uint64_t n_rows, const float *dQ, const float *dQQ,
-                                const uint2 *dRowLeaf, uint32_t T, const uint32_t *dVisitBits, const uint4 *dNodeVisit,
+                                const uint2 *dRowLeaf, uint32_t T, const uint2 *dVisitDir, const uint4 *dVisitRec,
                                 const ZhGroup *dGroups, uint32_t group, int metric, int param, uint64_t *dKeys, const uint32_t *dRunIf,
                                 hipStream_t s) {
     if (!n_rows) return hipSuccess;
 #define ZH_KIND_CASE(K) \
-    case K: return launch_scan_k<K>(dX, d, n_rows, dQ, dQQ, dRowLeaf, T, dVisitBits, dNodeVisit, dGroups, group, metric, param, dKeys, dRunIf, s)
+    case K: return launch_scan_k<K>(dX, d, n_rows, dQ, dQQ, dRowLeaf, T, dVisitDir, dVisitRec, dGroups, group, metric, param, dKeys, dRunIf, s)
     switch (zh_kind_of(metric)) {
         ZH_KIND_CASE(K_COS);
         ZH_KIND_CASE(K_MAX);
@@ -1996,7 +2032,7 @@
         ZH_KIND_CASE(K_P4);
         ZH_KIND_CASE(K_HAMM);
         ZH_KIND_CASE(K_PP);
-    default: return launch_scan_k<K_L2>(dX, d, n_rows, dQ, dQQ, dRowLeaf, T, dVisitBits, dNodeVisit, dGroups, group, metric, param, dKeys, dRunIf, s);
+    default: return launch_scan_k<K_L2>(dX, d, n_rows, dQ, dQQ, dRowLeaf, T, dVisitDir, dVisitRec, dGroups, group, metric, param, dKeys, dRunIf, s);
     }
 #undef ZH_KIND_CASE
 }
```
